# tanmayb123/OpenAI-Whisper-CoreML

Hardware: AMD Instinct MI355X
Metric: audio-sec/s (RTF) + decoder tok/s, Whisper-large-v2 30s chunks, 1->8 GPU (higher is better)
Workload: dtype bf16

## Files before the change

include/whisper_mi355x_debug.h:

```cpp
#ifndef WHISPER_MI355X_DEBUG_H
#define WHISPER_MI355X_DEBUG_H

#include "whisper_mi355x.h"

#ifdef __cplusplus
extern "C" {
#endif

WM_API int wmdbg_mel_filterbank(int n_mels, float *out);
WM_API int wmdbg_mel80(float *out);

WM_API int wmdbg_gemm(wm_ctx *ctx, const float *A, const float *W, const float *bias, float *C, int M, int N,
               int K, int epi);
WM_API int wmdbg_layernorm(wm_ctx *ctx, const float *x, const float *g, const float *b, int rows, int d,
                    float *out_f32, float *out_bf16_as_f32);
WM_API int wmdbg_enc_attention(wm_ctx *ctx, const float *q, const float *k, const float *v, int B, int H, int S,
                        float *out);
WM_API int wmdbg_dec_gemv(wm_ctx *ctx, const float *x, const float *ln_g, const float *ln_b, const float *W,
                   const float *bias, float *out, int B, int N, int K);
WM_API int wmdbg_dec_gemv_resid(wm_ctx *ctx, const float *x, const float *W, const float *bias, float *resid, float *copy_bf16,
                         float *stats, int B, int N, int K);
WM_API int wmdbg_dec_attention(wm_ctx *ctx, const float *q, const float *k, const float *v, int B, int H, int T,
                        int n_keys, int nsplit, float *out);

WM_API int wmdbg_bench_dec_gemv(wm_ctx *ctx, int B, int N, int K, int ln, int resid, int n_mats, int iters,
                         int nw_override, float *avg_us);
WM_API int wmdbg_bench_dec_attention(wm_ctx *ctx, int B, int H, int T, int n_keys, int nsplit, int n_slices,
                              int iters, float *avg_us);

WM_API int wmdbg_bench_launch_floor(wm_ctx *ctx, int iters, int grid, float *eager_us, float *graph_us);

WM_API int wmdbg_bench_graph_branches(wm_ctx *ctx, int iters, int grid, int us_each, float *one_us, float *two_us);

WM_API int wmdbg_bench_gemm(wm_ctx *ctx, int M, int N, int K, int epi, int iters, int n_w, float *us);

WM_API int wmdbg_set_gemm_tile(int tile);

WM_API int wmdbg_lane_parts(int B, int lanes, int explicit_lanes, int n_text_state);
WM_API int wmdbg_cu_mask(int cu_lo, int cu_hi, uint32_t *mask8);

WM_API int wmdbg_set_precision(wm_ctx *ctx, int precision);

WM_API int wmdbg_set_tuning(const char *key, int value);
WM_API int wmdbg_group_count(int B, int lanes, int explicit_lanes);

#ifdef __cplusplus
}
#endif
#endif
```

openai-whisper-coreml_amd/csrc/debug_hooks.cpp:

```cpp
#include <math.h>
#include <stdio.h>
#include <stdlib.h>
#include <string.h>

#include <vector>

#include "../../include/whisper_mi355x_debug.h"
#include "model.h"

int wm_gemm_set_tile_override(int tile);
extern "C" int wmdbg_set_gemm_tile(int tile) { return wm_gemm_set_tile_override(tile); }

extern "C" int wmdbg_set_tuning(const char *key, int value) {
    WM_REQUIRE(key, WM_ERR_INVALID, "wmdbg_set_tuning: null key");
    struct { const char *name; int *field; } table[] = {
        {"gemv_tn", &g_wm_tuning.gemv_tn}, {"gemv_nblk", &g_wm_tuning.gemv_nblk}, {"gemv_no_ppw2", &g_wm_tuning.gemv_no_ppw2}, {"gemv_ppw2_nblk", &g_wm_tuning.gemv_ppw2_nblk},
        {"prefetch_max_b", &g_wm_tuning.prefetch_max_b}, {"xattn_split_below", &g_wm_tuning.xattn_split_below},
        {"xattn_wgs", &g_wm_tuning.xattn_wgs}, {"xattn_no_flat", &g_wm_tuning.xattn_no_flat},
        {"xattn_lds_pad", &g_wm_tuning.xattn_lds_pad}, {"xattn_splits", &g_wm_tuning.xattn_splits},
        {"gemm_tile", &g_wm_tuning.gemm_tile}, {"gemm128_pipe", &g_wm_tuning.gemm128_pipe}, {"gemm_gm", &g_wm_tuning.gemm_gm}, {"no_early_stop", &g_wm_tuning.no_early_stop},
        {"xattn_no_deep", &g_wm_tuning.xattn_no_deep}, {"xattn_never_short", &g_wm_tuning.xattn_never_short},         {"logits_tn", &g_wm_tuning.logits_tn}, {"enc_attn_mfma_sum", &g_wm_tuning.enc_attn_mfma_sum},
        {"group_chunks", &g_wm_tuning.group_chunks}, {"argmax_rows_per_wg", &g_wm_tuning.argmax_rows_per_wg}, {"xattn_fuse_q", &g_wm_tuning.xattn_fuse_q},
        {"lane_parts", &g_wm_tuning.lane_parts}, {"lane_solo_cus", &g_wm_tuning.lane_solo_cus}, {"frontend_per_wave_twiddles", &g_wm_tuning.frontend_per_wave_twiddles},
    };
    if (strcmp(key, "reset") == 0) { g_wm_tuning = WmTuning(); return WM_OK; }
    for (auto &e : table)
        if (strcmp(key, e.name) == 0) { *e.field = value; return WM_OK; }
    wm_set_error("wmdbg_set_tuning: unknown key '%s'", key);
    return WM_ERR_INVALID;
}

extern "C" int wmdbg_group_count(int B, int lanes, int explicit_lanes) { return wm_group_count(B, lanes, explicit_lanes != 0, 0); }
extern "C" int wmdbg_lane_parts(int B, int lanes, int explicit_lanes, int n_text_state) {
    return wm_lane_parts(B, lanes, explicit_lanes != 0, n_text_state, 0);
}
extern "C" int wmdbg_cu_mask(int cu_lo, int cu_hi, uint32_t *mask8) { return wm_cu_mask(cu_lo, cu_hi, mask8); }

extern "C" int wmdbg_mel_filterbank(int n_mels, float *out) {
    WM_REQUIRE(out && n_mels > 0 && n_mels <= 256, WM_ERR_INVALID, "bad args");
    std::vector<float> f;
    wm_mel_filterbank(n_mels, f);
    memcpy(out, f.data(), f.size() * sizeof(float));
    return WM_OK;
}
extern "C" int wmdbg_mel80(float *out) {
    WM_REQUIRE(out, WM_ERR_INVALID, "null");
    memcpy(out, wm_mel80_table(), sizeof(float) * 80 * 201);
    return WM_OK;
}

static int up(void **d, const void *h, size_t bytes, hipStream_t s) {
    WM_HIP(hipMalloc(d, bytes + 512));
    WM_HIP(hipMemsetAsync(*d, 0, bytes + 512, s));
    if (h) WM_HIP(hipMemcpyAsync(*d, h, bytes, hipMemcpyHostToDevice, s));
    return WM_OK;
}
static void to_bf16(const float *in, std::vector<bf16_t> &out, size_t n) {
    out.resize(n);
    for (size_t i = 0; i < n; ++i) {
        uint32_t u;
        memcpy(&u, &in[i], 4);
        u += 0x7fffu + ((u >> 16) & 1u);
        out[i] = (bf16_t)(u >> 16);
    }
}
static void from_bf16(const std::vector<bf16_t> &in, float *out) {
    for (size_t i = 0; i < in.size(); ++i) {
        uint32_t u = (uint32_t)in[i] << 16;
        memcpy(&out[i], &u, 4);
    }
}

extern "C" int wmdbg_gemm(wm_ctx *ctx, const float *A, const float *W, const float *bias, float *C, int M, int N,
                          int K, int epi) {
    WM_TRY(wm_ctx_make_current(ctx));
    WM_REQUIRE(epi == EPI_F32 || epi == EPI_BIAS_BF16 || epi == EPI_GELU_BF16 || epi == EPI_RESID_F32, WM_ERR_INVALID,
               "wmdbg_gemm: epilogue %d not exposed", epi);
    std::vector<bf16_t> a16, w16;
    to_bf16(A, a16, (size_t)M * K);
    to_bf16(W, w16, (size_t)N * K);
    void *dA, *dW, *dB = nullptr, *dC;
    hipStream_t s = ctx->stream;
    WM_TRY(up(&dA, a16.data(), a16.size() * 2, s));
    WM_TRY(up(&dW, w16.data(), w16.size() * 2, s));
    if (bias) WM_TRY(up(&dB, bias, (size_t)N * 4, s));
    const bool f32out = (epi == EPI_F32 || epi == EPI_RESID_F32);
    WM_TRY(up(&dC, epi == EPI_RESID_F32 ? C : nullptr, (size_t)M * N * (f32out ? 4 : 2), s));
    GemmArgs g;
    memset(&g, 0, sizeof(g));
    g.A = (const bf16_t *)dA; g.a_rpb = (long)M + 1; g.a_rstride = K;
    g.W = (const bf16_t *)dW; g.bias = (const float *)dB; g.C = dC;
    g.c_rpb = (long)M + 1; g.c_rstride = N; g.M = M; g.N = N; g.K = K; g.epi = epi;
    int rc = wm_gemm(ctx, g);
    if (rc == WM_OK) {
        if (f32out) {
            WM_HIP(hipMemcpyAsync(C, dC, (size_t)M * N * 4, hipMemcpyDeviceToHost, s));
            WM_HIP(hipStreamSynchronize(s));
        } else {
            std::vector<bf16_t> c16((size_t)M * N);
            WM_HIP(hipMemcpyAsync(c16.data(), dC, c16.size() * 2, hipMemcpyDeviceToHost, s));
            WM_HIP(hipStreamSynchronize(s));
            from_bf16(c16, C);
        }
    }
    (void)hipFree(dA); (void)hipFree(dW); (void)hipFree(dC);
    if (dB) (void)hipFree(dB);
    return rc;
}

extern "C" int wmdbg_layernorm(wm_ctx *ctx, const float *x, const float *g, const float *b, int rows, int d,
                               float *out_f32, float *out_bf16_as_f32) {
    WM_TRY(wm_ctx_make_current(ctx));
    void *dx, *dg, *db, *of, *ob;
    hipStream_t s = ctx->stream;
    WM_TRY(up(&dx, x, (size_t)rows * d * 4, s));
    WM_TRY(up(&dg, g, (size_t)d * 4, s));
    WM_TRY(up(&db, b, (size_t)d * 4, s));
    WM_TRY(up(&of, nullptr, (size_t)rows * d * 4, s));
    WM_TRY(up(&ob, nullptr, (size_t)rows * d * 2, s));
    int rc = wm_layernorm(ctx, (const float *)dx, (const float *)dg, (const float *)db, rows, d, (bf16_t *)ob, (float *)of);
    if (rc == WM_OK) {
        std::vector<bf16_t> t((size_t)rows * d);
        WM_HIP(hipMemcpyAsync(out_f32, of, (size_t)rows * d * 4, hipMemcpyDeviceToHost, s));
        WM_HIP(hipMemcpyAsync(t.data(), ob, t.size() * 2, hipMemcpyDeviceToHost, s));
        WM_HIP(hipStreamSynchronize(s));
        from_bf16(t, out_bf16_as_f32);
    }
    (void)hipFree(dx); (void)hipFree(dg); (void)hipFree(db); (void)hipFree(of); (void)hipFree(ob);
    return rc;
}

extern "C" int wmdbg_enc_attention(wm_ctx *ctx, const float *q, const float *k, const float *v, int B, int H, int S,
                                   float *out) {
    WM_TRY(wm_ctx_make_current(ctx));
    const int d = H * 64, S_pad = ((S + 63) / 64) * 64;
    const size_t M = (size_t)B * S;
    std::vector<bf16_t> qk((M + 64) * 2 * d, 0), vt((size_t)B * H * 64 * S_pad, 0), tmp;
    auto bf = [](float f) { uint32_t u; memcpy(&u, &f, 4); u += 0x7fffu + ((u >> 16) & 1u); return (bf16_t)(u >> 16); };
    for (size_t mrow = 0; mrow < M; ++mrow)
        for (int j = 0; j < d; ++j) {
            qk[mrow * 2 * d + j] = bf(q[mrow * d + j] * WM_ENC_QSCALE);
            qk[mrow * 2 * d + d + j] = bf(k[mrow * d + j]);
        }
    for (int b = 0; b < B; ++b)
        for (int s = 0; s < S; ++s)
            for (int j = 0; j < d; ++j)
                vt[((size_t)(b * H + j / 64) * 64 + j % 64) * S_pad + wm_att_vt_pos((unsigned)s)] = bf(v[((size_t)b * S + s) * d + j]);
    void *dqk, *dvt, *datt;
    hipStream_t st = ctx->stream;
    WM_TRY(up(&dqk, qk.data(), qk.size() * 2, st));
    WM_TRY(up(&dvt, vt.data(), vt.size() * 2, st));
    WM_TRY(up(&datt, nullptr, M * d * 2, st));
    int rc = wm_enc_attention(ctx, (const bf16_t *)dqk, (const bf16_t *)dvt, (bf16_t *)datt, B, H, S, S_pad, d);
    if (rc == WM_OK) {
        tmp.resize(M * d);
        WM_HIP(hipMemcpyAsync(tmp.data(), datt, tmp.size() * 2, hipMemcpyDeviceToHost, st));
        WM_HIP(hipStreamSynchronize(st));
        from_bf16(tmp, out);
    }
    (void)hipFree(dqk); (void)hipFree(dvt); (void)hipFree(datt);
    return rc;
}

extern "C" int wmdbg_dec_gemv(wm_ctx *ctx, const float *x, const float *ln_g, const float *ln_b, const float *W,
                              const float *bias, float *out, int B, int N, int K) {
    WM_TRY(wm_ctx_make_current(ctx));
    WM_REQUIRE(B >= 1 && B <= WM_DEC_MAXB, WM_ERR_INVALID, "wmdbg_dec_gemv: B out of range");
    const int Npad = ((N + 15) / 16) * 16;
    std::vector<bf16_t> w16, x16;
    std::vector<float> wp((size_t)Npad * K, 0.f);
    for (size_t r = 0; r < (size_t)N; ++r)
        for (size_t k = 0; k < (size_t)K; ++k) wp[wm_tiled_offset(r, k, (size_t)K)] = W[r * K + k];
    to_bf16(wp.data(), w16, wp.size());
    {
        const int Bpad = ((B + 15) / 16) * 16;
        std::vector<float> xp((size_t)Bpad * K, 0.f);
        for (size_t b = 0; b < (size_t)B; ++b)
            for (size_t k = 0; k < (size_t)K; ++k) xp[wm_tiled_offset(b, k, (size_t)K)] = x[b * K + k];
        to_bf16(xp.data(), x16, xp.size());
    }
    void *dx16, *dg = nullptr, *db = nullptr, *dW, *dWf = nullptr, *dc1 = nullptr, *dc2 = nullptr, *dbias = nullptr, *dout;
    hipStream_t s = ctx->stream;
    WM_TRY(up(&dx16, x16.data(), x16.size() * 2, s));
    WM_TRY(up(&dW, w16.data(), w16.size() * 2, s));
    WM_TRY(up(&dout, nullptr, (size_t)B * N * 4, s));
    if (bias) WM_TRY(up(&dbias, bias, (size_t)N * 4, s));
    DecGemvArgs a;
    memset(&a, 0, sizeof(a));
    a.B = B; a.N = N; a.K = K; a.W = (const bf16_t *)dW; a.c2 = (const float *)dbias; a.a = (const bf16_t *)dx16;
    a.out_f32 = (float *)dout; a.ldo = N; a.epi = DE_Q; a.pos_ptr = nullptr;
    void *dst = nullptr;
    int rc = WM_OK;
    if (ln_g) {
        WM_TRY(up(&dg, ln_g, (size_t)K * 4, s));
        WM_TRY(up(&db, ln_b, (size_t)K * 4, s));
        WM_TRY(up(&dWf, nullptr, w16.size() * 2, s));
        WM_TRY(up(&dc1, nullptr, (size_t)Npad * 4, s));
        WM_TRY(up(&dc2, nullptr, (size_t)Npad * 4, s));
        rc = wm_ln_fold(ctx, (const bf16_t *)dW, (const float *)dg, (const float *)db, (const float *)dbias, N, K,
                        (bf16_t *)dWf, (float *)dc1, (float *)dc2);
        const int nblk = (B + 15) / 16;
        std::vector<float> st((size_t)nblk * 2 * K, 0.f);
        for (int b = 0; b < B; ++b)
            for (int k = 0; k < K; ++k) {
                const int part = k >> 4;
                const float v = x[(size_t)b * K + k];
                float *blk = st.data() + (size_t)(b >> 4) * 2 * K;
                blk[(part * 16 + (b & 15)) * 2] += v;
                blk[(part * 16 + (b & 15)) * 2 + 1] += v * v;
            }
        WM_TRY(up(&dst, st.data(), st.size() * 4, s));
        a.stats_in = (const float *)dst; a.stats_parts = K / 16;
        a.W = (const bf16_t *)dWf; a.c1 = (const float *)dc1; a.c2 = (const float *)dc2;
    }
    if (rc == WM_OK) rc = wm_dec_gemv(ctx, a);
    if (rc == WM_OK) {
        WM_HIP(hipMemcpyAsync(out, dout, (size_t)B * N * 4, hipMemcpyDeviceToHost, s));
        WM_HIP(hipStreamSynchronize(s));
    }
    void *fr[] = {dx16, dg, db, dW, dWf, dc1, dc2, dbias, dout, dst};
    for (void *p : fr)
        if (p) (void)hipFree(p);
    return rc;
}

extern "C" int wmdbg_dec_gemv_resid(wm_ctx *ctx, const float *x, const float *W, const float *bias, float *resid,
                                    float *copy_bf16, float *stats, int B, int N, int K) {
    WM_TRY(wm_ctx_make_current(ctx));
    WM_REQUIRE(B >= 1 && B <= WM_DEC_MAXB && N % 16 == 0, WM_ERR_INVALID, "wmdbg_dec_gemv_resid: B out of range / N % 16");
    const int Bpad = ((B + 15) / 16) * 16;
    std::vector<bf16_t> w16, x16;
    {
        std::vector<float> wp((size_t)N * K, 0.f), xp((size_t)Bpad * K, 0.f);
        for (size_t r = 0; r < (size_t)N; ++r)
            for (size_t k = 0; k < (size_t)K; ++k) wp[wm_tiled_offset(r, k, (size_t)K)] = W[r * K + k];
        for (size_t b = 0; b < (size_t)B; ++b)
            for (size_t k = 0; k < (size_t)K; ++k) xp[wm_tiled_offset(b, k, (size_t)K)] = x[b * K + k];
        to_bf16(wp.data(), w16, wp.size());
        to_bf16(xp.data(), x16, xp.size());
    }
    void *dx16, *dW, *dbias = nullptr, *dres, *dcopy, *dst;
    hipStream_t s = ctx->stream;
    WM_TRY(up(&dx16, x16.data(), x16.size() * 2, s));
    WM_TRY(up(&dW, w16.data(), w16.size() * 2, s));
    WM_TRY(up(&dres, resid, (size_t)B * N * 4, s));
    WM_TRY(up(&dcopy, nullptr, (size_t)Bpad * N * 2, s));
    WM_TRY(up(&dst, nullptr, (size_t)(Bpad / 16) * 2 * N * 4, s));
    if (bias) WM_TRY(up(&dbias, bias, (size_t)N * 4, s));
    DecGemvArgs a;
    memset(&a, 0, sizeof(a));
    a.epi = DE_RESID; a.B = B; a.N = N; a.K = K; a.W = (const bf16_t *)dW; a.c2 = (const float *)dbias;
    a.a = (const bf16_t *)dx16; a.out_f32 = (float *)dres; a.out_bf16 = (bf16_t *)dcopy; a.ldo = N;
    a.stats_out = (float *)dst;
    int rc = wm_dec_gemv(ctx, a);
    if (rc == WM_OK) {
        std::vector<bf16_t> c16((size_t)Bpad * N), lin((size_t)B * N);
        std::vector<float> st((size_t)(Bpad / 16) * 2 * N);
        WM_HIP(hipMemcpyAsync(resid, dres, (size_t)B * N * 4, hipMemcpyDeviceToHost, s));
        WM_HIP(hipMemcpyAsync(c16.data(), dcopy, c16.size() * 2, hipMemcpyDeviceToHost, s));
        WM_HIP(hipMemcpyAsync(st.data(), dst, st.size() * 4, hipMemcpyDeviceToHost, s));
        WM_HIP(hipStreamSynchronize(s));
        for (size_t b = 0; b < (size_t)B; ++b)
            for (size_t n = 0; n < (size_t)N; ++n) lin[b * N + n] = c16[wm_tiled_offset(b, n, (size_t)N)];
        from_bf16(lin, copy_bf16);
        for (int b = 0; b < B; ++b) {
            const float *blk = st.data() + (size_t)(b >> 4) * 2 * N;
            float s1 = 0.f, s2 = 0.f;
            for (int part = 0; part < N / 16; ++part) {
                s1 += blk[(part * 16 + (b & 15)) * 2];
                s2 += blk[(part * 16 + (b & 15)) * 2 + 1];
            }
            stats[b * 2] = s1;
            stats[b * 2 + 1] = s2;
        }
    }
    void *fr[] = {dx16, dW, dbias, dres, dcopy, dst};
    for (void *p : fr)
        if (p) (void)hipFree(p);
    return rc;
}

extern "C" int wmdbg_dec_attention(wm_ctx *ctx, const float *q, const float *k, const float *v, int B, int H, int T,
                                   int n_keys, int nsplit, float *out) {
    WM_TRY(wm_ctx_make_current(ctx));
    std::vector<bf16_t> k16, v16;
    to_bf16(k, k16, (size_t)B * H * T * 64);
    to_bf16(v, v16, (size_t)B * H * T * 64);
    void *dq, *dk, *dv, *dp;
    hipStream_t s = ctx->stream;
    WM_TRY(up(&dq, q, (size_t)B * H * 64 * 4, s));
    WM_TRY(up(&dk, k16.data(), k16.size() * 2, s));
    WM_TRY(up(&dv, v16.data(), v16.size() * 2, s));
    WM_TRY(up(&dp, nullptr, (size_t)B * H * WM_MAXSPLIT * 66 * 4, s));
    void *datt;
    WM_TRY(up(&datt, nullptr, ((size_t)B + 15) / 16 * 16 * H * 64 * 2, s));
    int rc = nsplit == 0 ? wm_dec_self_attention(ctx, (const float *)dq, (const bf16_t *)dk, (const bf16_t *)dv, B, H, T,
                                                 n_keys, nullptr, (bf16_t *)datt)
                         : wm_dec_attention(ctx, (const float *)dq, (const bf16_t *)dk, (const bf16_t *)dv, B, H, T, n_keys,
                                            nullptr, nsplit < 0 ? 1 : nsplit, (float *)dp, (bf16_t *)datt, nsplit < 0);
    if (rc == WM_OK) {
        const size_t Bpad = ((size_t)B + 15) / 16 * 16, dd = (size_t)H * 64;
        std::vector<bf16_t> o16(Bpad * dd), lin((size_t)B * dd);
        WM_HIP(hipMemcpyAsync(o16.data(), datt, o16.size() * 2, hipMemcpyDeviceToHost, s));
        WM_HIP(hipStreamSynchronize(s));
        for (size_t b = 0; b < (size_t)B; ++b)
            for (size_t k = 0; k < dd; ++k) lin[b * dd + k] = o16[wm_tiled_offset(b, k, dd)];
        from_bf16(lin, out);
    }
    (void)hipFree(datt);
    (void)hipFree(dq); (void)hipFree(dk); (void)hipFree(dv); (void)hipFree(dp);
    return rc;
}


extern "C" int wmdbg_bench_dec_gemv(wm_ctx *ctx, int B, int N, int K, int ln, int resid, int n_mats, int iters,
                                    int nw_override, float *avg_us) {
    (void)nw_override;
    WM_TRY(wm_ctx_make_current(ctx));
    WM_REQUIRE(B >= 1 && B <= WM_DEC_MAXB, WM_ERR_INVALID, "wmdbg_bench_dec_gemv: B out of range");
    hipStream_t s = ctx->stream;
    const int Npad = ((N + 15) / 16) * 16;
    void *dW, *dx16, *dc, *dout, *dout16;
    WM_TRY(up(&dW, nullptr, (size_t)n_mats * Npad * K * 2, s));
    WM_TRY(up(&dx16, nullptr, (size_t)WM_DEC_MAXB * K * 2, s));
    WM_TRY(up(&dc, nullptr, (size_t)Npad * 4, s));
    WM_TRY(up(&dout, nullptr, (size_t)WM_DEC_MAXB * Npad * 4, s));
    WM_TRY(up(&dout16, nullptr, (size_t)WM_DEC_MAXB * Npad * 2, s));
    WM_HIP(hipMemsetAsync(dW, 0x3c, (size_t)n_mats * Npad * K * 2, s));
    DecGemvArgs a;
    memset(&a, 0, sizeof(a));
    a.B = B; a.N = N; a.K = K; a.out_f32 = (float *)dout; a.ldo = Npad; a.epi = resid ? DE_RESID : DE_Q;
    a.a = (const bf16_t *)dx16; a.c2 = (const float *)dc;
    void *dstat;
    WM_TRY(up(&dstat, nullptr, (size_t)(WM_DEC_MAXB / 16) * 2 * (K > N ? K : N) * 4 + 4096, s));
    if (resid) { a.stats_out = (float *)dstat; a.out_bf16 = (bf16_t *)dout16; }
    if (ln) { a.c1 = (const float *)dc; a.stats_in = (const float *)dstat; a.stats_parts = K / 16; }
    hipEvent_t e0, e1;
    WM_HIP(hipEventCreate(&e0));
    WM_HIP(hipEventCreate(&e1));
    int rc = WM_OK;
    hipGraph_t g = nullptr;
    hipGraphExec_t ge = nullptr;
    WM_HIP(hipStreamBeginCapture(s, hipStreamCaptureModeThreadLocal));
    for (int i = 0; i < iters && rc == WM_OK; ++i) {
        a.W = (const bf16_t *)dW + (size_t)(i % n_mats) * Npad * K;
        rc = wm_dec_gemv(ctx, a);
    }
    WM_HIP(hipStreamEndCapture(s, &g));
    if (rc == WM_OK) {
        WM_HIP(hipGraphInstantiate(&ge, g, nullptr, nullptr, 0));
        WM_HIP(hipGraphLaunch(ge, s));
        WM_HIP(hipStreamSynchronize(s));
        WM_HIP(hipEventRecord(e0, s));
        WM_HIP(hipGraphLaunch(ge, s));
    }
    WM_HIP(hipEventRecord(e1, s));
    WM_HIP(hipStreamSynchronize(s));
    float ms = 0.f;
    WM_HIP(hipEventElapsedTime(&ms, e0, e1));
    *avg_us = ms * 1e3f / iters;
    (void)hipEventDestroy(e0); (void)hipEventDestroy(e1);
    if (ge) (void)hipGraphExecDestroy(ge);
    if (g) (void)hipGraphDestroy(g);
    void *fr[] = {dW, dx16, dc, dout, dout16, dstat};
    for (void *p : fr) (void)hipFree(p);
    return rc;
}

extern "C" int wmdbg_bench_dec_attention(wm_ctx *ctx, int B, int H, int T, int n_keys, int nsplit, int n_slices,
                                         int iters, float *avg_us) {
    WM_TRY(wm_ctx_make_current(ctx));
    hipStream_t s = ctx->stream;
    const size_t slice = (size_t)B * H * T * 64;
    void *dk, *dv, *dq, *dp, *datt;
    WM_TRY(up(&dk, nullptr, slice * n_slices * 2, s));
    WM_TRY(up(&dv, nullptr, slice * n_slices * 2, s));
    WM_TRY(up(&dq, nullptr, (size_t)B * H * 64 * 4, s));
    WM_TRY(up(&dp, nullptr, (size_t)B * H * WM_MAXSPLIT * 66 * 4, s));
    WM_TRY(up(&datt, nullptr, ((size_t)B + 15) / 16 * 16 * H * 64 * 2, s));
    hipEvent_t e0, e1;
    WM_HIP(hipEventCreate(&e0));
    WM_HIP(hipEventCreate(&e1));
    int rc = WM_OK;
    for (int pass = 0; pass < 2 && rc == WM_OK; ++pass) {
        if (pass == 1) WM_HIP(hipEventRecord(e0, s));
        for (int i = 0; i < iters && rc == WM_OK; ++i)
            rc = wm_dec_attention(ctx, (const float *)dq, (const bf16_t *)dk + (size_t)(i % n_slices) * slice,
                                  (const bf16_t *)dv + (size_t)(i % n_slices) * slice, B, H, T, n_keys, nullptr, nsplit,
                                  (float *)dp, (bf16_t *)datt, true);
    }
    WM_HIP(hipEventRecord(e1, s));
    WM_HIP(hipStreamSynchronize(s));
    float ms = 0.f;
    WM_HIP(hipEventElapsedTime(&ms, e0, e1));
    *avg_us = ms * 1e3f / iters;
    (void)hipEventDestroy(e0); (void)hipEventDestroy(e1);
    void *fr[] = {dk, dv, dq, dp, datt};
    for (void *p : fr) (void)hipFree(p);
    return rc;
}

int wm_launch_trivial(wm_ctx *ctx, int *p, int grid);
extern "C" int wmdbg_bench_launch_floor(wm_ctx *ctx, int iters, int grid, float *eager_us, float *graph_us) {
    WM_TRY(wm_ctx_make_current(ctx));
    hipStream_t s = ctx->stream;
    void *d;
    WM_TRY(up(&d, nullptr, 64, s));
    hipEvent_t e0, e1;
    WM_HIP(hipEventCreate(&e0));
    WM_HIP(hipEventCreate(&e1));
    for (int i = 0; i < 20; ++i) WM_TRY(wm_launch_trivial(ctx, (int *)d, grid));
    WM_HIP(hipEventRecord(e0, s));
    for (int i = 0; i < iters; ++i) WM_TRY(wm_launch_trivial(ctx, (int *)d, grid));
    WM_HIP(hipEventRecord(e1, s));
    WM_HIP(hipStreamSynchronize(s));
    float ms = 0.f;
    WM_HIP(hipEventElapsedTime(&ms, e0, e1));
    *eager_us = ms * 1e3f / iters;
    hipGraph_t g;
    hipGraphExec_t ge;
    WM_HIP(hipStreamBeginCapture(s, hipStreamCaptureModeThreadLocal));
    for (int i = 0; i < iters; ++i) (void)wm_launch_trivial(ctx, (int *)d, grid);
    WM_HIP(hipStreamEndCapture(s, &g));
    WM_HIP(hipGraphInstantiate(&ge, g, nullptr, nullptr, 0));
    WM_HIP(hipGraphLaunch(ge, s));
    WM_HIP(hipStreamSynchronize(s));
    WM_HIP(hipEventRecord(e0, s));
    WM_HIP(hipGraphLaunch(ge, s));
    WM_HIP(hipEventRecord(e1, s));
    WM_HIP(hipStreamSynchronize(s));
    WM_HIP(hipEventElapsedTime(&ms, e0, e1));
    *graph_us = ms * 1e3f / iters;
    (void)hipGraphExecDestroy(ge); (void)hipGraphDestroy(g);
    (void)hipEventDestroy(e0); (void)hipEventDestroy(e1); (void)hipFree(d);
    return WM_OK;
}

extern "C" int wmdbg_bench_gemm(wm_ctx *ctx, int M, int N, int K, int epi, int iters, int n_w, float *us) {
    WM_TRY(wm_ctx_make_current(ctx));
    WM_REQUIRE(epi == EPI_F32 || epi == EPI_BIAS_BF16 || epi == EPI_GELU_BF16 || epi == EPI_RESID_F32, WM_ERR_INVALID,
               "wmdbg_bench_gemm: epilogue %d not exposed", epi);
    WM_REQUIRE(n_w >= 1 && n_w <= 64, WM_ERR_INVALID, "wmdbg_bench_gemm: n_w out of range");
    hipStream_t s = ctx->stream;
    std::vector<bf16_t> a16((size_t)M * K), w16((size_t)N * K);
    uint32_t x = 12345u;
    auto gauss = [&]() {
        float acc = 0.f;
        for (int i = 0; i < 4; ++i) { x = x * 1664525u + 1013904223u; acc += (float)(x >> 8) * (1.0f / 16777216.0f); }
        return (acc - 2.0f) * 1.7320508f;
    };
    auto f2bf = [](float f) {
        uint32_t u;
        memcpy(&u, &f, 4);
        u += 0x7fffu + ((u >> 16) & 1u);
        return (bf16_t)(u >> 16);
    };
    for (auto &v : a16) v = f2bf(gauss());
    for (auto &v : w16) v = f2bf(0.02f * gauss());
    std::vector<float> bias(N);
    for (auto &v : bias) v = 0.01f * gauss();
    void *dA, *dB, *dC;
    std::vector<void *> dW(n_w, nullptr);
    WM_TRY(up(&dA, a16.data(), a16.size() * 2, s));
    for (int i = 0; i < n_w; ++i) WM_TRY(up(&dW[i], w16.data(), w16.size() * 2, s));
    WM_TRY(up(&dB, bias.data(), (size_t)N * 4, s));
    WM_TRY(up(&dC, nullptr, (size_t)M * N * 4, s));
    GemmArgs g;
    memset(&g, 0, sizeof(g));
    g.A = (const bf16_t *)dA; g.a_rpb = (long)M + 1; g.a_rstride = K;
    g.bias = (const float *)dB; g.C = dC;
    g.c_rpb = (long)M + 1; g.c_rstride = N; g.M = M; g.N = N; g.K = K; g.epi = epi;
    hipEvent_t e0, e1;
    WM_HIP(hipEventCreate(&e0));
    WM_HIP(hipEventCreate(&e1));
    for (int i = 0; i < 3; ++i) { g.W = (const bf16_t *)dW[i % n_w]; WM_TRY(wm_gemm(ctx, g)); }
    WM_HIP(hipEventRecord(e0, s));
    for (int i = 0; i < iters; ++i) { g.W = (const bf16_t *)dW[i % n_w]; WM_TRY(wm_gemm(ctx, g)); }
    WM_HIP(hipEventRecord(e1, s));
    WM_HIP(hipStreamSynchronize(s));
    float ms = 0.f;
    WM_HIP(hipEventElapsedTime(&ms, e0, e1));
    *us = ms * 1e3f / iters;
    (void)hipEventDestroy(e0); (void)hipEventDestroy(e1);
    (void)hipFree(dA); (void)hipFree(dB); (void)hipFree(dC);
    for (void *w : dW) (void)hipFree(w);
    return WM_OK;
}

int wm_launch_spin(hipStream_t s, int *p, int grid, int cycles);
extern "C" int wmdbg_bench_graph_branches(wm_ctx *ctx, int iters, int grid, int us_each, float *one_us, float *two_us) {
    WM_TRY(wm_ctx_make_current(ctx));
    hipStream_t s = ctx->stream, s2;
    WM_HIP(hipStreamCreateWithFlags(&s2, hipStreamNonBlocking));
    void *d;
    WM_TRY(up(&d, nullptr, 256, s));
    const int cycles = us_each * 100;
    hipEvent_t e0, e1, ef, ej;
    WM_HIP(hipEventCreate(&e0)); WM_HIP(hipEventCreate(&e1));
    WM_HIP(hipEventCreateWithFlags(&ef, hipEventDisableTiming)); WM_HIP(hipEventCreateWithFlags(&ej, hipEventDisableTiming));
    for (int nb = 1; nb <= 2; ++nb) {
        hipGraph_t g; hipGraphExec_t ge;
        WM_HIP(hipStreamBeginCapture(s, hipStreamCaptureModeThreadLocal));
        if (nb == 2) { WM_HIP(hipEventRecord(ef, s)); WM_HIP(hipStreamWaitEvent(s2, ef, 0)); }
        for (int i = 0; i < iters; ++i) {
            WM_TRY(wm_launch_spin(s, (int *)d, grid, cycles));
            if (nb == 2) WM_TRY(wm_launch_spin(s2, (int *)d + 16, grid, cycles));
        }
        if (nb == 2) { WM_HIP(hipEventRecord(ej, s2)); WM_HIP(hipStreamWaitEvent(s, ej, 0)); }
        WM_HIP(hipStreamEndCapture(s, &g));
        WM_HIP(hipGraphInstantiate(&ge, g, nullptr, nullptr, 0));
        WM_HIP(hipGraphLaunch(ge, s));
        WM_HIP(hipStreamSynchronize(s));
        WM_HIP(hipEventRecord(e0, s));
        WM_HIP(hipGraphLaunch(ge, s));
        WM_HIP(hipEventRecord(e1, s));
        WM_HIP(hipStreamSynchronize(s));
        float ms = 0.f;
        WM_HIP(hipEventElapsedTime(&ms, e0, e1));
        *(nb == 1 ? one_us : two_us) = ms * 1e3f;
        (void)hipGraphExecDestroy(ge); (void)hipGraphDestroy(g);
    }
    (void)hipEventDestroy(e0); (void)hipEventDestroy(e1); (void)hipEventDestroy(ef); (void)hipEventDestroy(ej);
    (void)hipStreamDestroy(s2); (void)hipFree(d);
    return WM_OK;
}
```

openai-whisper-coreml_amd/csrc/dec_kernels.hip:

```cpp
#include <stdlib.h>

#include <atomic>
#include <string.h>

#include "model.h"

namespace {

typedef __attribute__((ext_vector_type(8))) __bf16 bf16x8;
typedef __attribute__((ext_vector_type(4))) float f32x4;
typedef __attribute__((ext_vector_type(4))) unsigned u32x4;

typedef __attribute__((ext_vector_type(2))) float f32x2;
typedef __attribute__((ext_vector_type(2))) __bf16 bf16x2;

__device__ __forceinline__ bf16_t f2bf(float f) {
    const __bf16 h = (__bf16)f;
    return __builtin_bit_cast(bf16_t, h);
}
__device__ __forceinline__ float bf2f(bf16_t h) { return __uint_as_float((unsigned)h << 16); }
__device__ __forceinline__ unsigned pack2(float a, float b) {
    const f32x2 v = {a, b};
    return __builtin_bit_cast(unsigned, __builtin_convertvector(v, bf16x2));
}
// ... 208 lines not shown
            if (bvalid && nrow == 0) p.tilemax[(long)b * p.n_tiles + tile] = key;
            if (bvalid && nvalid && p.out_f32) p.out_f32[(long)b * p.ldo + n] = v;
            continue;
        }
        if (EPI == DE_RESID) {
            float xn = 0.f;
            if (bvalid && nvalid) {
                xn = o.xold[r] + v;
                p.out_f32[(long)b * p.ldo + n] = xn;
                if (p.out_bf16) p.out_bf16[wm_tiled_offset((size_t)b, (size_t)n, (size_t)p.ldo)] = f2bf(xn - o.off4[r]);
            }
            float s1 = xn, s2 = xn * xn;
#pragma unroll
            for (int q = 1; q < 16; q <<= 1) {
                s1 += __shfl_xor(s1, q);
                s2 += __shfl_xor(s2, q);
            }
            if (p.stats_out && nrow == 0)
                *(float2 *)(p.stats_out + (long)(b0 >> 4) * p.stats_stride + ((long)tile * 16 + bl) * 2) = make_float2(s1, s2);
            continue;
        }
        if (!bvalid || !nvalid) continue;
        if (EPI == DE_QKV) {
            const int d = p.N / 3;
            if (n < d) {
                p.out_f32[(long)b * d + n] = v;
            } else {
                const int hn = (n < 2 * d) ? n - d : n - 2 * d;
                bf16_t *c = (n < 2 * d) ? p.kcache : p.vcache;
                c[((long)(b * p.n_head + (hn >> 6)) * p.n_ctx + pos) * 64 + (hn & 63)] = f2bf(v);
            }
        } else if (EPI == DE_Q) {
            p.out_f32[(long)b * p.ldo + n] = v;
        } else if (EPI == DE_GELU) {
            p.out_bf16[wm_tiled_offset((size_t)b, (size_t)n, (size_t)p.ldo)] = f2bf(gelu_erf(v));
        }
    }
}

#define GEMV_PIN(x) asm volatile("" ::"s"(x))
template <int SPW, int TN, int NBLK, int EPI, bool LN, int PPW = 1, int RSP = 1>
__global__ __launch_bounds__((LN || SPW == 12 || TN * NBLK > 1 || PPW > 1) ? 512 : 1024) void dec_gemv_kernel(
    const bf16_t *__restrict__ hotW, const bf16_t *__restrict__ hotA, const int *__restrict__ hot_pos_ptr,
    const float *__restrict__ hot_c2, int hotK, int hot_n_tiles, int hotB, int hot_bgroups, int hot_n_tg, int hot_n_tg_pad,
    float *hot_out_f32, DecGemvDev pc) {
    extern __shared__ __attribute__((aligned(16))) char smem[];
    DecGemvDev p = pc;
    p.W = hotW; p.a = hotA; p.pos_ptr = hot_pos_ptr; p.c2 = hot_c2; p.K = hotK; p.n_tiles = hot_n_tiles; p.B = hotB;
    p.bgroups = hot_bgroups; p.n_tg = hot_n_tg; p.n_tg_pad = hot_n_tg_pad; p.out_f32 = hot_out_f32;
    constexpr int NU = TN * NBLK;
    const int NP = (p.K >> 5) / SPW;
    const int NW = NP / PPW;
    const int G = p.bgroups;
    const int wg = blockIdx.x;
    const int q = wg >> 3;
    const int tg = G == 1 ? wg : (q / G) * 8 + (wg & 7);
    const int grp = G == 1 ? 0 : q % G;
    if (wg >= p.n_tg_pad * G || tg >= p.n_tg) {
        int t = wg - p.n_tg_pad * G;
        if (p.pf_head_major && t >= 0) {
            const int per = p.pf_head_major, x = t & 7, m = t >> 3;
            const int hh = (x * per) / p.B + (m >> 2);
            const int end = (x + 1) * per < (p.pf_tiles >> 2) * p.B ? (x + 1) * per : (p.pf_tiles >> 2) * p.B;
            t = hh * p.B < end ? hh * 4 + (m & 3) : -1;
        }
        if (t >= 0 && t < p.pf_tiles) l2_warm_tile(p.pf_ptr, p.pf_tile_bytes, t, NW * 64);
        return;
    }
    float *red = (float *)smem;
    float *st = red + NP * NU * 256 + (threadIdx.x >> 6) * 32;
    const int tid = threadIdx.x, lane = tid & 63, wave = tid >> 6;
    const int nrow = lane & 15;
    const int tile0 = tg * TN;
    const int bb = grp * NBLK * 16;

    u32x4 wf[TN][SPW];
    auto load_wf = [&](int part) {
#pragma unroll
        for (int t = 0; t < TN; ++t) {
            const int tc = tile0 + t < p.n_tiles ? tile0 + t : p.n_tiles - 1;
            const bf16_t *wp = p.W + (((long)tc * (p.K >> 5) + (long)part * SPW) * 64 + lane) * 8;
#pragma unroll
#ifdef WM_GEMV_W_NONTEMPORAL
            for (int u = 0; u < SPW; ++u) wf[t][u] = __builtin_nontemporal_load((const u32x4 *)(wp + u * 512));
#else
            for (int u = 0; u < SPW; ++u) wf[t][u] = *(const u32x4 *)(wp + u * 512);
#endif
        }
    };
    load_wf(wave);
    u32x4 af[NBLK][SPW];
    auto load_af = [&](int part) {
#pragma unroll
        for (int j = 0; j < NBLK; ++j) {
            const int blk = (bb >> 4) + j;
            const int blkc = blk * 16 < p.B ? blk : (bb >> 4);
            const bf16_t *ap = p.a + (((long)blkc * (p.K >> 5) + (long)part * SPW) * 64 + lane) * 8;
#pragma unroll
            for (int u = 0; u < SPW; ++u) af[j][u] = *(const u32x4 *)(ap + u * 512);
        }
    };
    load_af(wave);
    GEMV_PIN(p.N); GEMV_PIN(p.ldo);
    if (LN) { GEMV_PIN(p.c1); GEMV_PIN(p.stats_in); GEMV_PIN(p.stats_stride); GEMV_PIN(p.mean_in); GEMV_PIN(p.mean_out); }
    if (EPI == DE_RESID) { GEMV_PIN(p.out_bf16); GEMV_PIN(p.stats_out); GEMV_PIN(p.stats_stride); GEMV_PIN(p.mean_in); }
    if (EPI == DE_QKV) { GEMV_PIN(p.kcache); GEMV_PIN(p.vcache); GEMV_PIN(p.n_ctx); GEMV_PIN(p.n_head); }
    if (EPI == DE_GELU) GEMV_PIN(p.out_bf16);
    if (EPI == DE_LOGITS) {
        GEMV_PIN(p.tilemax); GEMV_PIN(p.arg_first); GEMV_PIN(p.arg_last); GEMV_PIN(p.mask); GEMV_PIN(p.mask_words);
        GEMV_PIN(p.mask_first_pos); GEMV_PIN(p.ts.rng); GEMV_PIN(p.ts.key_ts); GEMV_PIN(p.ts.lse); GEMV_PIN(p.ts.ts_begin);
    }
    int pos = 0;
    unsigned mword0 = 0u, mword1 = 0u;
    GemvUnitOps<EPI, LN> ops;
    constexpr int RS = RSP;
    static_assert(RSP == 1 || RSP == 4, "row split: 1 or 4 waves per unit");
    constexpr int rs_shift = RS == 4 ? 2 : 0;
    const int ntask = NU << rs_shift;
    const bool has_unit = wave < ntask;
    const int my_u = wave >> rs_shift;
    const int my_r0 = RS == 4 ? (wave & 3) : 0, my_r1 = RS == 4 ? my_r0 + 1 : 4;
    const bool my_stats = my_r0 == 0;
    int utile = tile0, ub0 = bb;
    if (has_unit) {
        utile = tile0 + my_u % TN;
        ub0 = bb + (my_u / TN) * 16;
        if (utile >= p.n_tiles) utile = p.n_tiles - 1;
        if (ub0 >= p.B) ub0 = bb;
        gemv_unit_load<EPI, LN>(p, ops, utile, ub0, lane, my_r0, my_r1, my_stats);
    }
    if (p.pos_ptr) pos = *p.pos_ptr;
    if (EPI == DE_LOGITS && p.mask && has_unit) {
        const int n = utile * 16 + nrow;
        const int nc = n < p.N ? n : p.N - 1;
        mword0 = p.mask[nc >> 5];
        mword1 = p.mask[p.mask_words + (nc >> 5)];
    }

    f32x4 acc[NBLK][TN];
#pragma unroll
    for (int pp = 0; pp < PPW; ++pp) {
        const int part = wave + pp * NW;
        if (pp > 0) {
            load_wf(part);
            load_af(part);
        }
#pragma unroll
        for (int j = 0; j < NBLK; ++j)
#pragma unroll
            for (int t = 0; t < TN; ++t) {
                f32x4 a4 = {0.f, 0.f, 0.f, 0.f};
#pragma unroll
                for (int u = 0; u < SPW; ++u)
                    a4 = __builtin_amdgcn_mfma_f32_16x16x32_bf16(__builtin_bit_cast(bf16x8, af[j][u]),
                                                                 __builtin_bit_cast(bf16x8, wf[t][u]), a4, 0, 0, 0);
                acc[j][t] = a4;
            }
        if (PPW > 1 || NU > 1 || wave != 0 || RS == 4) {
#pragma unroll
            for (int j = 0; j < NBLK; ++j)
#pragma unroll
                for (int t = 0; t < TN; ++t) *(f32x4 *)(red + ((part * NU + j * TN + t) * 64 + lane) * 4) = acc[j][t];
        }
    }
    float *stbase = red + NP * NU * 256;
    if (has_unit && my_stats) gemv_unit_stats<EPI, LN>(p, ops, stbase + (RS == 4 ? my_u : wave) * 32, lane, utile, ub0);
    __syncthreads();
    for (int tk = wave; tk < ntask; tk += NW) {
        const int u = tk >> rs_shift;
        const int t = u % TN, j = u / TN;
        const int tile = tile0 + t, b0 = bb + j * 16;
        if (tile >= p.n_tiles || b0 >= p.B) continue;
        st = stbase + (RS == 4 ? u : wave) * 32;
        if (tk != wave) {
            gemv_unit_load<EPI, LN>(p, ops, tile, b0, lane);
            gemv_unit_stats<EPI, LN>(p, ops, st, lane, tile, b0);
            if (EPI == DE_LOGITS && p.mask) {
                const int n = tile * 16 + nrow;
                const int nc = n < p.N ? n : p.N - 1;
                mword0 = p.mask[nc >> 5];
                mword1 = p.mask[p.mask_words + (nc >> 5)];
            }
        }
        f32x4 sum;
        if (RS == 4) {
            const float *rp = red + (u * 64 + lane) * 4 + my_r0;
            float s1 = rp[0];
            for (int w = 1; w < NP; ++w) s1 += rp[w * NU * 256];
            sum = f32x4{s1, s1, s1, s1};
        } else {
            sum = (NU == 1 && PPW == 1) ? acc[0][0] : *(const f32x4 *)(red + ((0 * NU + u) * 64 + lane) * 4);
            for (int w = 1; w < NP; ++w) sum += *(const f32x4 *)(red + ((w * NU + u) * 64 + lane) * 4);
        }
        gemv_unit_epilogue<EPI, LN>(p, ops, sum, st, tile, b0, lane, pos, mword0, mword1, my_r0, my_r1);
    }
}

__global__ __launch_bounds__(256) void ln_fold_kernel(const bf16_t *__restrict__ W, const float *__restrict__ g,
                                                      const float *__restrict__ beta, const float *__restrict__ bias,
                                                      int N, int K, bf16_t *__restrict__ Wf, float *__restrict__ c1,
                                                      float *__restrict__ c2) {
    __shared__ float r1[4], r2[4];
    const int n = blockIdx.x;
    float s1 = 0.f, s2 = 0.f;
    for (int k = threadIdx.x; k < K; k += 256) {
        const size_t o = wm_tiled_offset((size_t)n, (size_t)k, (size_t)K);
        const float w = bf2f(W[o]);
        const bf16_t wf = f2bf(w * g[k]);
        Wf[o] = wf;
        s1 += bf2f(wf);
        s2 += beta[k] * w;
    }
#pragma unroll
    for (int o = 32; o > 0; o >>= 1) {
        s1 += __shfl_xor(s1, o);
        s2 += __shfl_xor(s2, o);
    }
    if ((threadIdx.x & 63) == 0) {
        r1[threadIdx.x >> 6] = s1;
        r2[threadIdx.x >> 6] = s2;
    }
    __syncthreads();
    if (threadIdx.x == 0) {
        c1[n] = (r1[0] + r1[1]) + (r1[2] + r1[3]);
        c2[n] = (n < N && bias ? bias[n] : 0.f) + ((r2[0] + r2[1]) + (r2[2] + r2[3]));
    }
}

__global__ __launch_bounds__(256) void dec_embed_kernel(const int *__restrict__ seq, const int *__restrict__ pos_ptr,
                                                        int B, const bf16_t *__restrict__ emb,
                                                        const float *__restrict__ pemb, int d,
                                                        float *__restrict__ x, bf16_t *__restrict__ xb,
                                                        float *__restrict__ stats_out, float *__restrict__ mean_buf) {
    __shared__ float r1[4], r2[4];
    const int b = blockIdx.x;
    const int pos = *pos_ptr;
    const long tok = seq[pos * B + b];
    float s1 = 0.f, s2 = 0.f;
    for (int j = threadIdx.x; j < d; j += 256) {
        const float v = bf2f(emb[wm_tiled_offset((size_t)tok, (size_t)j, (size_t)d)]) + pemb[(long)pos * d + j];
        x[(long)b * d + j] = v;
        s1 += v;
        s2 += v * v;
    }
#pragma unroll
    for (int o = 32; o > 0; o >>= 1) {
        s1 += __shfl_xor(s1, o);
        s2 += __shfl_xor(s2, o);
    }
    if ((threadIdx.x & 63) == 0) {
        r1[threadIdx.x >> 6] = s1;
        r2[threadIdx.x >> 6] = s2;
    }
    __syncthreads();
    {
        const float mean = ((r1[0] + r1[1]) + (r1[2] + r1[3])) / (float)d;
        for (int j = threadIdx.x; j < d; j += 256)
            xb[wm_tiled_offset((size_t)b, (size_t)j, (size_t)d)] = f2bf(x[(long)b * d + j] - mean);
        if (threadIdx.x == 0 && mean_buf) mean_buf[b] = mean;
    }
    if (stats_out) {
        float *blk = stats_out + (long)(b >> 4) * (2 * d) + (b & 15) * 2;
        for (int pt = 1 + threadIdx.x; pt < d / 16; pt += 256) *(float2 *)(blk + pt * 32) = make_float2(0.f, 0.f);
        if (threadIdx.x == 0)
            *(float2 *)blk = make_float2((r1[0] + r1[1]) + (r1[2] + r1[3]), (r2[0] + r2[1]) + (r2[2] + r2[3]));
    }
}

constexpr int ATT_MAXK = 1536;
#ifndef WM_XATTN_NT
#define WM_XATTN_NT true
#endif

template <int NS>
__device__ __forceinline__ float attn_merge(const float *m, const float *l, const float *o, int ostride, int e) {
    float mm[NS], ll[NS], oo[NS];
#pragma unroll
    for (int w = 0; w < NS; ++w) {
        mm[w] = m[w];
        ll[w] = l[w];
        oo[w] = o[w * ostride + e];
    }
    return attn_merge_core<NS>(mm, ll, oo);
}


template <int NS, int U, bool NT>
__device__ __forceinline__ void attn_load_block(const bf16_t *kb, const bf16_t *vb, int r0, const int &stream, const int &rg,
                                                int lim, int clamp, u32x4 (&kv)[U], u32x4 (&vv)[U]) {
#pragma unroll
    for (int u = 0; u < U; ++u) {
        int i = r0 + u * (NS * 8) + stream * 8 + rg;
        i = i < lim ? i : clamp;
        if (NT) {
            kv[u] = __builtin_nontemporal_load((const u32x4 *)(kb + (long)i * 64));
            vv[u] = __builtin_nontemporal_load((const u32x4 *)(vb + (long)i * 64));
        } else {
            kv[u] = *(const u32x4 *)(kb + (long)i * 64);
            vv[u] = *(const u32x4 *)(vb + (long)i * 64);
        }
    }
}

template <int U>
__device__ __forceinline__ void attn_block_fence(u32x4 (&kv)[U], u32x4 (&vv)[U]) {
    static_assert(U == 4, "attn_block_fence is written for 4 loads per block");
    asm volatile("" : "+v"(kv[0]), "+v"(kv[1]), "+v"(kv[2]), "+v"(kv[3]), "+v"(vv[0]), "+v"(vv[1]), "+v"(vv[2]), "+v"(vv[3]));
}

template <int NS, int U, bool MASK_V>
__device__ __forceinline__ void attn_block(const float (&qe)[8], int r0, int stream, int rg, int n_keys, const u32x4 (&kv)[U],
                                           const u32x4 (&vv)[U], float &m_run, float &l_run, float (&oa)[8]) {
    float sc[U];
    float mb = -1e30f;
#pragma unroll
    for (int u = 0; u < U; ++u) {
        const int i = r0 + u * (NS * 8) + stream * 8 + rg;
        float a = 0.f;
#pragma unroll
        for (int j = 0; j < 4; ++j) {
            a = __fmaf_rn(qe[2 * j], __uint_as_float(kv[u][j] << 16), a);
            a = __fmaf_rn(qe[2 * j + 1], __uint_as_float(kv[u][j] & 0xffff0000u), a);
        }
        a += __shfl_xor(a, 1);
        a += __shfl_xor(a, 2);
        a += __shfl_xor(a, 4);
        sc[u] = i < n_keys ? a : -1e30f;
        mb = fmaxf(mb, sc[u]);
    }
    mb = fmaxf(mb, __shfl_xor(mb, 8));
    mb = fmaxf(mb, __shfl_xor(mb, 16));
    mb = fmaxf(mb, __shfl_xor(mb, 32));
    const float m_new = fmaxf(m_run, mb);
    const float resc = __expf(m_run - m_new);
    l_run *= resc;
#pragma unroll
    for (int j = 0; j < 8; ++j) oa[j] *= resc;
#pragma unroll
    for (int u = 0; u < U; ++u) {
        const bool live_row = sc[u] > -1e29f;
        const float pv = live_row ? __expf(sc[u] - m_new) : 0.f;
        l_run += pv;
#pragma unroll
        for (int j = 0; j < 4; ++j) {
            const unsigned vw = (MASK_V && !live_row) ? 0u : vv[u][j];
            oa[2 * j] = __fmaf_rn(pv, __uint_as_float(vw << 16), oa[2 * j]);
            oa[2 * j + 1] = __fmaf_rn(pv, __uint_as_float(vw & 0xffff0000u), oa[2 * j + 1]);
        }
    }
    m_run = m_new;
}

__device__ __forceinline__ void attn_stream_reduce(float &l_run, float (&oa)[8]) {
#pragma unroll
    for (int i = 0; i < 8; ++i) {
        oa[i] += __shfl_xor(oa[i], 8);
        oa[i] += __shfl_xor(oa[i], 16);
        oa[i] += __shfl_xor(oa[i], 32);
    }
    l_run += __shfl_xor(l_run, 8);
    l_run += __shfl_xor(l_run, 16);
    l_run += __shfl_xor(l_run, 32);
}

struct AttnCold {
    bf16_t *att;
    float *part;
    const char *pf_ptr;
    long pf_tile_bytes;
};
template <int NS, int U, bool NT, bool DEEP = false>
__global__ __launch_bounds__(DEEP ? 256 : NS * 64) void dec_rows_attn_kernel(
    const float *__restrict__ q, const bf16_t *__restrict__ kc, const bf16_t *__restrict__ vc,
    const int *__restrict__ pos_ptr, const int *__restrict__ live_rows ,
    unsigned packA , unsigned packB ,
    unsigned packC , AttnCold cold) {
    const int H = (int)(packA & 0xffu), nsplit = (int)((packA >> 8) & 0xffu), flat_wpw = (int)(packA >> 16);
    const int T_stride = (int)(packB & 0xffffu), n_keys_const = (int)(packB >> 16);
    const int n_bh_full = (int)(packC & 0xffffu), n_wg = (int)(packC >> 16);
    const int d = H * 64;
    const int *n_live_ptr = live_rows ? live_rows + WM_DEC_MAXB : nullptr;
    constexpr bool SELF = NS == 4;
    if ((int)blockIdx.x >= n_wg) {
        l2_warm_tile(cold.pf_ptr, cold.pf_tile_bytes, (int)blockIdx.x - n_wg, blockDim.x);
        return;
    }
    __shared__ float wm_[NS], wl_[NS];
    __shared__ float wo_[NS][64];
    const int tid = threadIdx.x, lane = tid & 63, wave = tid >> 6;
    const int rg = lane >> 3, e8 = lane & 7;
    int stream = (int)blockIdx.y * (NS / nsplit) + wave;
    int bh0 = blockIdx.x, bh_step = n_wg;
    if (flat_wpw > 0) {
        const int unit = (int)blockIdx.x * flat_wpw + wave;
        if (unit >= n_bh_full * NS) return;
        bh0 = unit / NS;
        stream = unit % NS;
        bh_step = n_bh_full;
    }
    const int *dummy = (const int *)q;
    const int pos_raw = *(pos_ptr ? pos_ptr : dummy);
    const int nl_raw = *(n_live_ptr ? n_live_ptr : dummy);
    const int n_clamp = SELF ? T_stride - 1 : n_keys_const - 1;
    auto load_block = [&](const bf16_t *kb, const bf16_t *vb, int r0, int clamp, u32x4 (&kv)[U], u32x4 (&vv)[U]) {
        attn_load_block<NS, U, NT>(kb, vb, r0, stream, rg, clamp, clamp, kv, vv);
    };
    bool first = true;
    int n_bh = n_bh_full, n_keys = n_keys_const;
    for (int pi = bh0; pi < n_bh; pi += bh_step) {
        if (flat_wpw == 0 && !first) __syncthreads();
        const int h = pi % H;
        int b = pi / H;
        if (live_rows) b = live_rows[pi / H];
        const int bh = b * H + h;
        const bf16_t *kb = kc + (long)bh * T_stride * 64 + e8 * 8;
        const bf16_t *vb = vc + (long)bh * T_stride * 64 + e8 * 8;
        const f32x4 *qp = (const f32x4 *)(q + (long)b * d + h * 64 + e8 * 8);
        const f32x4 q0 = qp[0], q1 = qp[1];
        constexpr bool SPEC = SELF || DEEP;
        constexpr int NB = DEEP ? ATT_MAXK / (NS * 8 * U) : 1;
        u32x4 kall[NB][U], vall[NB][U];
        if (SPEC) {
#pragma unroll
            for (int blk = 0; blk < NB; ++blk)
                load_block(kb, vb, blk * (NS * 8 * U), first ? n_clamp : n_keys - 1, kall[blk], vall[blk]);
        }
        if (first) {
            int pos_v = pos_raw, nl_v = nl_raw;
            if (SPEC) asm volatile("" : "+s"(pos_v), "+s"(nl_v) : "v"(q0[0]));
            if (n_live_ptr) n_bh = nl_v * H;
            if (pos_ptr) n_keys = pos_v + 1;
            first = false;
            if (pi >= n_bh) break;
        }
        float qe[8];
#pragma unroll
        for (int i = 0; i < 4; ++i) {
            qe[i] = q0[i] * 0.125f;
            qe[4 + i] = q1[i] * 0.125f;
        }
        float m_run = -1e30f, l_run = 0.f;
        float oa[8] = {0, 0, 0, 0, 0, 0, 0, 0};
        auto process_block = [&](int r0, const u32x4 (&kv)[U], const u32x4 (&vv)[U]) {
            attn_block<NS, U, SELF>(qe, r0, stream, rg, n_keys, kv, vv, m_run, l_run, oa);
        };
        if (DEEP) {
#pragma unroll
            for (int blk = 0; blk < NB; ++blk)
                if (blk * (NS * 8 * U) < n_keys) process_block(blk * (NS * 8 * U), kall[blk], vall[blk]);
        } else {
            if (SPEC) {
                attn_block_fence<U>(kall[0], vall[0]);
                process_block(0, kall[0], vall[0]);
            }
            for (int r0 = SPEC ? NS * 8 * U : 0; r0 < n_keys; r0 += NS * 8 * U) {
                u32x4 kv[U], vv[U];
                load_block(kb, vb, r0, n_keys - 1, kv, vv);
                attn_block_fence<U>(kv, vv);
                process_block(r0, kv, vv);
            }
        }
        attn_stream_reduce(l_run, oa);
        if (nsplit > 1) {
            if (rg == 0) {
                float *po = cold.part + ((long)bh * NS + stream) * 66;
#pragma unroll
                for (int i = 0; i < 8; ++i) po[2 + e8 * 8 + i] = oa[i];
                if (e8 == 0) {
                    po[0] = m_run;
                    po[1] = l_run;
                }
            }
            continue;
        }
        if (rg == 0) {
#pragma unroll
            for (int i = 0; i < 8; ++i) wo_[wave][e8 * 8 + i] = oa[i];
            if (e8 == 0) {
                wm_[wave] = m_run;
                wl_[wave] = l_run;
            }
        }
        __syncthreads();
        if (tid < 64)
            cold.att[wm_tiled_offset((size_t)b, (size_t)(h * 64 + tid), (size_t)d)] = f2bf(attn_merge<NS>(wm_, wl_, &wo_[0][0], 64, tid));
    }
}

template <int NS, int U, bool NT, bool DEEP = false>
__global__ __launch_bounds__(DEEP ? 256 : NS * 64) void dec_xrows_attn_kernel(
    const float *__restrict__ q, const bf16_t *__restrict__ kc, const bf16_t *__restrict__ vc,
    const int *__restrict__ pos_ptr, const int *__restrict__ live_rows ,
    unsigned packA , unsigned packB ,
    unsigned packC , AttnCold cold) {
    const int H = (int)(packA & 0xffu), nsplit = (int)((packA >> 8) & 0xffu), flat_wpw = (int)(packA >> 16);
    const int T_stride = (int)(packB & 0xffffu), n_keys_const = (int)(packB >> 16);
    int n_bh = (int)(packC & 0xffffu);
    const int n_wg = (int)(packC >> 16);
    const int d = H * 64;
    const int *n_live_ptr = live_rows ? live_rows + WM_DEC_MAXB : nullptr;
    bf16_t *att = cold.att;
    float *part = cold.part;
    const char *pf_ptr = cold.pf_ptr;
    const long pf_tile_bytes = cold.pf_tile_bytes;
    if ((int)blockIdx.x >= n_wg) {
        l2_warm_tile(pf_ptr, pf_tile_bytes, (int)blockIdx.x - n_wg, blockDim.x);
        return;
    }
    if (n_live_ptr) n_bh = *n_live_ptr * H;
    __shared__ float wm_[NS], wl_[NS];
    __shared__ float wo_[NS][64];
    const int tid = threadIdx.x, lane = tid & 63, wave = tid >> 6;
    const int rg = lane >> 3, e8 = lane & 7;
    const int n_keys = pos_ptr ? (*pos_ptr + 1) : n_keys_const;
    const int last = n_keys - 1;
    int stream = (int)blockIdx.y * (NS / nsplit) + wave;
    int bh0 = blockIdx.x, bh_step = n_wg;
    if (flat_wpw > 0) {
        const int unit = (int)blockIdx.x * flat_wpw + wave;
        if (unit >= n_bh * NS) return;
        bh0 = unit / NS;
        stream = unit % NS;
        bh_step = n_bh;
    }
    for (int pi = bh0; pi < n_bh; pi += bh_step) {
        if (flat_wpw == 0 && pi != (int)blockIdx.x) __syncthreads();
        const int h = pi % H;
        const int b = live_rows ? live_rows[pi / H] : pi / H;
        const int bh = b * H + h;
        const bf16_t *kb = kc + (long)bh * T_stride * 64 + e8 * 8;
        const bf16_t *vb = vc + (long)bh * T_stride * 64 + e8 * 8;
        float qe[8];
        {
            const float *qp = q + (long)b * d + h * 64 + e8 * 8;
#pragma unroll
            for (int i = 0; i < 8; ++i) qe[i] = qp[i] * 0.125f;
        }
        float m_run = -1e30f, l_run = 0.f;
        float oa[8] = {0, 0, 0, 0, 0, 0, 0, 0};
        auto load_block = [&](int r0, u32x4 (&kv)[U], u32x4 (&vv)[U]) {
            attn_load_block<NS, U, NT>(kb, vb, r0, stream, rg, n_keys, last, kv, vv);
        };
        auto process_block = [&](int r0, const u32x4 (&kv)[U], const u32x4 (&vv)[U]) {
            attn_block<NS, U, false>(qe, r0, stream, rg, n_keys, kv, vv, m_run, l_run, oa);
        };
        if (DEEP) {
            constexpr int NB = ATT_MAXK / (NS * 8 * U);
            u32x4 kall[NB][U], vall[NB][U];
#pragma unroll
            for (int blk = 0; blk < NB; ++blk) load_block(blk * (NS * 8 * U), kall[blk], vall[blk]);
#pragma unroll
            for (int blk = 0; blk < NB; ++blk)
                if (blk * (NS * 8 * U) < n_keys) process_block(blk * (NS * 8 * U), kall[blk], vall[blk]);
        } else {
            for (int r0 = 0; r0 < n_keys; r0 += NS * 8 * U) {
                u32x4 kv[U], vv[U];
                load_block(r0, kv, vv);
                process_block(r0, kv, vv);
            }
        }
        attn_stream_reduce(l_run, oa);
        if (nsplit > 1) {
            if (rg == 0) {
                float *po = part + ((long)bh * NS + stream) * 66;
#pragma unroll
                for (int i = 0; i < 8; ++i) po[2 + e8 * 8 + i] = oa[i];
                if (e8 == 0) {
                    po[0] = m_run;
                    po[1] = l_run;
                }
            }
            continue;
        }
        if (rg == 0) {
#pragma unroll
            for (int i = 0; i < 8; ++i) wo_[wave][e8 * 8 + i] = oa[i];
            if (e8 == 0) {
                wm_[wave] = m_run;
                wl_[wave] = l_run;
            }
        }
        __syncthreads();
        if (tid < 64)
            att[wm_tiled_offset((size_t)b, (size_t)(h * 64 + tid), (size_t)d)] = f2bf(attn_merge<NS>(wm_, wl_, &wo_[0][0], 64, tid));
    }
}


struct FqCold {
    const float *c1, *c2, *stats_in, *mean_in;
    float *mean_out;
    bf16_t *att;
    long stats_stride;
    int K, N;
    const char *pf_ptr;
    long pf_tile_bytes;
    int n_wg;
};
template <int SPW, bool NT>
__global__ __launch_bounds__(512) void dec_xattn_fq_kernel(const bf16_t *__restrict__ Wq, const bf16_t *__restrict__ xb,
                                                           const bf16_t *__restrict__ kc, const bf16_t *__restrict__ vc,
                                                           const int *__restrict__ live_rows, unsigned packA ,
                                                           unsigned packB , int K, FqCold cold) {
    constexpr int NS = 8, U = 4;
    extern __shared__ __attribute__((aligned(16))) char smem[];
    const int H = (int)(packA & 0xffu), B = (int)(packA >> 8);
    const int T_stride = (int)(packB & 0xffffu), n_keys = (int)(packB >> 16);
    const int tid = threadIdx.x, lane = tid & 63, wave = tid >> 6;
    const int rg = lane >> 3, e8 = lane & 7;
    if ((int)blockIdx.x >= cold.n_wg) {
        l2_warm_tile(cold.pf_ptr, cold.pf_tile_bytes, (int)blockIdx.x - cold.n_wg, 512);
        return;
    }
    const int per = (H * B + 7) >> 3;
    const int pidx = ((int)blockIdx.x >> 3) + per * ((int)blockIdx.x & 7);
    if (((int)blockIdx.x >> 3) >= per || pidx >= H * B) return;
    const int h = pidx / B, bi = pidx % B;
    int n_live = B;
    if (live_rows) n_live = live_rows[WM_DEC_MAXB];
    int b = bi;
    if (live_rows) b = live_rows[bi];
    const int NP = (K >> 5) / SPW;
    const int blk = b >> 4, bl = b & 15;
    float *red = (float *)smem;
    float *stbase = red + NP * 4 * 256;
    float *q_lds = stbase + 4 * 32;
    u32x4 wf[4][SPW], af[SPW];
    if (wave < NP) {
#pragma unroll
        for (int t = 0; t < 4; ++t) {
            const bf16_t *wp = Wq + (((long)(h * 4 + t) * (K >> 5) + (long)wave * SPW) * 64 + lane) * 8;
#pragma unroll
            for (int u = 0; u < SPW; ++u) wf[t][u] = *(const u32x4 *)(wp + u * 512);
        }
        const bf16_t *ap = xb + (((long)blk * (K >> 5) + (long)wave * SPW) * 64 + lane) * 8;
#pragma unroll
        for (int u = 0; u < SPW; ++u) af[u] = *(const u32x4 *)(ap + u * 512);
    }
    DecGemvDev p = {};
    p.B = B; p.N = cold.N; p.K = K; p.c1 = cold.c1; p.c2 = cold.c2; p.stats_in = cold.stats_in;
    p.stats_stride = cold.stats_stride; p.mean_in = cold.mean_in; p.mean_out = cold.mean_out;
    p.out_f32 = nullptr; p.ts.rng = nullptr;
    GemvUnitOps<DE_Q, true> ops;
    const int my_tile = h * 4 + (wave & 3);
    if (wave < 4) gemv_unit_load<DE_Q, true>(p, ops, my_tile, blk * 16, lane, 0, 4, true);
    const int stream = wave;
    const int bh = b * H + h;
    const bf16_t *kb = kc + (long)bh * T_stride * 64 + e8 * 8;
    const bf16_t *vb = vc + (long)bh * T_stride * 64 + e8 * 8;
    auto load_block = [&](int r0, u32x4 (&kv)[U], u32x4 (&vv)[U]) {
        attn_load_block<NS, U, NT>(kb, vb, r0, stream, rg, n_keys - 1, n_keys - 1, kv, vv);
    };
    u32x4 kv0[U], vv0[U];
    load_block(0, kv0, vv0);
    if (bi >= n_live) return;
    if (wave < NP) {
#pragma unroll
        for (int t = 0; t < 4; ++t) {
            f32x4 a4 = {0.f, 0.f, 0.f, 0.f};
#pragma unroll
            for (int u = 0; u < SPW; ++u)
                a4 = __builtin_amdgcn_mfma_f32_16x16x32_bf16(__builtin_bit_cast(bf16x8, af[u]), __builtin_bit_cast(bf16x8, wf[t][u]), a4, 0, 0, 0);
            *(f32x4 *)(red + ((wave * 4 + t) * 64 + lane) * 4) = a4;
        }
    }
    if (wave < 4) gemv_unit_stats<DE_Q, true>(p, ops, stbase + wave * 32, lane, my_tile, blk * 16);
    __syncthreads();
    if (wave < 4) {
        f32x4 sum = *(const f32x4 *)(red + ((0 * 4 + wave) * 64 + lane) * 4);
        for (int w = 1; w < NP; ++w) sum += *(const f32x4 *)(red + ((w * 4 + wave) * 64 + lane) * 4);
        const float2 ms = *(const float2 *)(stbase + wave * 32 + bl * 2);
        const int kq = lane >> 4, nrow = lane & 15;
        float v = 0.f;
#pragma unroll
        for (int r = 0; r < 4; ++r)
            if (kq * 4 + r == bl) v = __fmaf_rn(ms.x, sum[r], __fmaf_rn(ms.y, ops.c1v, ops.c2v));
        if (kq == (bl >> 2)) q_lds[wave * 16 + nrow] = v;
    }
    __syncthreads();
    float qe[8];
#pragma unroll
    for (int i = 0; i < 8; ++i) qe[i] = q_lds[e8 * 8 + i] * 0.125f;
    float m_run = -1e30f, l_run = 0.f;
    float oa[8] = {0, 0, 0, 0, 0, 0, 0, 0};
    auto process_block = [&](int r0, const u32x4 (&kv)[U], const u32x4 (&vv)[U]) {
        attn_block<NS, U, false>(qe, r0, stream, rg, n_keys, kv, vv, m_run, l_run, oa);
    };
    process_block(0, kv0, vv0);
    for (int r0 = NS * 8 * U; r0 < n_keys; r0 += NS * 8 * U) {
        u32x4 kv[U], vv[U];
        load_block(r0, kv, vv);
        attn_block_fence<U>(kv, vv);
        process_block(r0, kv, vv);
    }
    attn_stream_reduce(l_run, oa);
    float *wm_ = red, *wl_ = red + NS, *wo_ = red + 2 * NS;
    __syncthreads();
    if (rg == 0) {
#pragma unroll
        for (int i = 0; i < 8; ++i) wo_[wave * 64 + e8 * 8 + i] = oa[i];
        if (e8 == 0) {
            wm_[wave] = m_run;
            wl_[wave] = l_run;
        }
    }
    __syncthreads();
    if (tid < 64)
        cold.att[wm_tiled_offset((size_t)b, (size_t)(h * 64 + tid), (size_t)(H * 64))] = f2bf(attn_merge<NS>(wm_, wl_, wo_, 64, tid));
}

template <int NS>
__global__ __launch_bounds__(64) void dec_attn_combine_kernel(const float *__restrict__ part, int H, int d,
                                                              bf16_t *__restrict__ att) {
    __shared__ float wm_[NS], wl_[NS];
    const int bh = blockIdx.x, b = bh / H, h = bh % H, e = threadIdx.x;
    const float *pp = part + (long)bh * NS * 66;
    float oo[NS], mm[NS], ll[NS];
#pragma unroll
    for (int w = 0; w < NS; ++w) oo[w] = pp[2 + w * 66 + e];
    if (e < NS) {
        wm_[e] = pp[e * 66];
        wl_[e] = pp[e * 66 + 1];
    }
    __syncthreads();
#pragma unroll
    for (int w = 0; w < NS; ++w) {
        mm[w] = wm_[w];
        ll[w] = wl_[w];
    }
    att[wm_tiled_offset((size_t)b, (size_t)(h * 64 + e), (size_t)d)] = f2bf(attn_merge_core<NS>(mm, ll, oo));
}

__global__ __launch_bounds__(1024) void argmax_embed_kernel(const unsigned long long *__restrict__ tilemax,
                                                             int n_tiles, int B, int *__restrict__ seq,
                                                             int *__restrict__ pos_ptr, int n_prompt,
                                                             int *__restrict__ result, int arg_first,
                                                             const bf16_t *__restrict__ emb,
                                                             const float *__restrict__ pemb, int d, int n_ctx,
                                                             float *__restrict__ x, bf16_t *__restrict__ xb,
                                                             float *__restrict__ stats_out, WmTsDev ts,
                                                             int *__restrict__ arrive, int fallback_tok,
                                                             float *__restrict__ mean_buf, WmStopDev stop, int rpw) {
    __shared__ int tok_s[16];
    __shared__ int is_last_s;
    const int lane = threadIdx.x & 63, wave = threadIdx.x >> 6;
    const int pos_raw = *(pos_ptr ? pos_ptr : (const int *)tilemax);
    int pos = 0;
    const int bw = blockIdx.x * rpw;
    __shared__ unsigned long long part_s[16][16];
    const int nrows = B - bw < rpw ? B - bw : rpw;
    const int hpr = (16 - nrows) / nrows;
    const int P = 1 + hpr;
    int my_row = -1, my_pi = 0;
    if (wave < nrows) { my_row = wave; }
    else if (wave - nrows < hpr * nrows) { my_row = (wave - nrows) % nrows; my_pi = 1 + (wave - nrows) / nrows; }
    if (my_row >= 0) {
        const unsigned long long *row = tilemax + (long)(bw + my_row) * n_tiles;
        const int chunk = (n_tiles + P - 1) / P, t_lo = my_pi * chunk, t_hi = t_lo + chunk < n_tiles ? t_lo + chunk : n_tiles;
        unsigned long long key = 0ull;
        for (int t0 = t_lo + lane; t0 < t_hi; t0 += 64 * 8) {
            unsigned long long k[8];
#pragma unroll
            for (int u = 0; u < 8; ++u) {
                const int t = t0 + 64 * u;
                k[u] = row[t < t_hi ? t : t0];
            }
#pragma unroll
            for (int u = 0; u < 8; ++u) key = k[u] > key ? k[u] : key;
        }
#pragma unroll
        for (int o = 32; o > 0; o >>= 1) {
            const unsigned long long ok = __shfl_xor(key, o);
            key = ok > key ? ok : key;
        }
        if (lane == 0) part_s[my_row][my_pi] = key;
    }
    __syncthreads();
    for (int b = bw + wave; b < B && b < bw + nrows; b += 16) {
        unsigned long long key = lane < P ? part_s[wave][lane] : 0ull;
        {
            int pv = pos_raw;
            asm volatile("" : "+s"(pv) : "v"((unsigned)key));
            pos = pos_ptr ? pv : 0;
        }
#pragma unroll
        for (int o = 8; o > 0; o >>= 1) {
            const unsigned long long ok = __shfl_xor(key, o);
            key = ok > key ? ok : key;
        }
        key = __shfl(key, 0);
        if (ts.rng) {
            const int t_first = ts.ts_begin >> 4;
            unsigned long long kts = 0ull;
            float M = -1e30f;
            for (int t = t_first + lane; t < n_tiles; t += 64) {
                const unsigned long long k2 = ts.key_ts[(long)b * n_tiles + t];
                kts = k2 > kts ? k2 : kts;
                M = fmaxf(M, ts.lse[((long)b * n_tiles + t) * 2]);
            }
#pragma unroll
            for (int o = 32; o > 0; o >>= 1) {
                const unsigned long long ok = __shfl_xor(kts, o);
                kts = ok > kts ? ok : kts;
                M = fmaxf(M, __shfl_xor(M, o));
            }
            float S = 0.f;
            for (int t = t_first + lane; t < n_tiles; t += 64) {
                const float2 ms = *(const float2 *)(ts.lse + ((long)b * n_tiles + t) * 2);
                S += ms.y * __expf(ms.x - M);
            }
#pragma unroll
            for (int o = 32; o > 0; o >>= 1) S += __shfl_xor(S, o);
            unsigned u = (unsigned)(key >> 32);
            u = (u & 0x80000000u) ? (u & 0x7fffffffu) : ~u;
            const float text_best = key ? __uint_as_float(u) : -1e30f;
            const float lse = S > 0.f ? M + __logf(S) : -1e30f;
            if (kts != 0ull && (key == 0ull || lse > text_best)) key = kts;
            else key = kts > key ? kts : key;
        }
        if (lane == 0) {
            int tok = key ? (int)(0xFFFFFFFFu - (unsigned)(key & 0xFFFFFFFFull)) : fallback_tok;
            if (stop.done && pos + 1 >= n_prompt) {
                const int gi = pos + 1 - n_prompt;
                if (stop.done[b]) {
                    tok = stop.pad_tok;
                } else if ((stop.eot >= 0 && tok == stop.eot) || (stop.budget && gi + 1 >= stop.budget[b])) {
                    stop.done[b] = 1;
                }
            }
            if (ts.rng && pos + 1 >= n_prompt) {
                int *hs = ts.hist + b * 4;
                const int n_s = hs[0] + 1;
                const bool prev_ts = hs[0] < 1 || hs[1] != 0;
                const bool last_ts = tok >= ts.ts_begin;
                const int last_val = last_ts ? tok : hs[3];
                hs[0] = n_s; hs[2] = hs[1]; hs[1] = last_ts ? 1 : 0; hs[3] = last_val;
                int text_lo = 0, text_hi = ts.ts_begin, ts_lo = ts.ts_begin, ts_hi = ts.n_vocab;
                if (last_ts) {
                    if (prev_ts) ts_hi = ts_lo;
                    else text_lo = ts.eot;
                }
                if (last_val >= 0) {
                    const int floor_ts = (last_ts && !prev_ts) ? last_val : last_val + 1;
                    ts_lo = floor_ts > ts_lo ? floor_ts : ts_lo;
                }
                *(int4 *)(ts.rng + b * 4) = make_int4(text_lo, text_hi, ts_lo, ts_hi);
            }
            int nxt = tok;
            if (seq) {
                if (pos + 1 >= n_prompt) seq[(pos + 1) * B + b] = tok;
                else nxt = seq[(pos + 1) * B + b];
            }
            tok_s[b - bw] = nxt;
            if (result) result[b] = tok - arg_first;
        }
    }
    __syncthreads();
    {
        int pv = pos_raw;
        asm volatile("" : "+s"(pv));
        pos = pos_ptr ? pv : 0;
    }
    if (x && pos + 1 < n_ctx) {
        for (int b = bw + wave; b < B && b < bw + nrows; b += 16) {
            const long tok = tok_s[b - bw];
            float s1 = 0.f, s2 = 0.f;
            constexpr int EV = 8;
            float ev[EV];
#pragma unroll
            for (int i = 0; i < EV; ++i) {
                const int j = lane + 64 * i;
                ev[i] = 0.f;
                if (j < d) {
                    const float v = bf2f(emb[wm_tiled_offset((size_t)tok, (size_t)j, (size_t)d)]) + pemb[(long)(pos + 1) * d + j];
                    x[(long)b * d + j] = v;
                    ev[i] = v;
                    s1 += v;
                    s2 += v * v;
                }
            }
            for (int j = lane + 64 * EV; j < d; j += 64) {
                const float v = bf2f(emb[wm_tiled_offset((size_t)tok, (size_t)j, (size_t)d)]) + pemb[(long)(pos + 1) * d + j];
                x[(long)b * d + j] = v;
                s1 += v;
                s2 += v * v;
            }
#pragma unroll
            for (int o = 32; o > 0; o >>= 1) {
                s1 += __shfl_xor(s1, o);
                s2 += __shfl_xor(s2, o);
            }
            {
                const float mean = s1 / (float)d;
#pragma unroll
                for (int i = 0; i < EV; ++i) {
                    const int j = lane + 64 * i;
                    if (j < d) xb[wm_tiled_offset((size_t)b, (size_t)j, (size_t)d)] = f2bf(ev[i] - mean);
                }
                for (int j = lane + 64 * EV; j < d; j += 64)
                    xb[wm_tiled_offset((size_t)b, (size_t)j, (size_t)d)] = f2bf(x[(long)b * d + j] - mean);
                if (lane == 0 && mean_buf) mean_buf[b] = mean;
            }
            if (stats_out) {
                float *blk = stats_out + (long)(b >> 4) * (2 * d) + (b & 15) * 2;
                for (int pt = 1 + lane; pt < d / 16; pt += 64) *(float2 *)(blk + pt * 32) = make_float2(0.f, 0.f);
                if (lane == 0) *(float2 *)blk = make_float2(s1, s2);
            }
        }
    }
    __syncthreads();
    if (!stop.done) {
        if (threadIdx.x == 0 && pos_ptr) {
            if (gridDim.x == 1) {
                *pos_ptr = pos + 1;
            } else if (atomicAdd(arrive, 1) == (int)gridDim.x - 1) {
                *arrive = 0;
                *pos_ptr = pos + 1;
            }
        }
        return;
    }
    if (threadIdx.x == 0) {
        int last = 1;
        if (gridDim.x > 1) {
            __threadfence();
            last = atomicAdd(arrive, 1) == (int)gridDim.x - 1;
            if (last) {
                *arrive = 0;
                __threadfence();
            }
        }
        is_last_s = last;
    }
    __syncthreads();
    if (is_last_s && wave == 0) {
        int n = 0;
        for (int b0 = 0; b0 < B; b0 += 64) {
            const int b = b0 + lane;
            const bool live = b < B && __hip_atomic_load(stop.done + (b < B ? b : 0), __ATOMIC_RELAXED, __HIP_MEMORY_SCOPE_AGENT) == 0;
            const unsigned long long m = __ballot(live);
            if (live) stop.live_rows[n + __popcll(m & ((1ull << lane) - 1ull))] = b;
            n += __popcll(m);
        }
        if (lane == 0) {
            *stop.n_live = n;
            if (pos_ptr) *pos_ptr = pos + 1;
        }
    }
}

__global__ void dec_live_init_kernel(WmStopDev stop, int B) {
    const int b = threadIdx.x;
    if (b < B) {
        stop.done[b] = 0;
        stop.live_rows[b] = b;
    }
    if (b == 0) *stop.n_live = B;
}

__device__ __forceinline__ unsigned hash32(unsigned x) {
    x ^= x >> 16;
    x *= 0x7feb352du;
    x ^= x >> 15;
    x *= 0x846ca68bu;
    x ^= x >> 16;
    return x;
}
__global__ __launch_bounds__(256) void synth_fill_kernel(void *dst, int is_bf16, size_t n, unsigned key,
                                                         float scale, int layout, int conv_c, int kpad,
                                                         int kind, float gain) {
    for (size_t i = (size_t)blockIdx.x * 256 + threadIdx.x; i < n; i += (size_t)gridDim.x * 256) {
        float v;
        if (kind == 2) {
            v = 1.0f;
        } else if (kind == 3) {
            v = 0.0f;
        } else {
            const unsigned h1 = hash32((unsigned)i ^ key);
            const unsigned h2 = hash32(h1 + 0x85ebca6bu);
            const int s = (int)(h1 & 0xffffu) + (int)(h1 >> 16) + (int)(h2 & 0xffffu) + (int)(h2 >> 16);
            v = __fmul_rn(__fmul_rn((float)(s - 131070), scale), gain);
        }
        size_t o = i;
        if (layout == WL_CONV) {
            const size_t per = (size_t)conv_c * 3;
            const size_t oc = i / per, rem = i % per, c = rem / 3, tap = rem % 3;
            o = oc * kpad + tap * conv_c + c;
        } else if (layout == WL_TILED) {
            o = wm_tiled_offset(i / (size_t)kpad, i % (size_t)kpad, (size_t)kpad);
        }
        if (is_bf16)
            ((bf16_t *)dst)[o] = f2bf(v);
        else
            ((float *)dst)[o] = (kind == 0) ? bf2f(f2bf(v)) : v;
    }
}

#define GEMV_ARGS(p) (p).W, (p).a, (p).pos_ptr, (p).c2, (p).K, (p).n_tiles, (p).B, (p).bgroups, (p).n_tg, (p).n_tg_pad, (p).out_f32, (p)
template <int SPW, int EPI, bool LN>
int launch_gemv_shape(wm_ctx *ctx, const DecGemvDev &p, int tn, int nblk, int nw, int grid, int ppw) {
    hipStream_t s = ctx->stream;
    if (ppw == 2) {
        constexpr bool TWO = !LN && EPI == DE_RESID && SPW >= 6 && SPW <= 10;
        if (!TWO || tn != 1 || nblk < 1 || nblk > 2 || nw % 2) { wm_set_error("dec_gemv: no two-part kernel for this shape"); return WM_ERR_INVALID; }
        const int w2 = nw / 2;
        const size_t lds2 = (size_t)nw * nblk * 1024 + (size_t)w2 * 32 * 4;
        if (nblk == 2) {
            if (w2 != 8) { wm_set_error("dec_gemv: the two-block two-part kernel needs 8 waves"); return WM_ERR_INVALID; }
            dec_gemv_kernel<TWO ? SPW : 6, 1, 2, TWO ? EPI : DE_RESID, TWO ? LN : false, 2, 4><<<grid, w2 * 64, lds2, s>>>(GEMV_ARGS(p));
            WM_HIP(hipGetLastError());
            return WM_OK;
        }
        if (w2 >= 4 && p.B > 1)
            dec_gemv_kernel<TWO ? SPW : 6, 1, 1, TWO ? EPI : DE_RESID, TWO ? LN : false, 2, 4><<<grid, w2 * 64, lds2, s>>>(GEMV_ARGS(p));
        else
            dec_gemv_kernel<TWO ? SPW : 6, 1, 1, TWO ? EPI : DE_RESID, TWO ? LN : false, 2><<<grid, w2 * 64, lds2, s>>>(GEMV_ARGS(p));
        WM_HIP(hipGetLastError());
        return WM_OK;
    }
    constexpr bool RESID = !LN && EPI == DE_RESID;
    const bool split = RESID && p.B > 1 && tn == 1 && nblk * 4 <= nw;
    if (split && RESID) {
        const size_t ldsr = (size_t)nw * nblk * 1024 + (size_t)nw * 32 * 4;
        if (nblk == 1) dec_gemv_kernel<SPW, 1, 1, RESID ? EPI : DE_RESID, RESID ? LN : false, 1, 4><<<grid, nw * 64, ldsr, s>>>(GEMV_ARGS(p));
        else if (nblk == 2 && SPW <= 8) dec_gemv_kernel<SPW <= 8 ? SPW : 2, 1, 2, RESID ? EPI : DE_RESID, RESID ? LN : false, 1, 4><<<grid, nw * 64, ldsr, s>>>(GEMV_ARGS(p));
        else { wm_set_error("dec_gemv: unsupported row-split shape (nblk %d, spw %d)", nblk, SPW); return WM_ERR_INVALID; }
        WM_HIP(hipGetLastError());
        return WM_OK;
    }
    const size_t lds = (size_t)nw * tn * nblk * 1024 + (size_t)nw * 32 * 4;
    const int th = nw * 64;
    constexpr bool WIDE = LN && (EPI == DE_QKV || EPI == DE_GELU || EPI == DE_LOGITS) && SPW <= 6;
    if (tn == 1 && nblk == 1) dec_gemv_kernel<SPW, 1, 1, EPI, LN><<<grid, th, lds, s>>>(GEMV_ARGS(p));
    else if (tn == 1 && nblk == 2 && SPW <= 8) dec_gemv_kernel<SPW <= 8 ? SPW : 2, 1, 2, EPI, LN><<<grid, th, lds, s>>>(GEMV_ARGS(p));
    else if (tn == 2 && nblk == 1 && WIDE && EPI == DE_LOGITS) dec_gemv_kernel<WIDE ? SPW : 2, 2, 1, WIDE ? EPI : DE_LOGITS, LN><<<grid, th, lds, s>>>(GEMV_ARGS(p));
    else if (tn == 4 && nblk == 1 && WIDE && EPI == DE_LOGITS) dec_gemv_kernel<WIDE ? SPW : 2, 4, 1, WIDE ? EPI : DE_LOGITS, LN><<<grid, th, lds, s>>>(GEMV_ARGS(p));
    else if (tn == 2 && nblk == 2 && WIDE) dec_gemv_kernel<WIDE ? SPW : 2, 2, 2, EPI, LN><<<grid, th, lds, s>>>(GEMV_ARGS(p));
    else if (tn == 4 && nblk == 2 && WIDE) dec_gemv_kernel<WIDE ? SPW : 2, 4, 2, EPI, LN><<<grid, th, lds, s>>>(GEMV_ARGS(p));
    else { wm_set_error("dec_gemv: unsupported launch shape (tn %d, nblk %d, spw %d)", tn, nblk, SPW); return WM_ERR_INVALID; }
    WM_HIP(hipGetLastError());
    return WM_OK;
}

template <int EPI, bool LN>
int launch_gemv(wm_ctx *ctx, const DecGemvDev &p, int spw, int tn, int nblk, int nw, int grid, int ppw) {
    switch (spw) {
        case 2: return launch_gemv_shape<2, EPI, LN>(ctx, p, tn, nblk, nw, grid, ppw);
        case 4: return launch_gemv_shape<4, EPI, LN>(ctx, p, tn, nblk, nw, grid, ppw);
        case 5: return launch_gemv_shape<5, EPI, LN>(ctx, p, tn, nblk, nw, grid, ppw);
        case 6: return launch_gemv_shape<6, EPI, LN>(ctx, p, tn, nblk, nw, grid, ppw);
        case 8: return launch_gemv_shape<8, EPI, LN>(ctx, p, tn, nblk, nw, grid, ppw);
        case 10: return launch_gemv_shape<10, EPI, LN>(ctx, p, tn, nblk, nw, grid, ppw);
        case 12: return launch_gemv_shape<12, EPI, LN>(ctx, p, tn, nblk, nw, grid, ppw);
        default: wm_set_error("dec_gemv: unsupported k-steps per wave %d", spw); return WM_ERR_INVALID;
    }
}

}

int wm_dec_gemv_split(int K, int *spw) {
    const int steps = K / 32;
    for (int nw = steps >= 96 ? 16 : 8; nw >= 1; --nw) {
        if (steps % nw) continue;
        const int s = steps / nw;
        if (s == 2 || s == 4 || s == 5 || s == 6 || s == 8 || s == 10 || s == 12) {
            if (spw) *spw = s;
            return nw;
        }
    }
    return 0;
}

static bool pf_enabled(int B) { return B <= g_wm_tuning.prefetch_max_b; }

static void pick_shape(int epi, bool ln, int spw, int nw, int B, int n_tiles, int n_cus, int *tn, int *nblk) {
    const int env_tn = g_wm_tuning.gemv_tn, env_nb = g_wm_tuning.gemv_nblk;
    const int blocks = (B + 15) / 16;
    *tn = 1;
    *nblk = 1;
    if (blocks < 2 && epi == DE_LOGITS && ln && spw <= 6) {
        *tn = (g_wm_tuning.logits_tn == 1 || g_wm_tuning.logits_tn == 2) ? g_wm_tuning.logits_tn : 4;
        return;
    }
    if (blocks < 2 || nw > 8 || spw > 8) return;
    *nblk = env_nb == 1 ? 1 : 2;
    const bool wide = ln && (epi == DE_QKV || epi == DE_GELU || epi == DE_LOGITS) && *nblk == 2 && spw <= 6;
    if (!wide) return;
    const int g = (blocks + 1) / 2;
    int best = 1, best_rounds = 1 << 30, best_wgs = 0;
    for (int t = 1; t <= 4; t *= 2) {
        const int wgs = ((n_tiles + t - 1) / t) * g;
        const int cap = n_cus * (t == 1 ? 2 : 1);
        const int rounds = (wgs + cap - 1) / cap;
        const int fill = n_cus * 3 / 4;
        const bool better = rounds < best_rounds || (rounds == best_rounds && best_wgs >= fill && wgs >= fill);
        if (better) { best = t; best_rounds = rounds; best_wgs = wgs; }
    }
    if (env_tn == 1 || env_tn == 2 || env_tn == 4) best = env_tn;
    *tn = best;
}

int wm_dec_gemv(wm_ctx *ctx, const DecGemvArgs &a) {
    WM_REQUIRE(a.B >= 1 && a.B <= WM_DEC_MAXB, WM_ERR_INVALID, "dec_gemv: B=%d out of range", a.B);
    WM_REQUIRE(a.K % 32 == 0, WM_ERR_INVALID, "dec_gemv: K=%d must be a multiple of 32", a.K);
    int spw = 0;
    const int nw = wm_dec_gemv_split(a.K, &spw);
    WM_REQUIRE(nw >= 1, WM_ERR_INVALID, "dec_gemv: K=%d cannot be split over the waves of a workgroup", a.K);
    const bool ln = a.c1 != nullptr;
    WM_REQUIRE(!ln || (a.stats_in && a.K % 64 == 0 && a.K / 16 <= 80), WM_ERR_INVALID,
               "dec_gemv: LayerNorm mode needs the producer's K/16 partial statistics (K a multiple of 64, <= 1280)");
    WM_REQUIRE(a.a != nullptr && a.W != nullptr, WM_ERR_INVALID, "dec_gemv: null operand");
    DecGemvDev p;
    memset(&p, 0, sizeof(p));
    p.B = a.B; p.N = a.N; p.K = a.K;
    p.W = a.W; p.c1 = a.c1; p.c2 = a.c2; p.a = a.a;
    p.stats_in = a.stats_in; p.stats_parts = a.K / 16; p.stats_out = a.stats_out;
    p.mean_in = a.mean_in; p.mean_out = a.mean_out;
    p.stats_stride = 2L * (a.epi == DE_RESID ? a.N : a.K);
    p.out_f32 = a.out_f32; p.out_bf16 = a.out_bf16;
    p.kcache = a.kcache; p.vcache = a.vcache; p.pos_ptr = a.pos_ptr; p.n_ctx = a.n_ctx; p.n_head = a.n_head;
    p.ldo = a.ldo; p.tilemax = a.argmax; p.arg_first = a.arg_first; p.arg_last = a.arg_last;
    p.mask = a.mask; p.mask_words = a.mask_words; p.mask_first_pos = a.mask_first_pos;
    p.ts = a.ts;
    p.n_tiles = (a.N + 15) / 16;
    int tn = 1, nblk = 1;
    pick_shape(a.epi, ln, spw, nw, a.B, p.n_tiles, ctx->n_cus, &tn, &nblk);
    p.bgroups = ((a.B + 15) / 16 + nblk - 1) / nblk;
    const bool no_ppw = g_wm_tuning.gemv_no_ppw2 != 0;
    const int ppw = (!no_ppw && !ln && a.epi == DE_RESID && nw == 16 && a.B > 16 && spw >= 6 && spw <= 10 && tn == 1 &&
                     nblk == 1) ? 2 : 1;
    if (ppw == 2) {
        const int blocks = (a.B + 15) / 16;
        const int knob = g_wm_tuning.gemv_ppw2_nblk;
        const bool two = knob ? knob == 2 : (p.n_tiles * blocks > ctx->n_cus && p.n_tiles * ((blocks + 1) / 2) <= ctx->n_cus);
        if (two) {
            nblk = 2;
            p.bgroups = (blocks + 1) / 2;
        }
    }
    p.n_tg = (p.n_tiles + tn - 1) / tn;
    p.n_tg_pad = p.bgroups > 1 ? (p.n_tg + 7) / 8 * 8 : p.n_tg;
    int grid = p.n_tg_pad * p.bgroups;
    if (pf_enabled(a.B) && a.pf_ptr && a.pf_rows >= 16 && grid % 8 == 0) {
        p.pf_ptr = (const char *)a.pf_ptr;
        p.pf_tile_bytes = 16L * a.pf_k * 2;
        p.pf_tiles = a.pf_rows / 16;
        p.pf_head_major = a.pf_head_major;
        grid += a.pf_head_major ? 32 * (a.pf_head_major / a.B + 2) : p.pf_tiles;
    }
    switch (a.epi * 2 + (ln ? 1 : 0)) {
        case DE_QKV * 2 + 1: {
            WmProfScope ps(&ctx->prof, "dec_gemv_ln_qkv", ctx->stream);
            return launch_gemv<DE_QKV, true>(ctx, p, spw, tn, nblk, nw, grid, ppw);
        }
        case DE_Q * 2 + 1: {
            WmProfScope ps(&ctx->prof, "dec_gemv_ln_q", ctx->stream);
            return launch_gemv<DE_Q, true>(ctx, p, spw, tn, nblk, nw, grid, ppw);
        }
        case DE_GELU * 2 + 1: {
            WmProfScope ps(&ctx->prof, "dec_gemv_ln_fc1", ctx->stream);
            return launch_gemv<DE_GELU, true>(ctx, p, spw, tn, nblk, nw, grid, ppw);
        }
        case DE_LOGITS * 2 + 1: {
            WmProfScope ps(&ctx->prof, "dec_gemv_ln_logits", ctx->stream);
            return launch_gemv<DE_LOGITS, true>(ctx, p, spw, tn, nblk, nw, grid, ppw);
        }
        case DE_RESID * 2: {
            WmProfScope ps(&ctx->prof, a.K > a.N ? "dec_gemv_fc2" : "dec_gemv_attn_out", ctx->stream);
            return launch_gemv<DE_RESID, false>(ctx, p, spw, tn, nblk, nw, grid, ppw);
        }
        case DE_Q * 2: {
            WmProfScope ps(&ctx->prof, "dec_gemv_plain", ctx->stream);
            return launch_gemv<DE_Q, false>(ctx, p, spw, tn, nblk, nw, grid, ppw);
        }
        default:
            wm_set_error("dec_gemv: unsupported (epilogue %d, LayerNorm %d) pair", a.epi, (int)ln);
            return WM_ERR_INVALID;
    }
}

int wm_ln_fold(wm_ctx *ctx, const bf16_t *W, const float *g, const float *beta, const float *bias, int N, int K,
               bf16_t *Wf, float *c1, float *c2) {
    const int npad = (N + 15) / 16 * 16;
    ln_fold_kernel<<<npad, 256, 0, ctx->stream>>>(W, g, beta, bias, N, K, Wf, c1, c2);
    WM_HIP(hipGetLastError());
    return WM_OK;
}

int wm_dec_embed(wm_ctx *ctx, const int *seq, const int *pos_ptr, int B, const bf16_t *emb, const float *pemb,
                 int d, float *x, bf16_t *xb, float *stats_out, float *mean_buf) {
    WmProfScope ps(&ctx->prof, "dec_embed", ctx->stream);
    dec_embed_kernel<<<B, 256, 0, ctx->stream>>>(seq, pos_ptr, B, emb, pemb, d, x, xb, stats_out, mean_buf);
    WM_HIP(hipGetLastError());
    return WM_OK;
}

int wm_dec_attn_splits(int B, int H) {
    const int bh = B * H;
    const int thr = g_wm_tuning.xattn_split_below;
    if (bh >= thr) return 1;
    int ns = 2;
    while (ns < 8 && bh * ns < 192) ns *= 2;
    return ns;
}

int wm_dec_attention(wm_ctx *ctx, const float *q, const bf16_t *kc, const bf16_t *vc, int B, int H,
                     int T_stride, int n_keys, const int *pos_ptr, int nsplit, float *part, bf16_t *att,
                     bool cross, const bf16_t *pf_ptr, int pf_rows, int pf_k, const int *live_rows, const int *n_live,
                     bool short_lived) {
    WM_REQUIRE(nsplit == 1 || nsplit == 2 || nsplit == 4 || nsplit == 8, WM_ERR_INVALID,
               "dec_attention: nsplit %d is not 1, 2, 4 or 8", nsplit);
    WM_REQUIRE(T_stride <= ATT_MAXK && n_keys <= ATT_MAXK, WM_ERR_INVALID,
               "dec_attention: more than %d keys", ATT_MAXK);
    WM_REQUIRE(nsplit == 1 || part != nullptr, WM_ERR_INVALID, "dec_attention: split launch without a partials buffer");
    WM_REQUIRE(H >= 1 && H <= 255 && B * H < 65536, WM_ERR_INVALID, "dec_attention: %d heads x %d rows do not fit the packed arguments", H, B);
    WM_REQUIRE((!live_rows && !n_live) || n_live == live_rows + WM_DEC_MAXB, WM_ERR_INVALID, "dec_attention: the live count must follow the live rows");
    {
        WmProfScope ps(&ctx->prof, cross ? "dec_attn_cross" : "dec_attn_self", ctx->stream);
        const int cap_cus = g_wm_tuning.xattn_wgs > 0 && g_wm_tuning.xattn_wgs < ctx->n_cus ? g_wm_tuning.xattn_wgs : ctx->n_cus;
        const int cap = short_lived ? (1 << 30) : cap_cus;
        int n_wg = B * H;
        if (n_wg > cap) {
            const int rounds = (n_wg + cap - 1) / cap;
            n_wg = (n_wg + rounds - 1) / rounds;
        }
        int gx = n_wg;
        long tile_bytes = 0;
        if (pf_enabled(B) && pf_ptr && nsplit == 1 && gx % 8 == 0 && pf_rows >= 16) {
            tile_bytes = 16L * pf_k * 2;
            gx += pf_rows / 16;
        }
        const bool no_flat = g_wm_tuning.xattn_no_flat != 0;
        if (nsplit > 1 && !no_flat) {
            const int units = B * H * 8;
            int wpw = (units + 255) / 256;
            wpw = wpw < 1 ? 1 : (wpw > 4 ? 4 : wpw);
            const int g = (units + wpw - 1) / wpw;
            const AttnCold cold = {att, part, nullptr, 0};
            const unsigned pA = (unsigned)H | (8u << 8) | ((unsigned)wpw << 16), pB = (unsigned)T_stride | ((unsigned)n_keys << 16);
            const unsigned pC = (unsigned)(B * H) | ((unsigned)g << 16);
            WM_REQUIRE(g < 65536, WM_ERR_INVALID, "dec_attention: flat grid too large");
            if (g_wm_tuning.xattn_no_deep)
                dec_xrows_attn_kernel<8, 4, WM_XATTN_NT><<<g, wpw * 64, 0, ctx->stream>>>(
                    q, kc, vc, pos_ptr, live_rows, pA, pB, pC, cold);
            else if ((size_t)B * H * T_stride * 64 * 2 * 2 <= (size_t)3200 * 1024)
                dec_rows_attn_kernel<8, 4, false, true><<<g, wpw * 64, 0, ctx->stream>>>(
                    q, kc, vc, pos_ptr, live_rows, pA, pB, pC, cold);
            else
                dec_rows_attn_kernel<8, 4, WM_XATTN_NT, true><<<g, wpw * 64, 0, ctx->stream>>>(
                    q, kc, vc, pos_ptr, live_rows, pA, pB, pC, cold);
        } else {
            dim3 grid(gx, nsplit);
            const int lds_pad = g_wm_tuning.xattn_lds_pad;
            static std::atomic<int> pad_set[64];
            if (lds_pad > pad_set[ctx->device & 63].load(std::memory_order_acquire)) {
                WM_HIP(hipFuncSetAttribute((const void *)dec_xrows_attn_kernel<8, 4, WM_XATTN_NT>,
                                           hipFuncAttributeMaxDynamicSharedMemorySize, lds_pad));
                pad_set[ctx->device & 63].store(lds_pad, std::memory_order_release);
            }
            const AttnCold cold = {att, part, (const char *)pf_ptr, tile_bytes};
            const unsigned pA = (unsigned)H | ((unsigned)nsplit << 8), pB = (unsigned)T_stride | ((unsigned)n_keys << 16);
            const unsigned pC = (unsigned)(B * H) | ((unsigned)n_wg << 16);
            dec_xrows_attn_kernel<8, 4, WM_XATTN_NT><<<grid, (8 / nsplit) * 64, nsplit == 1 ? lds_pad : 0, ctx->stream>>>(
                q, kc, vc, pos_ptr, live_rows, pA, pB, pC, cold);
        }
        WM_HIP(hipGetLastError());
    }
    if (nsplit > 1) {
        WmProfScope ps(&ctx->prof, "dec_attn_combine", ctx->stream);
        dec_attn_combine_kernel<8><<<B * H, 64, 0, ctx->stream>>>(part, H, H * 64, att);
        WM_HIP(hipGetLastError());
    }
    return WM_OK;
}

bool wm_dec_xattn_fq_applies(int B, int H, int K, bool short_lived) {
    if (!g_wm_tuning.xattn_fuse_q || short_lived) return false;
    const int pairs = B * H;
    if (pairs < g_wm_tuning.xattn_split_below || pairs > 256 || K != H * 64) return false;
    int spw = 0;
    const int nw = wm_dec_gemv_split(K, &spw);
    return nw >= 1 && nw <= 8 && (spw == 2 || spw == 4 || spw == 5 || spw == 6);
}

int wm_dec_xattn_fq(wm_ctx *ctx, const DecGemvArgs &qa, const bf16_t *kc, const bf16_t *vc, int B, int H, int T_stride,
                    int n_keys, bf16_t *att, const int *live_rows, const int *n_live, const bf16_t *pf_ptr, int pf_rows, int pf_k) {
    WM_REQUIRE(qa.c1 && qa.stats_in && qa.N == qa.K && qa.K == H * 64, WM_ERR_INVALID, "xattn_fq: not a LayerNorm-folded d x d query projection");
    WM_REQUIRE(H >= 1 && H <= 255 && B >= 1 && B <= WM_DEC_MAXB && T_stride <= ATT_MAXK && n_keys >= 1 && n_keys <= ATT_MAXK,
               WM_ERR_INVALID, "xattn_fq: bad geometry");
    WM_REQUIRE((!live_rows && !n_live) || n_live == live_rows + WM_DEC_MAXB, WM_ERR_INVALID, "xattn_fq: the live count must follow the live rows");
    int spw = 0;
    const int nw = wm_dec_gemv_split(qa.K, &spw);
    WM_REQUIRE(nw >= 1 && nw <= 8, WM_ERR_INVALID, "xattn_fq: K split over more than 8 waves");
    WmProfScope ps(&ctx->prof, "dec_attn_cross_fq", ctx->stream);
    FqCold cold;
    cold.c1 = qa.c1; cold.c2 = qa.c2; cold.stats_in = qa.stats_in; cold.mean_in = qa.mean_in; cold.mean_out = qa.mean_out;
    cold.att = att; cold.stats_stride = 2L * qa.K; cold.K = qa.K; cold.N = qa.N;
    const unsigned pA = (unsigned)H | ((unsigned)B << 8), pB = (unsigned)T_stride | ((unsigned)n_keys << 16);
    int grid = 8 * ((H * B + 7) / 8);
    cold.n_wg = grid; cold.pf_ptr = nullptr; cold.pf_tile_bytes = 0;
    if (pf_enabled(B) && pf_ptr && pf_rows >= 16) {
        cold.pf_ptr = (const char *)pf_ptr;
        cold.pf_tile_bytes = 16L * pf_k * 2;
        grid += pf_rows / 16;
    }
    const size_t lds = ((size_t)nw * 1024 + 128 + 64) * sizeof(float);
    hipStream_t s = ctx->stream;
    switch (spw) {
        case 2: dec_xattn_fq_kernel<2, WM_XATTN_NT><<<grid, 512, lds, s>>>(qa.W, qa.a, kc, vc, live_rows, pA, pB, qa.K, cold); break;
        case 4: dec_xattn_fq_kernel<4, WM_XATTN_NT><<<grid, 512, lds, s>>>(qa.W, qa.a, kc, vc, live_rows, pA, pB, qa.K, cold); break;
        case 5: dec_xattn_fq_kernel<5, WM_XATTN_NT><<<grid, 512, lds, s>>>(qa.W, qa.a, kc, vc, live_rows, pA, pB, qa.K, cold); break;
        case 6: dec_xattn_fq_kernel<6, WM_XATTN_NT><<<grid, 512, lds, s>>>(qa.W, qa.a, kc, vc, live_rows, pA, pB, qa.K, cold); break;
        default: wm_set_error("xattn_fq: unsupported k-steps per wave %d", spw); return WM_ERR_INVALID;
    }
    WM_HIP(hipGetLastError());
    return WM_OK;
}

int wm_dec_self_attention(wm_ctx *ctx, const float *q, const bf16_t *kc, const bf16_t *vc, int B, int H, int T_stride,
                          int n_keys, const int *pos_ptr, bf16_t *att, const bf16_t *pf_ptr, int pf_rows, int pf_k,
                          const int *live_rows, const int *n_live) {
    WM_REQUIRE(T_stride <= ATT_MAXK && n_keys <= ATT_MAXK && (pos_ptr || n_keys >= 1), WM_ERR_INVALID,
               "dec_self_attention: 1..%d keys", ATT_MAXK);
    WM_REQUIRE(H >= 1 && H <= 255 && B * H < 65536, WM_ERR_INVALID, "dec_self_attention: %d heads x %d rows do not fit the packed arguments", H, B);
    WM_REQUIRE((!live_rows && !n_live) || n_live == live_rows + WM_DEC_MAXB, WM_ERR_INVALID, "dec_self_attention: the live count must follow the live rows");
    WmProfScope ps(&ctx->prof, "dec_attn_self", ctx->stream);
    int gx = B * H;
    long tile_bytes = 0;
    if (pf_enabled(B) && pf_ptr && gx % 8 == 0 && pf_rows >= 16) {
        tile_bytes = 16L * pf_k * 2;
        gx += pf_rows / 16;
    }
    const AttnCold cold = {att, nullptr, (const char *)pf_ptr, tile_bytes};
    const unsigned pA = (unsigned)H | (1u << 8), pB = (unsigned)T_stride | ((unsigned)n_keys << 16);
    const unsigned pC = (unsigned)(B * H) | ((unsigned)(B * H) << 16);
    dec_rows_attn_kernel<4, 4, false><<<gx, 256, 0, ctx->stream>>>(q, kc, vc, pos_ptr, live_rows, pA, pB, pC, cold);
    WM_HIP(hipGetLastError());
    return WM_OK;
}

int wm_argmax_embed(wm_ctx *ctx, const unsigned long long *tilemax, int n_tiles, int B, int *seq, int *pos_ptr,
                    int n_prompt, int *result, int arg_first, const bf16_t *emb, const float *pemb, int d, int n_ctx,
                    float *x, bf16_t *xb, float *stats_out, const WmTsDev *ts, int *arrive, int fallback_tok,
                    float *mean_buf, const WmStopDev *stop) {
    WmProfScope ps(&ctx->prof, "argmax_embed", ctx->stream);
    WmTsDev t;
    memset(&t, 0, sizeof(t));
    if (ts) t = *ts;
    WmStopDev sp;
    memset(&sp, 0, sizeof(sp));
    if (stop) sp = *stop;
    int rpw = (arrive && (B > 16 || !sp.done)) ? 1 : 16;
    if (arrive && g_wm_tuning.argmax_rows_per_wg >= 1 && g_wm_tuning.argmax_rows_per_wg <= 16) rpw = g_wm_tuning.argmax_rows_per_wg;
    const int grid = arrive ? (B + rpw - 1) / rpw : 1;
    WM_REQUIRE(grid == 1 || B <= rpw * grid, WM_ERR_INVALID, "argmax_embed: bad grid");
    WM_REQUIRE(arrive || B <= 16, WM_ERR_INVALID, "argmax_embed: more than 16 rows need the arrival counter");
    argmax_embed_kernel<<<grid, 1024, 0, ctx->stream>>>(tilemax, n_tiles, B, seq, pos_ptr, n_prompt, result, arg_first,
                                                        emb, pemb, d, n_ctx, x, xb, stats_out, t, arrive, fallback_tok,
                                                        mean_buf, sp, rpw);
    WM_HIP(hipGetLastError());
    return WM_OK;
}

int wm_stop_init(wm_ctx *ctx, const WmStopDev &stop, int B) {
    dec_live_init_kernel<<<1, WM_DEC_MAXB, 0, ctx->stream>>>(stop, B);
    WM_HIP(hipGetLastError());
    return WM_OK;
}

namespace {
__global__ void ts_init_kernel(WmTsDev ts, int B) {
    const int b = threadIdx.x;
    if (b >= B) return;
    const int hi = ts.max_initial >= 0 && ts.ts_begin + ts.max_initial + 1 < ts.n_vocab ? ts.ts_begin + ts.max_initial + 1
                                                                                         : ts.n_vocab;
    *(int4 *)(ts.rng + b * 4) = make_int4(0, 0, ts.ts_begin, hi);
    *(int4 *)(ts.hist + b * 4) = make_int4(0, 0, 1, -1);
}
}

int wm_ts_init(wm_ctx *ctx, const WmTsDev &ts, int B) {
    ts_init_kernel<<<1, WM_DEC_MAXB, 0, ctx->stream>>>(ts, B);
    WM_HIP(hipGetLastError());
    return WM_OK;
}

namespace {
__global__ __launch_bounds__(128) void range_softmax_kernel(const float *__restrict__ logits, long ldo, int first, int n,
                                                            float *__restrict__ probs) {
    __shared__ float red[2];
    const int b = blockIdx.x, tid = threadIdx.x;
    const float *row = logits + (long)b * ldo + first;
    float m = -1e30f;
    for (int i = tid; i < n; i += 128) m = fmaxf(m, row[i]);
#pragma unroll
    for (int o = 32; o > 0; o >>= 1) m = fmaxf(m, __shfl_xor(m, o));
    if ((tid & 63) == 0) red[tid >> 6] = m;
    __syncthreads();
    m = fmaxf(red[0], red[1]);
    __syncthreads();
    float s = 0.f;
    for (int i = tid; i < n; i += 128) s += __expf(row[i] - m);
#pragma unroll
    for (int o = 32; o > 0; o >>= 1) s += __shfl_xor(s, o);
    if ((tid & 63) == 0) red[tid >> 6] = s;
    __syncthreads();
    const float inv = 1.0f / (red[0] + red[1]);
    for (int i = tid; i < n; i += 128) probs[(long)b * n + i] = __expf(row[i] - m) * inv;
}
}

int wm_range_softmax(wm_ctx *ctx, const float *logits, long ldo, int B, int first, int n, float *probs) {
    range_softmax_kernel<<<B, 128, 0, ctx->stream>>>(logits, ldo, first, n, probs);
    WM_HIP(hipGetLastError());
    return WM_OK;
}

int wm_fill_synthetic(wm_ctx *ctx, const WmTensor &t, uint32_t seed, int tensor_id, float gain) {
    if (t.kind == 4) return WM_OK;
    const unsigned key = [&] {
        unsigned x = seed + (unsigned)tensor_id * 0x9E3779B9u;
        x ^= x >> 16; x *= 0x7feb352du; x ^= x >> 15; x *= 0x846ca68bu; x ^= x >> 16;
        return x;
    }();
    const double std = (t.kind == 0) ? 0.02 : 0.01;
    const float scale = (float)(std / 37837.22659);
    const int grid = (int)((t.n_elems + 255) / 256 < 16384 ? (t.n_elems + 255) / 256 : 16384);
    synth_fill_kernel<<<grid, 256, 0, ctx->stream>>>(t.ptr, t.is_bf16 ? 1 : 0, t.n_elems, key, scale, t.layout,
                                                     t.conv_c, t.conv_kpad, t.kind, gain);
    WM_HIP(hipGetLastError());
    return WM_OK;
}

namespace {
__global__ void trivial_kernel(int *p) {
    if (p && threadIdx.x == 0 && blockIdx.x == 0) *p = *p + 1;
}
}
int wm_launch_trivial(wm_ctx *ctx, int *p, int grid) {
    trivial_kernel<<<grid, 64, 0, ctx->stream>>>(p);
    WM_HIP(hipGetLastError());
    return WM_OK;
}

namespace {
__global__ void spin_kernel(int *p, int cycles) {
    const long long t0 = wall_clock64();
    while (wall_clock64() - t0 < cycles) __builtin_amdgcn_s_sleep(2);
    if (p && threadIdx.x == 0 && blockIdx.x == 0) *p = *p + 1;
}
}
int wm_launch_spin(hipStream_t s, int *p, int grid, int cycles) {
    spin_kernel<<<grid, 256, 0, s>>>(p, cycles);
    return hipGetLastError() == hipSuccess ? WM_OK : WM_ERR_HIP;
}
```

openai-whisper-coreml_amd/csrc/model.cpp:

```cpp
#include "model.h"

#include <math.h>
#include <string.h>

static inline bf16_t host_f2bf(float f) {
    uint32_t u;
    memcpy(&u, &f, 4);
    u += 0x7fffu + ((u >> 16) & 1u);
    return (bf16_t)(u >> 16);
}
static inline float host_bf2f(bf16_t h) {
    uint32_t u = (uint32_t)h << 16;
    float f;
    memcpy(&f, &u, 4);
    return f;
}

static int dalloc(WmModel *m, void **p, size_t bytes, hipStream_t s) {
    bytes = (bytes + 255) & ~(size_t)255;
    WM_HIP(hipMalloc(p, bytes + 256));
    WM_HIP(hipMemsetAsync(*p, 0, bytes + 256, s));
    m->allocs.push_back(*p);
    return WM_OK;
}
template <typename T>
static int dalloc_t(WmModel *m, T **p, size_t n, hipStream_t s) {
    return dalloc(m, (void **)p, n * sizeof(T), s);
}

static void reg(WmModel *m, const std::string &name, void *ptr, bool is_bf16, size_t n, int kind,
                int layout = WL_PLAIN, int conv_c = 0, int kpad = 0) {
    WmTensor t;
    t.name = name; t.ptr = ptr; t.is_bf16 = is_bf16; t.n_elems = n; t.kind = kind;
    t.layout = layout; t.conv_c = conv_c; t.conv_kpad = kpad;
    m->index[name] = (int)m->tensors.size();
    m->tensors.push_back(t);
}

static int alloc_decode_buffers(WmModel *m, hipStream_t s) {
    const wm_dims &D = m->dims;
    const int d = D.n_text_state;
    WM_TRY(dalloc_t(m, &m->dx, (size_t)WM_DEC_MAXB * d, s));
    WM_TRY(dalloc_t(m, &m->dxb, (size_t)WM_DEC_MAXB * d, s));
    WM_TRY(dalloc_t(m, &m->dmean, (size_t)2 * WM_DEC_MAXB, s));
    WM_TRY(dalloc_t(m, &m->dq, (size_t)WM_DEC_MAXB * d, s));
    WM_TRY(dalloc_t(m, &m->dpart, (size_t)WM_DEC_MAXB * D.n_text_head * WM_MAXSPLIT * 66, s));
    WM_TRY(dalloc_t(m, &m->datt, (size_t)WM_DEC_MAXB * d, s));
    WM_TRY(dalloc_t(m, &m->dstats, (size_t)(WM_DEC_MAXB / 16) * (d / 16) * 16 * 2, s));
    WM_TRY(dalloc_t(m, &m->dhid, (size_t)WM_DEC_MAXB * 4 * d, s));
    WM_TRY(dalloc_t(m, &m->dlogits, (size_t)WM_DEC_MAXB * m->vpad, s));
    WM_TRY(dalloc_t(m, &m->dargmax, (size_t)WM_DEC_MAXB * (m->vpad / 16), s));
    WM_TRY(dalloc_t(m, &m->dresult, WM_DEC_MAXB, s));
    WM_TRY(dalloc_t(m, &m->dseq, (size_t)WM_DEC_MAXB * (D.n_text_ctx + 1), s));
    WM_TRY(dalloc_t(m, &m->dpos, 4, s));
    WM_TRY(dalloc_t(m, &m->darrive, 4, s));
    WM_TRY(dalloc_t(m, &m->ddone, WM_DEC_MAXB, s));
    WM_TRY(dalloc_t(m, &m->dbudget, WM_DEC_MAXB, s));
    WM_TRY(dalloc_t(m, &m->dlive, WM_DEC_MAXB + 4, s));
    m->dnlive = m->dlive + WM_DEC_MAXB;
    if (!m->h_nlive) WM_HIP(hipHostMalloc((void **)&m->h_nlive, WM_NLIVE_RING * sizeof(int), hipHostMallocDefault));
    WM_TRY(dalloc_t(m, &m->dts_rng, (size_t)WM_DEC_MAXB * 4, s));
    WM_TRY(dalloc_t(m, &m->dts_hist, (size_t)WM_DEC_MAXB * 4, s));
    WM_TRY(dalloc_t(m, &m->dts_key, (size_t)WM_DEC_MAXB * (m->vpad / 16), s));
    WM_TRY(dalloc_t(m, &m->dts_lse, (size_t)WM_DEC_MAXB * (m->vpad / 16) * 2, s));
    WM_TRY(dalloc_t(m, &m->dmask, (size_t)2 * (m->vpad / 32), s));
    WM_HIP(hipMemsetAsync(m->dmask, 0, (size_t)2 * (m->vpad / 32) * 4, s));
    return WM_OK;
}

WmStopDev wm_model_stop_dev(const WmModel *m) {
    WmStopDev t;
    memset(&t, 0, sizeof(t));
    if (!m->stop_on) return t;
    t.done = m->ddone; t.budget = m->budget_on ? m->dbudget : nullptr; t.live_rows = m->dlive; t.n_live = m->dnlive;
    t.eot = m->stop_eot;
    t.pad_tok = m->stop_eot >= 0 ? m->stop_eot : 0;
    return t;
}

void wm_model_drop_graphs(WmModel *m) {
    for (WmModel::GraphSet &g : m->graph_sets) g.destroy();
    m->graph_sets.clear();
    m->graph_cur = -1;
    m->lid_graph.destroy();
}

WmTsDev wm_model_ts_dev(const WmModel *m) {
    WmTsDev t;
    memset(&t, 0, sizeof(t));
    if (!m->ts_on) return t;
    t.rng = m->dts_rng; t.hist = m->dts_hist; t.key_ts = m->dts_key; t.lse = m->dts_lse;
    t.ts_begin = m->ts_begin; t.eot = m->ts_eot; t.n_vocab = m->dims.n_vocab; t.max_initial = m->ts_max_initial;
    return t;
}

int wm_model_set_timestamp_rules(wm_ctx *ctx, int enable, int32_t ts_begin, int32_t eot, int32_t max_initial) {
    WmModel *m = ctx->model;
    WM_REQUIRE(m, WM_ERR_STATE, "context has no model");
    if (enable) {
        const int V = m->dims.n_vocab;
        WM_REQUIRE(ts_begin > 0 && ts_begin < V && eot >= 0 && eot < ts_begin, WM_ERR_INVALID,
                   "timestamp rules: need 0 <= eot < timestamp_begin < n_vocab (%d)", V);
        if (!m->mask_host.empty())
            WM_REQUIRE(!((m->mask_host[eot >> 5] >> (eot & 31)) & 1u), WM_ERR_INVALID,
                       "timestamp rules: <|endoftext|> (%d) is in the suppress list", eot);
        if (m->ts_begin != ts_begin || m->ts_eot != eot || m->ts_max_initial != max_initial) {
            wm_model_drop_graphs(m);
        }
        m->ts_begin = ts_begin; m->ts_eot = eot; m->ts_max_initial = max_initial;
    }
    m->ts_on = enable != 0;
    return WM_OK;
}

int wm_model_set_suppress(wm_ctx *ctx, const int32_t *ids, int n, const int32_t *first_ids, int n_first) {
    WmModel *m = ctx->model;
    WM_REQUIRE(m, WM_ERR_STATE, "context has no model");
    WM_REQUIRE(n >= 0 && n_first >= 0 && (n == 0 || ids) && (n_first == 0 || first_ids), WM_ERR_INVALID,
               "set_suppress: bad list");
    const int words = m->vpad / 32, V = m->dims.n_vocab;
    std::vector<unsigned> bits((size_t)2 * words, 0u);
    for (int i = 0; i < n; ++i) {
        WM_REQUIRE(ids[i] >= 0 && ids[i] < V, WM_ERR_INVALID, "set_suppress: token %d outside [0, %d)", ids[i], V);
        bits[ids[i] >> 5] |= 1u << (ids[i] & 31);
    }
    for (int i = 0; i < words; ++i) bits[words + i] = bits[i];
    for (int i = 0; i < n_first; ++i) {
        WM_REQUIRE(first_ids[i] >= 0 && first_ids[i] < V, WM_ERR_INVALID, "set_suppress: token %d outside [0, %d)",
                   first_ids[i], V);
        bits[words + (first_ids[i] >> 5)] |= 1u << (first_ids[i] & 31);
    }
    size_t live0 = 0, live1 = 0;
    for (int t = 0; t < V; ++t) {
        live0 += !((bits[t >> 5] >> (t & 31)) & 1u);
        live1 += !((bits[words + (t >> 5)] >> (t & 31)) & 1u);
    }
    WM_REQUIRE(live0 > 0 && live1 > 0, WM_ERR_INVALID, "set_suppress: every token would be suppressed");
    if (m->ts_on)
        WM_REQUIRE(!((bits[m->ts_eot >> 5] >> (m->ts_eot & 31)) & 1u), WM_ERR_INVALID,
                   "set_suppress: <|endoftext|> (%d) must stay admissible while the timestamp rules are on", m->ts_eot);
    m->mask_host.assign(bits.begin(), bits.begin() + words);
    WM_HIP(hipMemcpyAsync(m->dmask, bits.data(), bits.size() * 4, hipMemcpyHostToDevice, ctx->stream));
    WM_HIP(hipStreamSynchronize(ctx->stream));
    m->mask_on = (n + n_first) > 0;
    return WM_OK;
}

int wm_model_create(wm_ctx *ctx, const wm_dims *dims) {
    const wm_dims &D = *dims;
    WM_REQUIRE(D.n_mels == 80 || D.n_mels == 128, WM_ERR_INVALID, "n_mels must be 80 or 128");
    WM_REQUIRE(D.n_audio_ctx == 1500, WM_ERR_INVALID, "n_audio_ctx must be 1500 (30 s chunks)");
    WM_REQUIRE(D.n_audio_state == D.n_text_state, WM_ERR_INVALID, "audio/text widths must match");
    WM_REQUIRE(D.n_audio_state % 64 == 0 && D.n_audio_state <= 1280 && D.n_audio_state >= 64,
               WM_ERR_INVALID, "model width must be a multiple of 64 in [64, 1280]");
    WM_REQUIRE(D.n_audio_head * 64 == D.n_audio_state && D.n_text_head * 64 == D.n_text_state,
               WM_ERR_INVALID, "head_dim must be 64 (Whisper uses 64 at every size)");
    WM_REQUIRE(D.n_text_ctx >= 8 && D.n_text_ctx <= 448 && D.n_vocab >= 16, WM_ERR_INVALID, "bad text dims");
    WM_REQUIRE(D.n_audio_layer >= 1 && D.n_text_layer >= 1, WM_ERR_INVALID, "bad layer counts");
    WM_REQUIRE(wm_dec_gemv_split(D.n_text_state, nullptr) > 0 && wm_dec_gemv_split(4 * D.n_text_state, nullptr) > 0,
               WM_ERR_INVALID, "model width %d: the decode GEMV cannot split K = d / 4d over its waves", D.n_text_state);
    WmModel *m = new WmModel();
    ctx->model = m;
    m->dims = D;
    const int d = D.n_audio_state;
    hipStream_t s = ctx->stream;
    m->k1pad = ((3 * D.n_mels + 63) / 64) * 64;
    m->vpad = ((D.n_vocab + 15) / 16) * 16;

    WM_TRY(dalloc_t(m, &m->conv1_w, (size_t)d * m->k1pad, s));
    WM_TRY(dalloc_t(m, &m->conv1_b, d, s));
    WM_TRY(dalloc_t(m, &m->conv2_w, (size_t)d * 3 * d, s));
    WM_TRY(dalloc_t(m, &m->conv2_b, d, s));
    WM_TRY(dalloc_t(m, &m->enc_pos, (size_t)D.n_audio_ctx * d, s));
    reg(m, "encoder.conv1.weight", m->conv1_w, true, (size_t)d * D.n_mels * 3, 0, WL_CONV, D.n_mels, m->k1pad);
    reg(m, "encoder.conv1.bias", m->conv1_b, false, d, 1);
    reg(m, "encoder.conv2.weight", m->conv2_w, true, (size_t)d * d * 3, 0, WL_CONV, d, 3 * d);
    reg(m, "encoder.conv2.bias", m->conv2_b, false, d, 1);
    reg(m, "encoder.positional_embedding", m->enc_pos, false, (size_t)D.n_audio_ctx * d, 4);

    auto attn_regs = [&](const std::string &p, bf16_t *wq, float *bq, bf16_t *wk, bf16_t *wv, float *bv,
                         bf16_t *wo, float *bo, float *lg, float *lb, const char *a, int lq, int lkv, int lo) {
        const size_t dd = (size_t)d * d;
        reg(m, p + "." + a + ".query.weight", wq, true, dd, 0, lq, 0, d);
        reg(m, p + "." + a + ".query.bias", bq, false, d, 1);
        reg(m, p + "." + a + ".key.weight", wk, true, dd, 0, lkv, 0, d);
        reg(m, p + "." + a + ".value.weight", wv, true, dd, 0, lkv, 0, d);
        reg(m, p + "." + a + ".value.bias", bv, false, d, 1);
        reg(m, p + "." + a + ".out.weight", wo, true, dd, 0, lo, 0, d);
        reg(m, p + "." + a + ".out.bias", bo, false, d, 1);
        reg(m, p + "." + a + "_ln.weight", lg, false, d, 2);
        reg(m, p + "." + a + "_ln.bias", lb, false, d, 3);
    };
    auto mlp_regs = [&](const std::string &p, bf16_t *w1, float *b1, bf16_t *w2, float *b2, float *lg, float *lb,
                        int lay) {
        reg(m, p + ".mlp.0.weight", w1, true, (size_t)4 * d * d, 0, lay, 0, d);
        reg(m, p + ".mlp.0.bias", b1, false, 4 * d, 1);
        reg(m, p + ".mlp.2.weight", w2, true, (size_t)4 * d * d, 0, lay, 0, 4 * d);
        reg(m, p + ".mlp.2.bias", b2, false, d, 1);
        reg(m, p + ".mlp_ln.weight", lg, false, d, 2);
        reg(m, p + ".mlp_ln.bias", lb, false, d, 3);
    };

    m->enc.resize(D.n_audio_layer);
    for (int i = 0; i < D.n_audio_layer; ++i) {
        EncLayerW &L = m->enc[i];
        WM_TRY(dalloc_t(m, &L.ln1_g, d, s)); WM_TRY(dalloc_t(m, &L.ln1_b, d, s));
        WM_TRY(dalloc_t(m, &L.wqkv, (size_t)3 * d * d, s)); WM_TRY(dalloc_t(m, &L.bqkv, 3 * d, s));
        WM_TRY(dalloc_t(m, &L.wo, (size_t)d * d, s)); WM_TRY(dalloc_t(m, &L.bo, d, s));
        WM_TRY(dalloc_t(m, &L.ln2_g, d, s)); WM_TRY(dalloc_t(m, &L.ln2_b, d, s));
        WM_TRY(dalloc_t(m, &L.w1, (size_t)4 * d * d, s)); WM_TRY(dalloc_t(m, &L.b1, 4 * d, s));
        WM_TRY(dalloc_t(m, &L.w2, (size_t)4 * d * d, s)); WM_TRY(dalloc_t(m, &L.b2, d, s));
        const std::string p = "encoder.blocks." + std::to_string(i);
        attn_regs(p, L.wqkv, L.bqkv, L.wqkv + (size_t)d * d, L.wqkv + (size_t)2 * d * d, L.bqkv + 2 * d, L.wo,
                  L.bo, L.ln1_g, L.ln1_b, "attn", WL_PLAIN, WL_PLAIN, WL_PLAIN);
        mlp_regs(p, L.w1, L.b1, L.w2, L.b2, L.ln2_g, L.ln2_b, WL_PLAIN);
    }
    WM_TRY(dalloc_t(m, &m->ln_post_g, d, s)); WM_TRY(dalloc_t(m, &m->ln_post_b, d, s));
    reg(m, "encoder.ln_post.weight", m->ln_post_g, false, d, 2);
    reg(m, "encoder.ln_post.bias", m->ln_post_b, false, d, 3);

    WM_TRY(dalloc_t(m, &m->tok_emb, (size_t)m->vpad * d, s));
    WM_TRY(dalloc_t(m, &m->dec_pos, (size_t)D.n_text_ctx * d, s));
    reg(m, "decoder.token_embedding.weight", m->tok_emb, true, (size_t)D.n_vocab * d, 0, WL_TILED, 0, d);
    reg(m, "decoder.positional_embedding", m->dec_pos, false, (size_t)D.n_text_ctx * d, 0);
    m->dec.resize(D.n_text_layer);
    for (int i = 0; i < D.n_text_layer; ++i) {
        DecLayerW &L = m->dec[i];
        WM_TRY(dalloc_t(m, &L.ln1_g, d, s)); WM_TRY(dalloc_t(m, &L.ln1_b, d, s));
        WM_TRY(dalloc_t(m, &L.wqkv, (size_t)3 * d * d, s)); WM_TRY(dalloc_t(m, &L.bqkv, 3 * d, s));
        WM_TRY(dalloc_t(m, &L.wo, (size_t)d * d, s)); WM_TRY(dalloc_t(m, &L.bo, d, s));
        WM_TRY(dalloc_t(m, &L.lnx_g, d, s)); WM_TRY(dalloc_t(m, &L.lnx_b, d, s));
        WM_TRY(dalloc_t(m, &L.wxq, (size_t)d * d, s)); WM_TRY(dalloc_t(m, &L.bxq, d, s));
        WM_TRY(dalloc_t(m, &L.wxkv, (size_t)2 * d * d, s)); WM_TRY(dalloc_t(m, &L.bxkv, 2 * d, s));
        WM_TRY(dalloc_t(m, &L.wxo, (size_t)d * d, s)); WM_TRY(dalloc_t(m, &L.bxo, d, s));
        WM_TRY(dalloc_t(m, &L.ln2_g, d, s)); WM_TRY(dalloc_t(m, &L.ln2_b, d, s));
        WM_TRY(dalloc_t(m, &L.w1, (size_t)4 * d * d, s)); WM_TRY(dalloc_t(m, &L.b1, 4 * d, s));
        WM_TRY(dalloc_t(m, &L.w2, (size_t)4 * d * d, s)); WM_TRY(dalloc_t(m, &L.b2, d, s));
        WM_TRY(dalloc_t(m, &L.wqkv_f, (size_t)3 * d * d, s)); WM_TRY(dalloc_t(m, &L.wxq_f, (size_t)d * d, s));
        WM_TRY(dalloc_t(m, &L.w1_f, (size_t)4 * d * d, s));
        WM_TRY(dalloc_t(m, &L.qkv_c1, 3 * d, s)); WM_TRY(dalloc_t(m, &L.qkv_c2, 3 * d, s));
        WM_TRY(dalloc_t(m, &L.xq_c1, d, s)); WM_TRY(dalloc_t(m, &L.xq_c2, d, s));
        WM_TRY(dalloc_t(m, &L.fc1_c1, 4 * d, s)); WM_TRY(dalloc_t(m, &L.fc1_c2, 4 * d, s));
        const std::string p = "decoder.blocks." + std::to_string(i);
        attn_regs(p, L.wqkv, L.bqkv, L.wqkv + (size_t)d * d, L.wqkv + (size_t)2 * d * d, L.bqkv + 2 * d, L.wo,
                  L.bo, L.ln1_g, L.ln1_b, "attn", WL_TILED, WL_TILED, WL_TILED);
        attn_regs(p, L.wxq, L.bxq, L.wxkv, L.wxkv + (size_t)d * d, L.bxkv + d, L.wxo, L.bxo, L.lnx_g, L.lnx_b,
                  "cross_attn", WL_TILED, WL_PLAIN, WL_TILED);
        mlp_regs(p, L.w1, L.b1, L.w2, L.b2, L.ln2_g, L.ln2_b, WL_TILED);
    }
    WM_TRY(dalloc_t(m, &m->ln_g, d, s)); WM_TRY(dalloc_t(m, &m->ln_b, d, s));
    reg(m, "decoder.ln.weight", m->ln_g, false, d, 2);
    reg(m, "decoder.ln.bias", m->ln_b, false, d, 3);
    WM_TRY(dalloc_t(m, &m->emb_f, (size_t)m->vpad * d, s));
    WM_TRY(dalloc_t(m, &m->logit_c1, m->vpad, s)); WM_TRY(dalloc_t(m, &m->logit_c2, m->vpad, s));

    WM_TRY(alloc_decode_buffers(m, s));
    WM_HIP(hipStreamSynchronize(s));
    return WM_OK;
}

int wm_model_clone(wm_ctx *child, const wm_ctx *parent) {
    const WmModel *pm = parent->model;
    WM_REQUIRE(pm && pm->finalized, WM_ERR_STATE, "clone: the parent's weights must be finalised");
    WmModel *m = new WmModel();
    child->model = m;
    m->dims = pm->dims; m->finalized = true; m->k1pad = pm->k1pad; m->vpad = pm->vpad;
    m->conv1_w = pm->conv1_w; m->conv2_w = pm->conv2_w; m->conv1_b = pm->conv1_b; m->conv2_b = pm->conv2_b;
    m->enc_pos = pm->enc_pos; m->enc = pm->enc; m->ln_post_g = pm->ln_post_g; m->ln_post_b = pm->ln_post_b;
    m->tok_emb = pm->tok_emb; m->dec_pos = pm->dec_pos; m->dec = pm->dec; m->ln_g = pm->ln_g; m->ln_b = pm->ln_b;
    m->emb_f = pm->emb_f; m->logit_c1 = pm->logit_c1; m->logit_c2 = pm->logit_c2;
    m->tensors = pm->tensors; m->index = pm->index;
    m->shares_weights = true;
    WM_TRY(alloc_decode_buffers(m, child->stream));
    WM_HIP(hipMemcpyAsync(m->dmask, pm->dmask, (size_t)2 * (m->vpad / 32) * 4, hipMemcpyDeviceToDevice, child->stream));
    m->mask_on = pm->mask_on; m->mask_host = pm->mask_host;
    m->ts_on = pm->ts_on; m->ts_begin = pm->ts_begin; m->ts_eot = pm->ts_eot; m->ts_max_initial = pm->ts_max_initial;
    WM_HIP(hipStreamSynchronize(child->stream));
    return WM_OK;
}

void wm_model_destroy(wm_ctx *ctx) {
    WmModel *m = ctx->model;
    if (!m) return;
    wm_model_drop_graphs(m);
    if (m->h_nlive) (void)hipHostFree(m->h_nlive);
    for (void *p : m->allocs) (void)hipFree(p);
    if (m->pcm_stage) (void)hipFree(m->pcm_stage);
    if (m->io_stage) (void)hipFree(m->io_stage);
    delete m;
    ctx->model = nullptr;
}

int wm_model_set_tensor(wm_ctx *ctx, const char *name, const float *data, size_t n) {
    WmModel *m = ctx->model;
    WM_REQUIRE(m, WM_ERR_STATE, "context has no model");
    WM_REQUIRE(!m->shares_weights, WM_ERR_STATE, "a cloned context shares its parent's weights: set them on the parent");
    WM_REQUIRE(name && data, WM_ERR_INVALID, "null name / data");
    auto it = m->index.find(name);
    WM_REQUIRE(it != m->index.end(), WM_ERR_INVALID, "unknown tensor '%s'", name);
    WmTensor &t = m->tensors[it->second];
    WM_REQUIRE(n == t.n_elems, WM_ERR_INVALID, "tensor '%s': %zu elements given, %zu expected", name, n, t.n_elems);
    if (!t.is_bf16) {
        WM_HIP(hipMemcpy(t.ptr, data, n * sizeof(float), hipMemcpyHostToDevice));
    } else if (t.layout == WL_PLAIN) {
        std::vector<bf16_t> tmp(n);
        for (size_t i = 0; i < n; ++i) tmp[i] = host_f2bf(data[i]);
        WM_HIP(hipMemcpy(t.ptr, tmp.data(), n * sizeof(bf16_t), hipMemcpyHostToDevice));
    } else if (t.layout == WL_TILED) {
        const size_t K = (size_t)t.conv_kpad, N = n / K;
        const size_t Np = (N + 15) / 16 * 16;
        std::vector<bf16_t> tmp(Np * K, 0);
        for (size_t r = 0; r < N; ++r)
            for (size_t k = 0; k < K; ++k) tmp[wm_tiled_offset(r, k, K)] = host_f2bf(data[r * K + k]);
        WM_HIP(hipMemcpy(t.ptr, tmp.data(), tmp.size() * sizeof(bf16_t), hipMemcpyHostToDevice));
    } else {
        const size_t per = (size_t)t.conv_c * 3, O = n / per;
        std::vector<bf16_t> tmp(O * t.conv_kpad, 0);
        for (size_t o = 0; o < O; ++o)
            for (int c = 0; c < t.conv_c; ++c)
                for (int tap = 0; tap < 3; ++tap)
                    tmp[o * t.conv_kpad + (size_t)tap * t.conv_c + c] = host_f2bf(data[o * per + (size_t)c * 3 + tap]);
        WM_HIP(hipMemcpy(t.ptr, tmp.data(), tmp.size() * sizeof(bf16_t), hipMemcpyHostToDevice));
    }
    t.set = true;
    m->finalized = false;
    return WM_OK;
}

int wm_model_get_tensor(wm_ctx *ctx, const char *name, float *data, size_t n) {
    WmModel *m = ctx->model;
    WM_REQUIRE(m, WM_ERR_STATE, "context has no model");
    WM_REQUIRE(name && data, WM_ERR_INVALID, "null name / data");
    auto it = m->index.find(name);
    WM_REQUIRE(it != m->index.end(), WM_ERR_INVALID, "unknown tensor '%s'", name);
    const WmTensor &t = m->tensors[it->second];
    WM_REQUIRE(n == t.n_elems, WM_ERR_INVALID, "tensor '%s': %zu elements asked, %zu stored", name, n, t.n_elems);
    WM_HIP(hipStreamSynchronize(ctx->stream));
    if (!t.is_bf16) {
        WM_HIP(hipMemcpy(data, t.ptr, n * sizeof(float), hipMemcpyDeviceToHost));
    } else if (t.layout == WL_PLAIN) {
        std::vector<bf16_t> tmp(n);
        WM_HIP(hipMemcpy(tmp.data(), t.ptr, n * sizeof(bf16_t), hipMemcpyDeviceToHost));
        for (size_t i = 0; i < n; ++i) data[i] = host_bf2f(tmp[i]);
    } else if (t.layout == WL_TILED) {
        const size_t K = (size_t)t.conv_kpad, N = n / K;
        const size_t Np = (N + 15) / 16 * 16;
        std::vector<bf16_t> tmp(Np * K);
        WM_HIP(hipMemcpy(tmp.data(), t.ptr, tmp.size() * sizeof(bf16_t), hipMemcpyDeviceToHost));
        for (size_t r = 0; r < N; ++r)
            for (size_t k = 0; k < K; ++k) data[r * K + k] = host_bf2f(tmp[wm_tiled_offset(r, k, K)]);
    } else {
        const size_t per = (size_t)t.conv_c * 3, O = n / per;
        std::vector<bf16_t> tmp(O * t.conv_kpad);
        WM_HIP(hipMemcpy(tmp.data(), t.ptr, tmp.size() * sizeof(bf16_t), hipMemcpyDeviceToHost));
        for (size_t o = 0; o < O; ++o)
            for (int c = 0; c < t.conv_c; ++c)
                for (int tap = 0; tap < 3; ++tap)
                    data[o * per + (size_t)c * 3 + tap] = host_bf2f(tmp[o * t.conv_kpad + (size_t)tap * t.conv_c + c]);
    }
    return WM_OK;
}

int wm_model_init_synthetic(wm_ctx *ctx, uint64_t seed, float matrix_gain) {
    WmModel *m = ctx->model;
    WM_REQUIRE(m, WM_ERR_STATE, "context has no model");
    WM_REQUIRE(!m->shares_weights, WM_ERR_STATE, "a cloned context shares its parent's weights");
    const int d = m->dims.n_audio_state;
    for (size_t i = 0; i < m->tensors.size(); ++i) {
        WmTensor &t = m->tensors[i];
        if (t.kind == 4) {
            const int L = m->dims.n_audio_ctx, half = d / 2;
            std::vector<float> pe((size_t)L * d);
            const double inc = log(10000.0) / (half - 1);
            for (int p = 0; p < L; ++p)
                for (int j = 0; j < half; ++j) {
                    const double a = (double)p * exp(-inc * j);
                    pe[(size_t)p * d + j] = (float)sin(a);
                    pe[(size_t)p * d + half + j] = (float)cos(a);
                }
            WM_HIP(hipMemcpy(t.ptr, pe.data(), pe.size() * sizeof(float), hipMemcpyHostToDevice));
        } else {
            const bool scaled = t.kind == 0 && t.name.find("positional") == std::string::npos;
            WM_TRY(wm_fill_synthetic(ctx, t, (uint32_t)(seed & 0xffffffffu), (int)i, scaled ? matrix_gain : 1.0f));
        }
        t.set = true;
    }
    WM_HIP(hipStreamSynchronize(ctx->stream));
    m->finalized = false;
    return WM_OK;
}

int wm_model_finalize(wm_ctx *ctx) {
    WmModel *m = ctx->model;
    WM_REQUIRE(m, WM_ERR_STATE, "context has no model");
    for (const WmTensor &t : m->tensors)
        WM_REQUIRE(t.set, WM_ERR_STATE, "tensor '%s' was never set", t.name.c_str());
    const int d = m->dims.n_text_state;
    for (DecLayerW &L : m->dec) {
        WM_TRY(wm_ln_fold(ctx, L.wqkv, L.ln1_g, L.ln1_b, L.bqkv, 3 * d, d, L.wqkv_f, L.qkv_c1, L.qkv_c2));
        WM_TRY(wm_ln_fold(ctx, L.wxq, L.lnx_g, L.lnx_b, L.bxq, d, d, L.wxq_f, L.xq_c1, L.xq_c2));
        WM_TRY(wm_ln_fold(ctx, L.w1, L.ln2_g, L.ln2_b, L.b1, 4 * d, d, L.w1_f, L.fc1_c1, L.fc1_c2));
    }
    WM_TRY(wm_ln_fold(ctx, m->tok_emb, m->ln_g, m->ln_b, nullptr, m->dims.n_vocab, d, m->emb_f, m->logit_c1, m->logit_c2));
    WM_HIP(hipStreamSynchronize(ctx->stream));
    m->finalized = true;
    return WM_OK;
}

int wm_model_reserve(wm_ctx *ctx, int B) {
    WmModel *m = ctx->model;
    WM_REQUIRE(m, WM_ERR_STATE, "context has no model");
    if (B <= m->cap_b) return WM_OK;
    WM_HIP(hipStreamSynchronize(ctx->stream));
    void *olds[] = {m->mel_t, m->h1p, m->x, m->xn, m->qk, m->vt, m->att, m->hid, m->xa_f32, m->mel_f32, m->xkv, m->skv};
    for (void *p : olds)
        if (p) {
            (void)hipFree(p);
            for (auto &a : m->allocs)
                if (a == p) a = nullptr;
        }
    const wm_dims &D = m->dims;
    const int d = D.n_audio_state, H = D.n_audio_head;
    const size_t M = (size_t)B * 1500;
    hipStream_t s = ctx->stream;
    WM_TRY(dalloc_t(m, &m->mel_t, (size_t)B * 3002 * D.n_mels, s));
    WM_TRY(dalloc_t(m, &m->h1p, (size_t)B * 3001 * d, s));
    WM_TRY(dalloc_t(m, &m->x, M * d, s));
    WM_TRY(dalloc_t(m, &m->xn, M * d, s));
    WM_TRY(dalloc_t(m, &m->qk, (M + 64) * 2 * d, s));
    WM_TRY(dalloc_t(m, &m->vt, (size_t)B * H * 64 * 1536, s));
    WM_TRY(dalloc_t(m, &m->att, M * d, s));
    WM_TRY(dalloc_t(m, &m->hid, M * 4 * d, s));
    WM_TRY(dalloc_t(m, &m->xa_f32, M * d, s));
    WM_TRY(dalloc_t(m, &m->mel_f32, (size_t)B * D.n_mels * WM_N_FRAMES, s));
    WM_TRY(dalloc_t(m, &m->xkv, (size_t)D.n_text_layer * 2 * B * H * 1500 * 64, s));
    const int Bd = B < WM_DEC_MAXB ? B : WM_DEC_MAXB;
    WM_TRY(dalloc_t(m, &m->skv, (size_t)D.n_text_layer * 2 * Bd * H * D.n_text_ctx * 64, s));
    m->cap_b = B;
    WM_HIP(hipStreamSynchronize(s));
    return WM_OK;
}

static GemmArgs plain_gemm(const bf16_t *A, int lda, const bf16_t *W, const float *bias, void *C, int ldc,
                           int M, int N, int K, int epi) {
    GemmArgs g;
    memset(&g, 0, sizeof(g));
    g.A = A; g.a_rpb = (long)M + 1; g.a_bstride = 0; g.a_rstride = lda;
    g.W = W; g.bias = bias; g.C = C;
    g.c_rpb = (long)M + 1; g.c_bstride = 0; g.c_rstride = ldc;
    g.M = M; g.N = N; g.K = K; g.epi = epi;
    return g;
}

int wm_model_encode_dev(wm_ctx *ctx, const float *d_mel, int B, float *d_xa_out) {
    WmModel *m = ctx->model;
    WM_REQUIRE(m && m->finalized, WM_ERR_STATE, "model weights not finalised (wm_finalize)");
    WM_REQUIRE(B >= 1, WM_ERR_INVALID, "B must be >= 1");
    WM_TRY(wm_model_reserve(ctx, B));
    const wm_dims &D = m->dims;
    const int d = D.n_audio_state, H = D.n_audio_head, S = 1500, C = D.n_mels;
    const int M = B * S;
    WM_TRY(wm_mel_to_time_major(ctx, d_mel, B, C, m->mel_t));
    {
        GemmArgs g;
        memset(&g, 0, sizeof(g));
        g.A = m->mel_t; g.a_rpb = 3000; g.a_bstride = 3002L * C; g.a_rstride = C;
        g.W = m->conv1_w; g.bias = m->conv1_b;
        g.C = m->h1p + d; g.c_rpb = 3000; g.c_bstride = 3001L * d; g.c_rstride = d;
        g.M = B * 3000; g.N = d; g.K = m->k1pad; g.epi = EPI_GELU_BF16;
        WM_TRY(wm_gemm(ctx, g));
    }
    {
        GemmArgs g;
        memset(&g, 0, sizeof(g));
        g.A = m->h1p; g.a_rpb = S; g.a_bstride = 3001L * d; g.a_rstride = 2L * d;
        g.W = m->conv2_w; g.bias = m->conv2_b;
        g.C = m->x; g.c_rpb = S; g.c_bstride = (long)S * d; g.c_rstride = d;
        g.M = M; g.N = d; g.K = 3 * d; g.epi = EPI_CONV2_F32; g.pos = m->enc_pos;
        WM_TRY(wm_gemm(ctx, g));
    }
    for (int i = 0; i < D.n_audio_layer; ++i) {
        const EncLayerW &L = m->enc[i];
        WM_TRY(wm_layernorm(ctx, m->x, L.ln1_g, L.ln1_b, M, d, m->xn, nullptr));
        GemmArgs g = plain_gemm(m->xn, d, L.wqkv, L.bqkv, m->qk, 2 * d, M, 3 * d, d, EPI_QKV_ENC);
        g.vt = m->vt; g.d_model = d; g.n_head = H; g.seq = S; g.seq_pad = 1536; g.batch = B;
        WM_TRY(wm_gemm(ctx, g));
        WM_TRY(wm_enc_attention(ctx, m->qk, m->vt, m->att, B, H, S, 1536, d));
        WM_TRY(wm_gemm(ctx, plain_gemm(m->att, d, L.wo, L.bo, m->x, d, M, d, d, EPI_RESID_F32)));
        WM_TRY(wm_layernorm(ctx, m->x, L.ln2_g, L.ln2_b, M, d, m->xn, nullptr));
        WM_TRY(wm_gemm(ctx, plain_gemm(m->xn, d, L.w1, L.b1, m->hid, 4 * d, M, 4 * d, d, EPI_GELU_BF16)));
        WM_TRY(wm_gemm(ctx, plain_gemm(m->hid, 4 * d, L.w2, L.b2, m->x, d, M, d, 4 * d, EPI_RESID_F32)));
    }
    WM_TRY(wm_layernorm(ctx, m->x, m->ln_post_g, m->ln_post_b, M, d, m->xn, d_xa_out ? d_xa_out : m->xa_f32));
    return WM_OK;
}

int wm_model_set_xa(wm_ctx *ctx, const float *d_xa, int B) {
    WmModel *m = ctx->model;
    WM_REQUIRE(m && m->finalized, WM_ERR_STATE, "model weights not finalised (wm_finalize)");
    WM_TRY(wm_model_reserve(ctx, B));
    return wm_f32_to_bf16(ctx, d_xa, m->xn, (size_t)B * 1500 * m->dims.n_audio_state);
}

int wm_model_cross_kv(wm_ctx *ctx, int B) {
    WmModel *m = ctx->model;
    const wm_dims &D = m->dims;
    const int d = D.n_text_state, H = D.n_text_head, S = 1500, M = B * S;
    for (int l = 0; l < D.n_text_layer; ++l) {
        const DecLayerW &L = m->dec[l];
        GemmArgs g = plain_gemm(m->xn, d, L.wxkv, L.bxkv, m->xkv + (size_t)l * 2 * B * H * S * 64, 0, M, 2 * d, d,
                                EPI_XKV);
        g.d_model = d; g.n_head = H; g.seq = S; g.batch = B;
        WM_TRY(wm_gemm(ctx, g));
    }
    return WM_OK;
}

int wm_model_decode_begin(wm_ctx *ctx, int B) {
    WmModel *m = ctx->model;
    WM_REQUIRE(m && m->finalized, WM_ERR_STATE, "model weights not finalised (wm_finalize)");
    WM_REQUIRE(B >= 1 && B <= WM_DEC_MAXB, WM_ERR_INVALID, "decode batch must be 1..%d", WM_DEC_MAXB);
    WM_HIP(hipMemsetAsync(m->darrive, 0, sizeof(int), ctx->stream));
    m->stop_on = false;
    m->xattn_shared = false;
    return WM_OK;
}

int wm_model_set_pos(wm_ctx *ctx, int pos) {
    WmModel *m = ctx->model;
    if (pos == 0) {
        WM_HIP(hipMemsetAsync(m->dpos, 0, sizeof(int), ctx->stream));
        return WM_OK;
    }
    WM_HIP(hipMemcpyAsync(m->dpos, &pos, sizeof(int), hipMemcpyHostToDevice, ctx->stream));
    WM_HIP(hipStreamSynchronize(ctx->stream));
    return WM_OK;
}

int wm_model_decode_step(wm_ctx *ctx, int B, bool want_logits, int arg_first, int arg_last, int mask_first_pos, bool use_ts) {
    WmModel *m = ctx->model;
    const wm_dims &D = m->dims;
    const int d = D.n_text_state, H = D.n_text_head, T = D.n_text_ctx, S = 1500;
    const int ns = wm_dec_attn_splits(B, H);
    const int xns = g_wm_tuning.xattn_splits > 0 ? g_wm_tuning.xattn_splits : ns;
    const int *live = m->stop_on ? m->dlive : nullptr, *nlive = m->stop_on ? m->dnlive : nullptr;
    int cur = 0;
    auto mean_buf = [&](int i) { return m->dmean + (size_t)i * WM_DEC_MAXB; };
    for (int l = 0; l < D.n_text_layer; ++l) {
        const DecLayerW &L = m->dec[l];
        bf16_t *kc = m->skv + (size_t)(l * 2 + 0) * B * H * T * 64;
        bf16_t *vc = m->skv + (size_t)(l * 2 + 1) * B * H * T * 64;
        const bf16_t *xk = m->xkv + (size_t)(l * 2 + 0) * B * H * S * 64;
        const bf16_t *xv = m->xkv + (size_t)(l * 2 + 1) * B * H * S * 64;
        DecGemvArgs a;
        memset(&a, 0, sizeof(a));
        a.epi = DE_QKV; a.B = B; a.N = 3 * d; a.K = d; a.W = L.wqkv_f; a.c1 = L.qkv_c1; a.c2 = L.qkv_c2;
        a.a = m->dxb; a.out_f32 = m->dq; a.kcache = kc; a.vcache = vc;
        a.stats_in = m->dstats;
        a.mean_in = mean_buf(cur); a.mean_out = mean_buf(cur ^ 1); cur ^= 1;
        a.pos_ptr = m->dpos; a.n_ctx = T; a.n_head = H;
        WM_TRY(wm_dec_gemv(ctx, a));
        WM_TRY(wm_dec_self_attention(ctx, m->dq, kc, vc, B, H, T, 0, m->dpos, m->datt, L.wo, d, d, live, nlive));
        memset(&a, 0, sizeof(a));
        a.epi = DE_RESID; a.B = B; a.N = d; a.K = d; a.W = L.wo; a.c2 = L.bo;
        a.a = m->datt; a.out_f32 = m->dx; a.out_bf16 = m->dxb; a.ldo = d; a.stats_out = m->dstats;
        a.mean_in = mean_buf(cur);
        a.pf_ptr = L.wxq_f; a.pf_rows = d; a.pf_k = d;
        const bool xshort = m->xattn_shared && !g_wm_tuning.xattn_never_short;
        const bool fuse_q = xns == 1 && wm_dec_xattn_fq_applies(B, H, d, xshort);
        a.pf_head_major = fuse_q ? (H * B + 7) / 8 : 0;
        WM_TRY(wm_dec_gemv(ctx, a));
        memset(&a, 0, sizeof(a));
        a.epi = DE_Q; a.B = B; a.N = d; a.K = d; a.W = L.wxq_f; a.c1 = L.xq_c1; a.c2 = L.xq_c2;
        a.a = m->dxb; a.out_f32 = m->dq; a.ldo = d;
        a.stats_in = m->dstats;
        a.mean_in = mean_buf(cur); a.mean_out = mean_buf(cur ^ 1); cur ^= 1;
        if (fuse_q) {
            WM_TRY(wm_dec_xattn_fq(ctx, a, xk, xv, B, H, S, S, m->datt, live, nlive, L.wxo, d, d));
        } else {
            WM_TRY(wm_dec_gemv(ctx, a));
            WM_TRY(wm_dec_attention(ctx, m->dq, xk, xv, B, H, S, S, nullptr, xns, m->dpart, m->datt, true, L.wxo, d, d, live, nlive, xshort));
        }
        memset(&a, 0, sizeof(a));
        a.epi = DE_RESID; a.B = B; a.N = d; a.K = d; a.W = L.wxo; a.c2 = L.bxo;
        a.a = m->datt; a.out_f32 = m->dx; a.out_bf16 = m->dxb; a.ldo = d; a.stats_out = m->dstats;
        a.mean_in = mean_buf(cur);
        a.pf_ptr = L.w1_f; a.pf_rows = 4 * d; a.pf_k = d;
        WM_TRY(wm_dec_gemv(ctx, a));
        memset(&a, 0, sizeof(a));
        a.epi = DE_GELU; a.B = B; a.N = 4 * d; a.K = d; a.W = L.w1_f; a.c1 = L.fc1_c1; a.c2 = L.fc1_c2;
        a.a = m->dxb; a.out_bf16 = m->dhid; a.ldo = 4 * d;
        a.stats_in = m->dstats;
        a.mean_in = mean_buf(cur); a.mean_out = mean_buf(cur ^ 1); cur ^= 1;
        a.pf_ptr = L.w2; a.pf_rows = d; a.pf_k = 4 * d;
        WM_TRY(wm_dec_gemv(ctx, a));
        memset(&a, 0, sizeof(a));
        a.epi = DE_RESID; a.B = B; a.N = d; a.K = 4 * d; a.W = L.w2; a.c2 = L.b2;
        a.a = m->dhid; a.out_f32 = m->dx; a.out_bf16 = m->dxb; a.ldo = d; a.stats_out = m->dstats;
        a.mean_in = mean_buf(cur);
        if (l + 1 < D.n_text_layer) { a.pf_ptr = m->dec[l + 1].wqkv_f; a.pf_rows = 3 * d; a.pf_k = d; }
        WM_TRY(wm_dec_gemv(ctx, a));
    }
    {
        DecGemvArgs a;
        memset(&a, 0, sizeof(a));
        a.epi = DE_LOGITS; a.B = B; a.N = D.n_vocab; a.K = d; a.W = m->emb_f; a.c1 = m->logit_c1; a.c2 = m->logit_c2;
        a.a = m->dxb; a.stats_in = m->dstats;
        a.mean_in = mean_buf(cur); a.mean_out = mean_buf(cur ^ 1);
        a.out_f32 = want_logits ? m->dlogits : nullptr; a.ldo = m->vpad;
        a.argmax = m->dargmax; a.arg_first = arg_first; a.arg_last = arg_last;
        if (mask_first_pos >= 0) {
            a.mask = m->dmask; a.mask_words = m->vpad / 32; a.mask_first_pos = mask_first_pos; a.pos_ptr = m->dpos;
        }
        if (use_ts) a.ts = wm_model_ts_dev(m);
        WM_TRY(wm_dec_gemv(ctx, a));
    }
    return WM_OK;
}

int wm_model_embed_first(wm_ctx *ctx, int B) {
    WmModel *m = ctx->model;
    return wm_dec_embed(ctx, m->dseq, m->dpos, B, m->tok_emb, m->dec_pos, m->dims.n_text_state, m->dx, m->dxb, m->dstats, m->dmean);
}

int wm_model_close_step(wm_ctx *ctx, int B, int n_prompt, bool write_seq, int *result, int arg_first, bool use_ts) {
    WmModel *m = ctx->model;
    const WmTsDev t = wm_model_ts_dev(m);
    const WmStopDev sp = wm_model_stop_dev(m);
    return wm_argmax_embed(ctx, m->dargmax, m->vpad / 16, B, write_seq ? m->dseq : nullptr, m->dpos, n_prompt, result,
                           arg_first, m->tok_emb, m->dec_pos, m->dims.n_text_state, m->dims.n_text_ctx, m->dx, m->dxb,
                           m->dstats, use_ts ? &t : nullptr, m->darrive, use_ts ? m->ts_eot : arg_first, m->dmean,
                           m->stop_on ? &sp : nullptr);
}
```

openai-whisper-coreml_amd/csrc/model.h:

```cpp
#pragma once
#include "wm_internal.h"

struct EncLayerW {
    float *ln1_g, *ln1_b;
    bf16_t *wqkv;
    float *bqkv;
    bf16_t *wo;
    float *bo;
    float *ln2_g, *ln2_b;
    bf16_t *w1;
    float *b1;
    bf16_t *w2;
    float *b2;
};
struct DecLayerW {
    float *ln1_g, *ln1_b;
    bf16_t *wqkv;
    float *bqkv;
    bf16_t *wo;
    float *bo;
    float *lnx_g, *lnx_b;
    bf16_t *wxq;
    float *bxq;
    bf16_t *wxkv;
    float *bxkv;
    bf16_t *wxo;
    float *bxo;
    float *ln2_g, *ln2_b;
    bf16_t *w1;
    float *b1;
    bf16_t *w2;
    float *b2;
    bf16_t *wqkv_f, *wxq_f, *w1_f;
    float *qkv_c1, *qkv_c2, *xq_c1, *xq_c2, *fc1_c1, *fc1_c2;
};

enum WmLayout { WL_PLAIN = 0, WL_CONV = 1, WL_TILED = 2 };
__host__ __device__ static inline size_t wm_tiled_offset(size_t n, size_t k, size_t K) {
    return (((n >> 4) * (K >> 5) + (k >> 5)) * 64 + (n & 15) + 16 * ((k & 31) >> 3)) * 8 + (k & 7);
}
struct WmTensor {
    std::string name;
    void *ptr = nullptr;
    bool is_bf16 = false;
    size_t n_elems = 0;
    int layout = WL_PLAIN;
    int conv_c = 0, conv_kpad = 0;
    int kind = 0;
    bool set = false;
};

struct WmTsDev {
    int *rng;
    int *hist;
    unsigned long long *key_ts;
    float *lse;
    int ts_begin, eot, n_vocab, max_initial;
};

struct WmStopDev {
    int *done;
    const int *budget;
    int *live_rows;
    int *n_live;
    int eot, pad_tok;
};

struct WmModel {
    wm_dims dims;
    bool finalized = false;
    bool shares_weights = false;
    int k1pad = 0;
    int vpad = 0;
    bf16_t *conv1_w = nullptr, *conv2_w = nullptr;
    float *conv1_b = nullptr, *conv2_b = nullptr, *enc_pos = nullptr;
    std::vector<EncLayerW> enc;
    float *ln_post_g = nullptr, *ln_post_b = nullptr;
    bf16_t *tok_emb = nullptr;
    float *dec_pos = nullptr;
    std::vector<DecLayerW> dec;
    float *ln_g = nullptr, *ln_b = nullptr;
    bf16_t *emb_f = nullptr;
    float *logit_c1 = nullptr, *logit_c2 = nullptr;
    std::vector<void *> allocs;
    std::vector<WmTensor> tensors;
    std::map<std::string, int> index;
    int cap_b = 0;
    bf16_t *mel_t = nullptr;
    bf16_t *h1p = nullptr;
    float *x = nullptr;
    bf16_t *xn = nullptr;
    bf16_t *qk = nullptr;
    bf16_t *vt = nullptr;
    bf16_t *att = nullptr;
    bf16_t *hid = nullptr;
    float *xa_f32 = nullptr;
    float *mel_f32 = nullptr;
    bf16_t *xkv = nullptr;
    bf16_t *skv = nullptr;
    float *dx = nullptr;
    bf16_t *dxb = nullptr;
    float *dmean = nullptr;
    float *dq = nullptr;
    float *dpart = nullptr;
    float *dstats = nullptr;
    bf16_t *datt = nullptr;
    bf16_t *dhid = nullptr;
    float *dlogits = nullptr;
    unsigned long long *dargmax = nullptr;
    int *dresult = nullptr;
    int *dseq = nullptr;
    int *dpos = nullptr;
    int *darrive = nullptr;
    int *ddone = nullptr, *dbudget = nullptr, *dlive = nullptr, *dnlive = nullptr;
    int *h_nlive = nullptr;
    bool xattn_shared = false;
    bool stop_on = false;
    bool budget_on = false;
    int stop_eot = -1;
    std::vector<int32_t> budget_host;
    struct GraphSet {
        int B = 0, n_prompt = 0, cap_b = 0, mask = 0, stop_key = 0;
        int burst[2] = {0, 0};
        hipGraph_t g1[2] = {nullptr, nullptr}, gk[2] = {nullptr, nullptr};
        hipGraphExec_t e1[2] = {nullptr, nullptr}, ek[2] = {nullptr, nullptr};
        void destroy() {
            for (int i = 0; i < 2; ++i) {
                if (e1[i]) (void)hipGraphExecDestroy(e1[i]);
                if (g1[i]) (void)hipGraphDestroy(g1[i]);
                if (ek[i]) (void)hipGraphExecDestroy(ek[i]);
                if (gk[i]) (void)hipGraphDestroy(gk[i]);
                e1[i] = ek[i] = nullptr;
                g1[i] = gk[i] = nullptr;
            }
        }
        unsigned long stamp = 0;
    };
    struct LidGraph {
        int B = 0, cap_b = 0, first = 0, last = 0, logits = 0;
        hipGraph_t g = nullptr;
        hipGraphExec_t e = nullptr;
        void destroy() {
            if (e) (void)hipGraphExecDestroy(e);
            if (g) (void)hipGraphDestroy(g);
            e = nullptr; g = nullptr; B = 0;
        }
    } lid_graph;
    std::vector<int32_t> lid_host;
    static constexpr int kMaxGraphSets = 4;
    std::vector<GraphSet> graph_sets;
    int graph_cur = -1;
    unsigned long graph_clock = 0;
    unsigned *dmask = nullptr;
    bool mask_on = false;
    std::vector<unsigned> mask_host;
    bool ts_on = false;
    int ts_begin = 0, ts_eot = 0, ts_max_initial = -1;
    int *dts_rng = nullptr, *dts_hist = nullptr;
    unsigned long long *dts_key = nullptr;
    float *dts_lse = nullptr;
    void *pcm_stage = nullptr;
    size_t pcm_stage_bytes = 0;
    float *io_stage = nullptr;
    size_t io_stage_bytes = 0;
};

int wm_model_create(wm_ctx *ctx, const wm_dims *dims);
void wm_model_destroy(wm_ctx *ctx);
int wm_model_clone(wm_ctx *child, const wm_ctx *parent);
int wm_model_reserve(wm_ctx *ctx, int B);
int wm_model_set_tensor(wm_ctx *ctx, const char *name, const float *data, size_t n);
int wm_model_get_tensor(wm_ctx *ctx, const char *name, float *data, size_t n);
int wm_model_init_synthetic(wm_ctx *ctx, uint64_t seed, float matrix_gain);
int wm_model_finalize(wm_ctx *ctx);
int wm_model_encode_dev(wm_ctx *ctx, const float *d_mel, int B, float *d_xa_out );
int wm_model_cross_kv(wm_ctx *ctx, int B);
int wm_model_set_xa(wm_ctx *ctx, const float *d_xa, int B);
int wm_model_decode_begin(wm_ctx *ctx, int B);
int wm_model_decode_step(wm_ctx *ctx, int B, bool want_logits, int arg_first, int arg_last, int mask_first_pos = -1,
                         bool use_ts = false);
WmTsDev wm_model_ts_dev(const WmModel *m);
int wm_model_set_timestamp_rules(wm_ctx *ctx, int enable, int32_t ts_begin, int32_t eot, int32_t max_initial);
int wm_model_set_suppress(wm_ctx *ctx, const int32_t *ids, int n, const int32_t *first_ids, int n_first);
int wm_model_embed_first(wm_ctx *ctx, int B);
int wm_model_close_step(wm_ctx *ctx, int B, int n_prompt, bool write_seq, int *result, int arg_first, bool use_ts = false);
WmStopDev wm_model_stop_dev(const WmModel *m);
void wm_model_drop_graphs(WmModel *m);
int wm_model_set_pos(wm_ctx *ctx, int pos);

enum GemmEpi {
    EPI_BIAS_BF16 = 0,
    EPI_GELU_BF16 = 1,
    EPI_RESID_F32 = 2,
    EPI_CONV2_F32 = 3,
    EPI_QKV_ENC = 4,
    EPI_XKV = 5,
    EPI_F32 = 6
};
#define WM_ENC_QSCALE (0.125f * 1.44269504088896340736f)
__host__ __device__ static inline unsigned wm_att_vt_pos(unsigned s) { return (s & ~12u) | ((s & 4u) << 1) | ((s & 8u) >> 1); }
struct GemmArgs {
    const bf16_t *A;
    long a_rpb, a_bstride, a_rstride;
    const bf16_t *W;
    const float *bias;
    void *C;
    long c_rpb, c_bstride, c_rstride;
    int M, N, K;
    int epi;
    const float *pos;
    bf16_t *vt;
    int d_model, n_head, seq, seq_pad, batch;
};
int wm_gemm(wm_ctx *ctx, const GemmArgs &g);

int wm_layernorm(wm_ctx *ctx, const float *x, const float *g, const float *b, int rows, int d,
                 bf16_t *out_bf16 , float *out_f32 );
int wm_mel_to_time_major(wm_ctx *ctx, const float *mel, int B, int n_mels, bf16_t *mel_t);
int wm_f32_to_bf16(wm_ctx *ctx, const float *in, bf16_t *out, size_t n);
int wm_enc_attention(wm_ctx *ctx, const bf16_t *qk, const bf16_t *vt, bf16_t *att, int B, int H,
                     int S, int S_pad, int d);

constexpr int WM_DEC_MAXB = 128;
constexpr int WM_NLIVE_RING = 16;
constexpr int WM_MAXSPLIT = 8;
enum DecEpi { DE_QKV = 0, DE_Q = 1, DE_RESID = 2, DE_GELU = 3, DE_LOGITS = 4 };
struct DecGemvArgs {
    int epi;
    int B, N, K;
    const bf16_t *W;
    const float *c1;
    const float *c2;
    const bf16_t *a;
    const float *stats_in;
    int stats_parts;
    float *stats_out;
    const float *mean_in;
    float *mean_out;
    float *out_f32;
    bf16_t *out_bf16;
    bf16_t *kcache, *vcache;
    const int *pos_ptr;
    int n_ctx, n_head;
    long ldo;
    unsigned long long *argmax;
    int arg_first, arg_last;
    const unsigned *mask;
    int mask_words, mask_first_pos;
    WmTsDev ts;
    const bf16_t *pf_ptr;
    int pf_rows, pf_k;
    int pf_head_major;
};
int wm_dec_gemv(wm_ctx *ctx, const DecGemvArgs &a);
bool wm_dec_xattn_fq_applies(int B, int H, int K, bool short_lived);
int wm_dec_xattn_fq(wm_ctx *ctx, const DecGemvArgs &qa, const bf16_t *kc, const bf16_t *vc, int B, int H, int T_stride,
                    int n_keys, bf16_t *att, const int *live_rows, const int *n_live, const bf16_t *pf_ptr = nullptr,
                    int pf_rows = 0, int pf_k = 0);
int wm_dec_gemv_split(int K, int *spw);
int wm_ln_fold(wm_ctx *ctx, const bf16_t *W, const float *g, const float *beta, const float *bias , int N,
               int K, bf16_t *Wf, float *c1, float *c2);
int wm_dec_embed(wm_ctx *ctx, const int *seq, const int *pos_ptr, int B, const bf16_t *emb, const float *pemb,
                 int d, float *x, bf16_t *xb, float *stats_out, float *mean_buf );
int wm_dec_attn_splits(int B, int H);
int wm_dec_attention(wm_ctx *ctx, const float *q, const bf16_t *kc, const bf16_t *vc, int B, int H,
                     int T_stride, int n_keys, const int *pos_ptr, int nsplit, float *part, bf16_t *att,
                     bool cross, const bf16_t *pf_ptr = nullptr, int pf_rows = 0, int pf_k = 0,
                     const int *live_rows = nullptr, const int *n_live = nullptr, bool short_lived = false);
int wm_dec_self_attention(wm_ctx *ctx, const float *q, const bf16_t *kc, const bf16_t *vc, int B, int H, int T_stride,
                          int n_keys, const int *pos_ptr, bf16_t *att, const bf16_t *pf_ptr = nullptr, int pf_rows = 0,
                          int pf_k = 0, const int *live_rows = nullptr, const int *n_live = nullptr);
int wm_argmax_embed(wm_ctx *ctx, const unsigned long long *tilemax, int n_tiles, int B, int *seq, int *pos_ptr,
                    int n_prompt, int *result, int arg_first, const bf16_t *emb, const float *pemb, int d, int n_ctx,
                    float *x, bf16_t *xb, float *stats_out, const WmTsDev *ts = nullptr, int *arrive = nullptr,
                    int fallback_tok = 0, float *mean_buf = nullptr, const WmStopDev *stop = nullptr);
int wm_stop_init(wm_ctx *ctx, const WmStopDev &stop, int B);
int wm_ts_init(wm_ctx *ctx, const WmTsDev &ts, int B);
int wm_range_softmax(wm_ctx *ctx, const float *logits, long ldo, int B, int first, int n, float *probs);
int wm_fill_synthetic(wm_ctx *ctx, const WmTensor &t, uint32_t seed, int tensor_id, float gain);
```

openai-whisper-coreml_amd/csrc/wm_internal.h:

```cpp
#pragma once
#include <hip/hip_runtime.h>
#include <stdint.h>
#include <exception>
#include <map>
#include <new>
#include <string>
#include <vector>

#include "../../include/whisper_mi355x.h"

void wm_set_error(const char *fmt, ...);

#define WM_HIP(expr)                                                                      \
    do {                                                                                  \
        hipError_t _e = (expr);                                                           \
        if (_e != hipSuccess) {                                                           \
            wm_set_error("%s:%d: %s failed: %s", __FILE__, __LINE__, #expr,               \
                         hipGetErrorString(_e));                                          \
            return WM_ERR_HIP;                                                            \
        }                                                                                 \
    } while (0)

#define WM_TRY(expr)                                                                      \
    do {                                                                                  \
        int _s = (expr);                                                                  \
        if (_s != WM_OK) return _s;                                                       \
    } while (0)

#define WM_REQUIRE(cond, code, ...)                                                       \
    do {                                                                                  \
        if (!(cond)) {                                                                    \
            wm_set_error(__VA_ARGS__);                                                    \
            return (code);                                                                \
        }                                                                                 \
    } while (0)

#define WM_API_CATCH                                                                      \
    catch (const std::bad_alloc &) {                                                      \
        wm_set_error("out of host memory");                                               \
        return WM_ERR_NOMEM;                                                              \
    }                                                                                     \
    catch (const std::exception &e) {                                                     \
        wm_set_error("internal error: %s", e.what());                                     \
        return WM_ERR_NOMEM;                                                              \
    }                                                                                     \
    catch (...) {                                                                         \
        wm_set_error("internal error (unknown exception)");                               \
        return WM_ERR_NOMEM;                                                              \
    }

constexpr int WM_N_SAMPLES = 480000;
constexpr int WM_N_FFT = 400;
constexpr int WM_HOP = 160;
constexpr int WM_N_BINS = 201;
constexpr int WM_N_FRAMES = 3000;
constexpr int WM_MEL_MAXW = 32;

typedef unsigned short bf16_t;

struct WmProfFamily {
    double ms = 0.0;
    long n = 0;
    std::vector<std::pair<hipEvent_t, hipEvent_t>> pending;
};

struct WmProfiler {
    bool on = false;
    std::map<std::string, WmProfFamily> fam;
    std::vector<hipEvent_t> pool;
    hipEvent_t get();
    void begin(const char *name, hipStream_t s, hipEvent_t *e0);
    void end(const char *name, hipStream_t s, hipEvent_t e0);
    void drain();
    void reset();
    ~WmProfiler();
};

struct WmProfScope {
    WmProfiler *p;
    const char *name;
    hipStream_t s;
    hipEvent_t e0 = nullptr;
    WmProfScope(WmProfiler *p_, const char *n, hipStream_t s_) : p(p_), name(n), s(s_) {
        if (p && p->on) p->begin(name, s, &e0);
    }
    ~WmProfScope() {
        if (p && p->on && e0) p->end(name, s, e0);
    }
};

struct WmFrontend {
    float *cos32 = nullptr, *sin32 = nullptr, *win32 = nullptr;
    double *cos64 = nullptr, *sin64 = nullptr, *win64 = nullptr;
    int *band_start[2] = {nullptr, nullptr};
    int *band_len[2] = {nullptr, nullptr};
    float *band_w[2] = {nullptr, nullptr};
    int band_maxw[2] = {0, 0};
    void *gmax = nullptr;
    int gmax_cap = 0;
    void *scratch = nullptr;
    size_t scratch_bytes = 0;
    bool ready = false;
};

int wm_frontend_init(WmFrontend *fe, hipStream_t stream);
void wm_frontend_destroy(WmFrontend *fe);
int wm_frontend_run(WmFrontend *fe, WmProfiler *prof, hipStream_t stream, const void *d_pcm,
                    wm_dtype pcm_dtype, int n_chunks, int n_mels, void *d_out,
                    wm_dtype out_dtype);
void wm_mel_filterbank(int n_mels, std::vector<float> &out );
const float *wm_mel80_table();

struct WmModel;
struct wm_ctx;

struct WmDebugHooks {
    int (*encode_dev)(wm_ctx *ctx, const float *d_mel, int B, float *d_xa);
    int (*decode_logits_dev)(wm_ctx *ctx, const int32_t *host_tokens , int B, int T, const float *d_xa,
                             float *d_logits );
};

struct wm_ctx {
    int device = 0;
    hipStream_t stream = nullptr;
    WmProfiler prof;
    WmFrontend fe;
    WmModel *model = nullptr;
    float stage_ms[3] = {0, 0, 0};
    std::vector<wm_ctx *> lanes;
    const WmDebugHooks *dbg_hooks = nullptr;
    int max_lanes = 0;
    int n_cus = 256, cu_lo = 0, cu_hi = 32;
    std::vector<wm_ctx *> part_lanes[2];
    bool no_cu_masks = false;
    std::map<int, wm_ctx *> solo_lanes;
};
int wm_clone_cus(wm_ctx *parent, int cu_lo, int cu_hi, wm_ctx **out);
int wm_cu_mask(int cu_lo, int cu_hi, uint32_t mask[8]);

int wm_ctx_make_current(const wm_ctx *ctx);
int wm_group_count(int B, int L, bool explicit_lanes, int gc_probe);
int wm_lane_parts(int B, int L, bool explicit_lanes, int n_text_state, int n_text_layer);

struct WmTuning {
    int gemv_tn = 0;
    int gemv_nblk = 0;
    int gemv_ppw2_nblk = 0;
    int gemv_no_ppw2 = 0;
    int prefetch_max_b = 16;
    int xattn_split_below = 96;
    int xattn_wgs = 256;
    int xattn_no_flat = 0;
    int xattn_lds_pad = 84 * 1024;
    int xattn_splits = 0;
    int gemm_tile = 0;
    int gemm_gm = 4;
    int gemm128_pipe = 0;
    int no_early_stop = 0;
    int logits_tn = 0;
    int enc_attn_mfma_sum = 0;
    int xattn_never_short = 0;
    int xattn_no_deep = 0;
    int xattn_fuse_q = 1;
    int argmax_rows_per_wg = 0;
    int group_chunks = 0;
    int frontend_per_wave_twiddles = 0;
    int lane_parts = 0;
    int lane_solo_cus = 0;
};
extern WmTuning g_wm_tuning;

#include <atomic>
extern std::atomic<int> g_wm_active_decodes[64];
```

Before: 2207.

## Compress cross-attention KV cache to a packed 12-bit format with bf16 fallback

```diff
diff --git a/include/whisper_mi355x_debug.h b/include/whisper_mi355x_debug.h
--- a/include/whisper_mi355x_debug.h
+++ b/include/whisper_mi355x_debug.h
@@ -22,6 +22,9 @@
                          float *stats, int B, int N, int K);
 WM_API int wmdbg_dec_attention(wm_ctx *ctx, const float *q, const float *k, const float *v, int B, int H, int T,
                         int n_keys, int nsplit, float *out);
+WM_API long wmdbg_xkv_plane_bytes(int T);
+WM_API int wmdbg_xkv_pack(wm_ctx *ctx, const uint16_t *src, int n_planes, int T, uint8_t *out, unsigned long long *stats);
+WM_API int wmdbg_xkv_stats(wm_ctx *ctx, unsigned long long *stats);
 
 WM_API int wmdbg_bench_dec_gemv(wm_ctx *ctx, int B, int N, int K, int ln, int resid, int n_mats, int iters,
                          int nw_override, float *avg_us);
diff --git a/openai-whisper-coreml_amd/csrc/debug_hooks.cpp b/openai-whisper-coreml_amd/csrc/debug_hooks.cpp
--- a/openai-whisper-coreml_amd/csrc/debug_hooks.cpp
+++ b/openai-whisper-coreml_amd/csrc/debug_hooks.cpp
@@ -21,7 +21,7 @@
         {"gemm_tile", &g_wm_tuning.gemm_tile}, {"gemm128_pipe", &g_wm_tuning.gemm128_pipe}, {"gemm_gm", &g_wm_tuning.gemm_gm}, {"no_early_stop", &g_wm_tuning.no_early_stop},
         {"xattn_no_deep", &g_wm_tuning.xattn_no_deep}, {"xattn_never_short", &g_wm_tuning.xattn_never_short},         {"logits_tn", &g_wm_tuning.logits_tn}, {"enc_attn_mfma_sum", &g_wm_tuning.enc_attn_mfma_sum},
         {"group_chunks", &g_wm_tuning.group_chunks}, {"argmax_rows_per_wg", &g_wm_tuning.argmax_rows_per_wg}, {"xattn_fuse_q", &g_wm_tuning.xattn_fuse_q},
-        {"lane_parts", &g_wm_tuning.lane_parts}, {"lane_solo_cus", &g_wm_tuning.lane_solo_cus}, {"frontend_per_wave_twiddles", &g_wm_tuning.frontend_per_wave_twiddles},
+        {"xkv_bf16", &g_wm_tuning.xkv_bf16}, {"lane_parts", &g_wm_tuning.lane_parts}, {"lane_solo_cus", &g_wm_tuning.lane_solo_cus}, {"frontend_per_wave_twiddles", &g_wm_tuning.frontend_per_wave_twiddles},
     };
     if (strcmp(key, "reset") == 0) { g_wm_tuning = WmTuning(); return WM_OK; }
     for (auto &e : table)
@@ -294,10 +294,19 @@
     WM_TRY(up(&dp, nullptr, (size_t)B * H * WM_MAXSPLIT * 66 * 4, s));
     void *datt;
     WM_TRY(up(&datt, nullptr, ((size_t)B + 15) / 16 * 16 * H * 64 * 2, s));
+    char *pk = nullptr, *pv = nullptr;
+    if (nsplit != 0 && !g_wm_tuning.xkv_bf16) {
+        const size_t pb = (size_t)B * H * wm_xkv_plane_bytes(T);
+        WM_TRY(up((void **)&pk, nullptr, pb, s));
+        WM_TRY(up((void **)&pv, nullptr, pb, s));
+        WM_TRY(wm_xkv_pack(ctx, (const bf16_t *)dk, pk, (long)B * H, T, nullptr));
+        WM_TRY(wm_xkv_pack(ctx, (const bf16_t *)dv, pv, (long)B * H, T, nullptr));
+    }
     int rc = nsplit == 0 ? wm_dec_self_attention(ctx, (const float *)dq, (const bf16_t *)dk, (const bf16_t *)dv, B, H, T,
                                                  n_keys, nullptr, (bf16_t *)datt)
                          : wm_dec_attention(ctx, (const float *)dq, (const bf16_t *)dk, (const bf16_t *)dv, B, H, T, n_keys,
-                                            nullptr, nsplit < 0 ? 1 : nsplit, (float *)dp, (bf16_t *)datt, nsplit < 0);
+                                            nullptr, nsplit < 0 ? 1 : nsplit, (float *)dp, (bf16_t *)datt, nsplit < 0, nullptr, 0,
+                                            0, nullptr, nullptr, false, pk, pv);
     if (rc == WM_OK) {
         const size_t Bpad = ((size_t)B + 15) / 16 * 16, dd = (size_t)H * 64;
         std::vector<bf16_t> o16(Bpad * dd), lin((size_t)B * dd);
@@ -308,6 +317,8 @@
         from_bf16(lin, out);
     }
     (void)hipFree(datt);
+    if (pk) (void)hipFree(pk);
+    if (pv) (void)hipFree(pv);
     (void)hipFree(dq); (void)hipFree(dk); (void)hipFree(dv); (void)hipFree(dp);
     return rc;
 }
@@ -378,6 +389,14 @@
     WM_TRY(up(&dq, nullptr, (size_t)B * H * 64 * 4, s));
     WM_TRY(up(&dp, nullptr, (size_t)B * H * WM_MAXSPLIT * 66 * 4, s));
     WM_TRY(up(&datt, nullptr, ((size_t)B + 15) / 16 * 16 * H * 64 * 2, s));
+    char *pk = nullptr, *pv = nullptr;
+    const size_t pslice = (size_t)B * H * wm_xkv_plane_bytes(T);
+    if (!g_wm_tuning.xkv_bf16) {
+        WM_TRY(up((void **)&pk, nullptr, pslice * n_slices, s));
+        WM_TRY(up((void **)&pv, nullptr, pslice * n_slices, s));
+        WM_TRY(wm_xkv_pack(ctx, (const bf16_t *)dk, pk, (long)B * H * n_slices, T, nullptr));
+        WM_TRY(wm_xkv_pack(ctx, (const bf16_t *)dv, pv, (long)B * H * n_slices, T, nullptr));
+    }
     hipEvent_t e0, e1;
     WM_HIP(hipEventCreate(&e0));
     WM_HIP(hipEventCreate(&e1));
@@ -387,7 +406,8 @@
         for (int i = 0; i < iters && rc == WM_OK; ++i)
             rc = wm_dec_attention(ctx, (const float *)dq, (const bf16_t *)dk + (size_t)(i % n_slices) * slice,
                                   (const bf16_t *)dv + (size_t)(i % n_slices) * slice, B, H, T, n_keys, nullptr, nsplit,
-                                  (float *)dp, (bf16_t *)datt, true);
+                                  (float *)dp, (bf16_t *)datt, true, nullptr, 0, 0, nullptr, nullptr, false,
+                                  pk ? pk + (i % n_slices) * pslice : nullptr, pv ? pv + (i % n_slices) * pslice : nullptr);
     }
     WM_HIP(hipEventRecord(e1, s));
     WM_HIP(hipStreamSynchronize(s));
@@ -395,9 +415,40 @@
     WM_HIP(hipEventElapsedTime(&ms, e0, e1));
     *avg_us = ms * 1e3f / iters;
     (void)hipEventDestroy(e0); (void)hipEventDestroy(e1);
-    void *fr[] = {dk, dv, dq, dp, datt};
-    for (void *p : fr) (void)hipFree(p);
-    return rc;
+    void *fr[] = {dk, dv, dq, dp, datt, pk, pv};
+    for (void *p : fr)
+        if (p) (void)hipFree(p);
+    return rc;
+}
+
+extern "C" long wmdbg_xkv_plane_bytes(int T) { return wm_xkv_plane_bytes(T); }
+extern "C" int wmdbg_xkv_pack(wm_ctx *ctx, const uint16_t *src, int n_planes, int T, uint8_t *out, unsigned long long *stats) {
+    WM_TRY(wm_ctx_make_current(ctx));
+    WM_REQUIRE(n_planes >= 1 && T >= 1, WM_ERR_INVALID, "wmdbg_xkv_pack: bad geometry");
+    hipStream_t s = ctx->stream;
+    const size_t in_bytes = (size_t)n_planes * T * 64 * 2, out_bytes = (size_t)n_planes * wm_xkv_plane_bytes(T);
+    void *din, *dout, *dst;
+    WM_TRY(up(&din, src, in_bytes, s));
+    WM_TRY(up(&dout, nullptr, out_bytes, s));
+    WM_TRY(up(&dst, nullptr, 3 * sizeof(unsigned long long), s));
+    int rc = wm_xkv_pack(ctx, (const bf16_t *)din, (char *)dout, n_planes, T, (unsigned long long *)dst);
+    unsigned long long st[3] = {0, 0, 0};
+    if (rc == WM_OK) {
+        WM_HIP(hipMemcpyAsync(out, dout, out_bytes, hipMemcpyDeviceToHost, s));
+        WM_HIP(hipMemcpyAsync(st, dst, sizeof(st), hipMemcpyDeviceToHost, s));
+        WM_HIP(hipStreamSynchronize(s));
+        for (int i = 0; i < 3; ++i) stats[i] += st[i];
+    }
+    (void)hipFree(din); (void)hipFree(dout); (void)hipFree(dst);
+    return rc;
+}
+
+extern "C" int wmdbg_xkv_stats(wm_ctx *ctx, unsigned long long *stats) {
+    WM_TRY(wm_ctx_make_current(ctx));
+    WM_REQUIRE(ctx->model, WM_ERR_STATE, "wmdbg_xkv_stats: context has no model");
+    WM_HIP(hipStreamSynchronize(ctx->stream));
+    WM_HIP(hipMemcpy(stats, ctx->model->xkv_stats, 3 * sizeof(unsigned long long), hipMemcpyDeviceToHost));
+    return WM_OK;
 }
 
 int wm_launch_trivial(wm_ctx *ctx, int *p, int grid);
diff --git a/openai-whisper-coreml_amd/csrc/dec_kernels.hip b/openai-whisper-coreml_amd/csrc/dec_kernels.hip
--- a/openai-whisper-coreml_amd/csrc/dec_kernels.hip
+++ b/openai-whisper-coreml_amd/csrc/dec_kernels.hip
@@ -534,6 +534,72 @@
     }
 }
 
+constexpr int XKV_ROW_BYTES = 96;
+__host__ __device__ constexpr long xkv_plane_bytes(int T_stride) { return (long)T_stride * XKV_ROW_BYTES + ATT_MAXK * 4L; }
+__device__ __forceinline__ int xkv_meta_index(int i) { return (i >> 8) * 256 + (i & 63) * 4 + ((i >> 6) & 3); }
+typedef unsigned u32x3a __attribute__((ext_vector_type(3), aligned(4)));
+
+__device__ __forceinline__ u32x4 xkv_decode(u32x3a d, unsigned meta) {
+    const unsigned t03 = __builtin_amdgcn_perm(meta, meta, 0u) + 0x01020304u;
+    const unsigned cw = d[2];
+    const unsigned h0 = __builtin_amdgcn_perm(meta, t03, cw & 0x07070707u) | ((cw << 4) & 0x80808080u);
+    const unsigned h1 = __builtin_amdgcn_perm(meta, t03, (cw >> 4) & 0x07070707u) | (cw & 0x80808080u);
+    u32x4 w;
+    w[0] = __builtin_amdgcn_perm(h0, d[0], 0x05010400u);
+    w[1] = __builtin_amdgcn_perm(h0, d[0], 0x07030602u);
+    w[2] = __builtin_amdgcn_perm(h1, d[1], 0x05010400u);
+    w[3] = __builtin_amdgcn_perm(h1, d[1], 0x07030602u);
+    return w;
+}
+
+template <int NS, int U, bool NT>
+__device__ __forceinline__ void attn_load_block_packed(const char *kp, const char *vp, const unsigned *km, const unsigned *vm,
+                                                       const bf16_t *kx, const bf16_t *vx, unsigned kml, unsigned vml, int r0,
+                                                       const int &stream, const int &rg, int lim, int clamp, u32x4 (&kv)[U],
+                                                       u32x4 (&vv)[U]) {
+    static_assert(NS == 8 && U == 4, "the metadata layout is written for 8 streams of 4 rows per block");
+    const int mo = (r0 >> 8) * 256 + (stream * 8 + rg) * 4;
+    u32x4 km4, vm4;
+    u32x3a kd[U], vd[U];
+    int row[U];
+    if (NT) {
+        km4 = __builtin_nontemporal_load((const u32x4 *)(km + mo));
+        vm4 = __builtin_nontemporal_load((const u32x4 *)(vm + mo));
+    } else {
+        km4 = *(const u32x4 *)(km + mo);
+        vm4 = *(const u32x4 *)(vm + mo);
+    }
+#pragma unroll
+    for (int u = 0; u < U; ++u) {
+        int i = r0 + u * (NS * 8) + stream * 8 + rg;
+        const bool in = i < lim;
+        row[u] = in ? i : clamp;
+        if (NT) {
+            kd[u] = __builtin_nontemporal_load((const u32x3a *)(kp + (long)row[u] * XKV_ROW_BYTES));
+            vd[u] = __builtin_nontemporal_load((const u32x3a *)(vp + (long)row[u] * XKV_ROW_BYTES));
+        } else {
+            kd[u] = *(const u32x3a *)(kp + (long)row[u] * XKV_ROW_BYTES);
+            vd[u] = *(const u32x3a *)(vp + (long)row[u] * XKV_ROW_BYTES);
+        }
+        if (!in) {
+            km4[u] = kml;
+            vm4[u] = vml;
+        }
+    }
+#pragma unroll
+    for (int u = 0; u < U; ++u) {
+        kv[u] = xkv_decode(kd[u], km4[u]);
+        vv[u] = xkv_decode(vd[u], vm4[u]);
+    }
+    if (((km4[0] | km4[1] | km4[2] | km4[3] | vm4[0] | vm4[1] | vm4[2] | vm4[3]) & 0x80u) != 0u) {
+#pragma unroll
+        for (int u = 0; u < U; ++u) {
+            if (km4[u] & 0x80u) kv[u] = *(const u32x4 *)(kx + (long)row[u] * 64);
+            if (vm4[u] & 0x80u) vv[u] = *(const u32x4 *)(vx + (long)row[u] * 64);
+        }
+    }
+}
+
 template <int U>
 __device__ __forceinline__ void attn_block_fence(u32x4 (&kv)[U], u32x4 (&vv)[U]) {
     static_assert(U == 4, "attn_block_fence is written for 4 loads per block");
@@ -600,8 +666,9 @@
     float *part;
     const char *pf_ptr;
     long pf_tile_bytes;
+    const bf16_t *kx, *vx;
 };
-template <int NS, int U, bool NT, bool DEEP = false>
+template <int NS, int U, bool NT, bool DEEP = false, bool PK = false>
 __global__ __launch_bounds__(DEEP ? 256 : NS * 64) void dec_rows_attn_kernel(
     const float *__restrict__ q, const bf16_t *__restrict__ kc, const bf16_t *__restrict__ vc,
     const int *__restrict__ pos_ptr, const int *__restrict__ live_rows ,
@@ -634,8 +701,16 @@
     const int pos_raw = *(pos_ptr ? pos_ptr : dummy);
     const int nl_raw = *(n_live_ptr ? n_live_ptr : dummy);
     const int n_clamp = SELF ? T_stride - 1 : n_keys_const - 1;
+    const char *kp = nullptr, *vp = nullptr;
     auto load_block = [&](const bf16_t *kb, const bf16_t *vb, int r0, int clamp, u32x4 (&kv)[U], u32x4 (&vv)[U]) {
-        attn_load_block<NS, U, NT>(kb, vb, r0, stream, rg, clamp, clamp, kv, vv);
+        if constexpr (PK) {
+            const unsigned *km = (const unsigned *)(kp + (long)T_stride * XKV_ROW_BYTES);
+            const unsigned *vm = (const unsigned *)(vp + (long)T_stride * XKV_ROW_BYTES);
+            attn_load_block_packed<NS, U, NT>(kp + e8 * 12, vp + e8 * 12, km, vm, kb, vb, km[xkv_meta_index(clamp)],
+                                              vm[xkv_meta_index(clamp)], r0, stream, rg, clamp, clamp, kv, vv);
+        } else {
+            attn_load_block<NS, U, NT>(kb, vb, r0, stream, rg, clamp, clamp, kv, vv);
+        }
     };
     bool first = true;
     int n_bh = n_bh_full, n_keys = n_keys_const;
@@ -645,8 +720,10 @@
         int b = pi / H;
         if (live_rows) b = live_rows[pi / H];
         const int bh = b * H + h;
-        const bf16_t *kb = kc + (long)bh * T_stride * 64 + e8 * 8;
-        const bf16_t *vb = vc + (long)bh * T_stride * 64 + e8 * 8;
+        const bf16_t *kb = (PK ? cold.kx : kc) + (long)bh * T_stride * 64 + e8 * 8;
+        const bf16_t *vb = (PK ? cold.vx : vc) + (long)bh * T_stride * 64 + e8 * 8;
+        kp = (const char *)kc + (long)bh * xkv_plane_bytes(T_stride);
+        vp = (const char *)vc + (long)bh * xkv_plane_bytes(T_stride);
         const f32x4 *qp = (const f32x4 *)(q + (long)b * d + h * 64 + e8 * 8);
         const f32x4 q0 = qp[0], q1 = qp[1];
         constexpr bool SPEC = SELF || DEEP;
@@ -719,7 +796,7 @@
     }
 }
 
-template <int NS, int U, bool NT, bool DEEP = false>
+template <int NS, int U, bool NT, bool DEEP = false, bool PK = false>
 __global__ __launch_bounds__(DEEP ? 256 : NS * 64) void dec_xrows_attn_kernel(
     const float *__restrict__ q, const bf16_t *__restrict__ kc, const bf16_t *__restrict__ vc,
     const int *__restrict__ pos_ptr, const int *__restrict__ live_rows ,
@@ -760,8 +837,17 @@
         const int h = pi % H;
         const int b = live_rows ? live_rows[pi / H] : pi / H;
         const int bh = b * H + h;
-        const bf16_t *kb = kc + (long)bh * T_stride * 64 + e8 * 8;
-        const bf16_t *vb = vc + (long)bh * T_stride * 64 + e8 * 8;
+        const bf16_t *kb = (PK ? cold.kx : kc) + (long)bh * T_stride * 64 + e8 * 8;
+        const bf16_t *vb = (PK ? cold.vx : vc) + (long)bh * T_stride * 64 + e8 * 8;
+        const char *kp = (const char *)kc + (long)bh * xkv_plane_bytes(T_stride), *vp = (const char *)vc + (long)bh * xkv_plane_bytes(T_stride);
+        const unsigned *km = (const unsigned *)(kp + (long)T_stride * XKV_ROW_BYTES), *vm = (const unsigned *)(vp + (long)T_stride * XKV_ROW_BYTES);
+        unsigned kml = 0, vml = 0;
+        if (PK) {
+            kml = km[xkv_meta_index(last)];
+            vml = vm[xkv_meta_index(last)];
+            kp += e8 * 12;
+            vp += e8 * 12;
+        }
         float qe[8];
         {
             const float *qp = q + (long)b * d + h * 64 + e8 * 8;
@@ -771,7 +857,10 @@
         float m_run = -1e30f, l_run = 0.f;
         float oa[8] = {0, 0, 0, 0, 0, 0, 0, 0};
         auto load_block = [&](int r0, u32x4 (&kv)[U], u32x4 (&vv)[U]) {
-            attn_load_block<NS, U, NT>(kb, vb, r0, stream, rg, n_keys, last, kv, vv);
+            if constexpr (PK)
+                attn_load_block_packed<NS, U, NT>(kp, vp, km, vm, kb, vb, kml, vml, r0, stream, rg, n_keys, last, kv, vv);
+            else
+                attn_load_block<NS, U, NT>(kb, vb, r0, stream, rg, n_keys, last, kv, vv);
         };
         auto process_block = [&](int r0, const u32x4 (&kv)[U], const u32x4 (&vv)[U]) {
             attn_block<NS, U, false>(qe, r0, stream, rg, n_keys, kv, vv, m_run, l_run, oa);
@@ -828,8 +917,9 @@
     const char *pf_ptr;
     long pf_tile_bytes;
     int n_wg;
+    const bf16_t *kx, *vx;
 };
-template <int SPW, bool NT>
+template <int SPW, bool NT, bool PK = false>
 __global__ __launch_bounds__(512) void dec_xattn_fq_kernel(const bf16_t *__restrict__ Wq, const bf16_t *__restrict__ xb,
                                                            const bf16_t *__restrict__ kc, const bf16_t *__restrict__ vc,
                                                            const int *__restrict__ live_rows, unsigned packA ,
@@ -878,10 +968,21 @@
     if (wave < 4) gemv_unit_load<DE_Q, true>(p, ops, my_tile, blk * 16, lane, 0, 4, true);
     const int stream = wave;
     const int bh = b * H + h;
-    const bf16_t *kb = kc + (long)bh * T_stride * 64 + e8 * 8;
-    const bf16_t *vb = vc + (long)bh * T_stride * 64 + e8 * 8;
+    const bf16_t *kb = (PK ? cold.kx : kc) + (long)bh * T_stride * 64 + e8 * 8;
+    const bf16_t *vb = (PK ? cold.vx : vc) + (long)bh * T_stride * 64 + e8 * 8;
+    const char *kp = (const char *)kc + (long)bh * xkv_plane_bytes(T_stride), *vp = (const char *)vc + (long)bh * xkv_plane_bytes(T_stride);
+    const unsigned *km = (const unsigned *)(kp + (long)T_stride * XKV_ROW_BYTES), *vm = (const unsigned *)(vp + (long)T_stride * XKV_ROW_BYTES);
+    unsigned kml = 0, vml = 0;
+    if (PK) {
+        kml = km[xkv_meta_index(n_keys - 1)];
+        vml = vm[xkv_meta_index(n_keys - 1)];
+    }
     auto load_block = [&](int r0, u32x4 (&kv)[U], u32x4 (&vv)[U]) {
-        attn_load_block<NS, U, NT>(kb, vb, r0, stream, rg, n_keys - 1, n_keys - 1, kv, vv);
+        if constexpr (PK)
+            attn_load_block_packed<NS, U, NT>(kp + e8 * 12, vp + e8 * 12, km, vm, kb, vb, kml, vml, r0, stream, rg, n_keys - 1,
+                                              n_keys - 1, kv, vv);
+        else
+            attn_load_block<NS, U, NT>(kb, vb, r0, stream, rg, n_keys - 1, n_keys - 1, kv, vv);
     };
     u32x4 kv0[U], vv0[U];
     load_block(0, kv0, vv0);
@@ -961,6 +1062,52 @@
         ll[w] = wl_[w];
     }
     att[wm_tiled_offset((size_t)b, (size_t)(h * 64 + e), (size_t)d)] = f2bf(attn_merge_core<NS>(mm, ll, oo));
+}
+
+__global__ __launch_bounds__(256) void xkv_pack_kernel(const bf16_t *__restrict__ src, char *__restrict__ dst, long n_planes,
+                                                       int T_stride, unsigned long long *__restrict__ stats) {
+    const int lane = threadIdx.x & 63;
+    const long gr = (long)blockIdx.x * 4 + (threadIdx.x >> 6);
+    const long plane = gr / ATT_MAXK;
+    const int i = (int)(gr % ATT_MAXK);
+    if (plane >= n_planes) return;
+    char *pd = dst + plane * xkv_plane_bytes(T_stride);
+    unsigned *meta = (unsigned *)(pd + (long)T_stride * XKV_ROW_BYTES);
+    if (i >= T_stride) {
+        if (lane == 0) meta[xkv_meta_index(i)] = 0u;
+        return;
+    }
+    const unsigned x = ((const unsigned short *)src)[(plane * T_stride + i) * 64 + lane];
+    const int h7 = (int)((x >> 8) & 0x7fu);
+    int mx = h7;
+#pragma unroll
+    for (int o = 1; o < 64; o <<= 1) mx = max(mx, __shfl_xor(mx, o));
+    const int base = max(mx, 6);
+    const bool esc = base - h7 > 6;
+    int emax = esc ? h7 : -1, emin = esc ? h7 : 128;
+#pragma unroll
+    for (int o = 1; o < 64; o <<= 1) {
+        emax = max(emax, __shfl_xor(emax, o));
+        emin = min(emin, __shfl_xor(emin, o));
+    }
+    const unsigned code = (esc ? 7u : (unsigned)(base - h7)) | ((x >> 12) & 8u);
+    const unsigned hi_code = __shfl_down(code, 4);
+    const int e8 = lane >> 3, k = lane & 7;
+    char *row = pd + (long)i * XKV_ROW_BYTES + e8 * 12;
+    row[k] = (char)(x & 0xffu);
+    if (k < 4) row[8 + k] = (char)(code | hi_code << 4);
+    const unsigned long long n_esc = __popcll(__ballot(esc));
+    if (lane == 0) {
+        const bool ovf = emax >= 0 && emax != emin;
+        meta[xkv_meta_index(i)] = ovf ? 0xffffffffu
+                                      : (unsigned)(base - 4) | (unsigned)(base - 5) << 8 | (unsigned)(base - 6) << 16 |
+                                            (unsigned)(emax < 0 ? 0 : emax) << 24;
+        if (stats && n_esc) {
+            atomicAdd(&stats[0], n_esc);
+            atomicAdd(&stats[1], 1ull);
+            if (ovf) atomicAdd(&stats[2], 1ull);
+        }
+    }
 }
 
 __global__ __launch_bounds__(1024) void argmax_embed_kernel(const unsigned long long *__restrict__ tilemax,
@@ -1439,7 +1586,7 @@
 int wm_dec_attention(wm_ctx *ctx, const float *q, const bf16_t *kc, const bf16_t *vc, int B, int H,
                      int T_stride, int n_keys, const int *pos_ptr, int nsplit, float *part, bf16_t *att,
                      bool cross, const bf16_t *pf_ptr, int pf_rows, int pf_k, const int *live_rows, const int *n_live,
-                     bool short_lived) {
+                     bool short_lived, const char *pk, const char *pv) {
     WM_REQUIRE(nsplit == 1 || nsplit == 2 || nsplit == 4 || nsplit == 8, WM_ERR_INVALID,
                "dec_attention: nsplit %d is not 1, 2, 4 or 8", nsplit);
     WM_REQUIRE(T_stride <= ATT_MAXK && n_keys <= ATT_MAXK, WM_ERR_INVALID,
@@ -1447,6 +1594,8 @@
     WM_REQUIRE(nsplit == 1 || part != nullptr, WM_ERR_INVALID, "dec_attention: split launch without a partials buffer");
     WM_REQUIRE(H >= 1 && H <= 255 && B * H < 65536, WM_ERR_INVALID, "dec_attention: %d heads x %d rows do not fit the packed arguments", H, B);
     WM_REQUIRE((!live_rows && !n_live) || n_live == live_rows + WM_DEC_MAXB, WM_ERR_INVALID, "dec_attention: the live count must follow the live rows");
+    WM_REQUIRE(!pk == !pv && (!pk || !pos_ptr), WM_ERR_INVALID, "dec_attention: a packed cache needs both planes and a fixed key count");
+    const bf16_t *kin = pk ? (const bf16_t *)pk : kc, *vin = pk ? (const bf16_t *)pv : vc;
     {
         WmProfScope ps(&ctx->prof, cross ? "dec_attn_cross" : "dec_attn_self", ctx->stream);
         const int cap_cus = g_wm_tuning.xattn_wgs > 0 && g_wm_tuning.xattn_wgs < ctx->n_cus ? g_wm_tuning.xattn_wgs : ctx->n_cus;
@@ -1468,19 +1617,22 @@
             int wpw = (units + 255) / 256;
             wpw = wpw < 1 ? 1 : (wpw > 4 ? 4 : wpw);
             const int g = (units + wpw - 1) / wpw;
-            const AttnCold cold = {att, part, nullptr, 0};
+            const AttnCold cold = {att, part, nullptr, 0, kc, vc};
             const unsigned pA = (unsigned)H | (8u << 8) | ((unsigned)wpw << 16), pB = (unsigned)T_stride | ((unsigned)n_keys << 16);
             const unsigned pC = (unsigned)(B * H) | ((unsigned)g << 16);
             WM_REQUIRE(g < 65536, WM_ERR_INVALID, "dec_attention: flat grid too large");
+#define WM_XATTN_LAUNCH(KERNEL, ...)                                                                               \
+    do {                                                                                                           \
+        if (pk) KERNEL<__VA_ARGS__, true><<<g, wpw * 64, 0, ctx->stream>>>(q, kin, vin, pos_ptr, live_rows, pA, pB, pC, cold); \
+        else KERNEL<__VA_ARGS__, false><<<g, wpw * 64, 0, ctx->stream>>>(q, kc, vc, pos_ptr, live_rows, pA, pB, pC, cold);   \
+    } while (0)
             if (g_wm_tuning.xattn_no_deep)
-                dec_xrows_attn_kernel<8, 4, WM_XATTN_NT><<<g, wpw * 64, 0, ctx->stream>>>(
-                    q, kc, vc, pos_ptr, live_rows, pA, pB, pC, cold);
+                WM_XATTN_LAUNCH(dec_xrows_attn_kernel, 8, 4, WM_XATTN_NT, false);
             else if ((size_t)B * H * T_stride * 64 * 2 * 2 <= (size_t)3200 * 1024)
-                dec_rows_attn_kernel<8, 4, false, true><<<g, wpw * 64, 0, ctx->stream>>>(
-                    q, kc, vc, pos_ptr, live_rows, pA, pB, pC, cold);
+                WM_XATTN_LAUNCH(dec_rows_attn_kernel, 8, 4, false, true);
             else
-                dec_rows_attn_kernel<8, 4, WM_XATTN_NT, true><<<g, wpw * 64, 0, ctx->stream>>>(
-                    q, kc, vc, pos_ptr, live_rows, pA, pB, pC, cold);
+                WM_XATTN_LAUNCH(dec_rows_attn_kernel, 8, 4, WM_XATTN_NT, true);
+#undef WM_XATTN_LAUNCH
         } else {
             dim3 grid(gx, nsplit);
             const int lds_pad = g_wm_tuning.xattn_lds_pad;
@@ -1488,13 +1640,19 @@
             if (lds_pad > pad_set[ctx->device & 63].load(std::memory_order_acquire)) {
                 WM_HIP(hipFuncSetAttribute((const void *)dec_xrows_attn_kernel<8, 4, WM_XATTN_NT>,
                                            hipFuncAttributeMaxDynamicSharedMemorySize, lds_pad));
+                WM_HIP(hipFuncSetAttribute((const void *)dec_xrows_attn_kernel<8, 4, WM_XATTN_NT, false, true>,
+                                           hipFuncAttributeMaxDynamicSharedMemorySize, lds_pad));
                 pad_set[ctx->device & 63].store(lds_pad, std::memory_order_release);
             }
-            const AttnCold cold = {att, part, (const char *)pf_ptr, tile_bytes};
+            const AttnCold cold = {att, part, (const char *)pf_ptr, tile_bytes, kc, vc};
             const unsigned pA = (unsigned)H | ((unsigned)nsplit << 8), pB = (unsigned)T_stride | ((unsigned)n_keys << 16);
             const unsigned pC = (unsigned)(B * H) | ((unsigned)n_wg << 16);
-            dec_xrows_attn_kernel<8, 4, WM_XATTN_NT><<<grid, (8 / nsplit) * 64, nsplit == 1 ? lds_pad : 0, ctx->stream>>>(
-                q, kc, vc, pos_ptr, live_rows, pA, pB, pC, cold);
+            if (pk)
+                dec_xrows_attn_kernel<8, 4, WM_XATTN_NT, false, true><<<grid, (8 / nsplit) * 64, nsplit == 1 ? lds_pad : 0, ctx->stream>>>(
+                    q, kin, vin, pos_ptr, live_rows, pA, pB, pC, cold);
+            else
+                dec_xrows_attn_kernel<8, 4, WM_XATTN_NT><<<grid, (8 / nsplit) * 64, nsplit == 1 ? lds_pad : 0, ctx->stream>>>(
+                    q, kc, vc, pos_ptr, live_rows, pA, pB, pC, cold);
         }
         WM_HIP(hipGetLastError());
     }
@@ -1516,7 +1674,8 @@
 }
 
 int wm_dec_xattn_fq(wm_ctx *ctx, const DecGemvArgs &qa, const bf16_t *kc, const bf16_t *vc, int B, int H, int T_stride,
-                    int n_keys, bf16_t *att, const int *live_rows, const int *n_live, const bf16_t *pf_ptr, int pf_rows, int pf_k) {
+                    int n_keys, bf16_t *att, const int *live_rows, const int *n_live, const bf16_t *pf_ptr, int pf_rows, int pf_k,
+                    const char *pk, const char *pv) {
     WM_REQUIRE(qa.c1 && qa.stats_in && qa.N == qa.K && qa.K == H * 64, WM_ERR_INVALID, "xattn_fq: not a LayerNorm-folded d x d query projection");
     WM_REQUIRE(H >= 1 && H <= 255 && B >= 1 && B <= WM_DEC_MAXB && T_stride <= ATT_MAXK && n_keys >= 1 && n_keys <= ATT_MAXK,
                WM_ERR_INVALID, "xattn_fq: bad geometry");
@@ -1524,6 +1683,7 @@
     int spw = 0;
     const int nw = wm_dec_gemv_split(qa.K, &spw);
     WM_REQUIRE(nw >= 1 && nw <= 8, WM_ERR_INVALID, "xattn_fq: K split over more than 8 waves");
+    WM_REQUIRE(!pk == !pv, WM_ERR_INVALID, "xattn_fq: a packed cache needs both planes");
     WmProfScope ps(&ctx->prof, "dec_attn_cross_fq", ctx->stream);
     FqCold cold;
     cold.c1 = qa.c1; cold.c2 = qa.c2; cold.stats_in = qa.stats_in; cold.mean_in = qa.mean_in; cold.mean_out = qa.mean_out;
@@ -1531,6 +1691,8 @@
     const unsigned pA = (unsigned)H | ((unsigned)B << 8), pB = (unsigned)T_stride | ((unsigned)n_keys << 16);
     int grid = 8 * ((H * B + 7) / 8);
     cold.n_wg = grid; cold.pf_ptr = nullptr; cold.pf_tile_bytes = 0;
+    cold.kx = kc; cold.vx = vc;
+    const bf16_t *kin = pk ? (const bf16_t *)pk : kc, *vin = pk ? (const bf16_t *)pv : vc;
     if (pf_enabled(B) && pf_ptr && pf_rows >= 16) {
         cold.pf_ptr = (const char *)pf_ptr;
         cold.pf_tile_bytes = 16L * pf_k * 2;
@@ -1539,12 +1701,36 @@
     const size_t lds = ((size_t)nw * 1024 + 128 + 64) * sizeof(float);
     hipStream_t s = ctx->stream;
     switch (spw) {
-        case 2: dec_xattn_fq_kernel<2, WM_XATTN_NT><<<grid, 512, lds, s>>>(qa.W, qa.a, kc, vc, live_rows, pA, pB, qa.K, cold); break;
-        case 4: dec_xattn_fq_kernel<4, WM_XATTN_NT><<<grid, 512, lds, s>>>(qa.W, qa.a, kc, vc, live_rows, pA, pB, qa.K, cold); break;
-        case 5: dec_xattn_fq_kernel<5, WM_XATTN_NT><<<grid, 512, lds, s>>>(qa.W, qa.a, kc, vc, live_rows, pA, pB, qa.K, cold); break;
-        case 6: dec_xattn_fq_kernel<6, WM_XATTN_NT><<<grid, 512, lds, s>>>(qa.W, qa.a, kc, vc, live_rows, pA, pB, qa.K, cold); break;
+        case 2:
+            if (pk) dec_xattn_fq_kernel<2, WM_XATTN_NT, true><<<grid, 512, lds, s>>>(qa.W, qa.a, kin, vin, live_rows, pA, pB, qa.K, cold);
+            else dec_xattn_fq_kernel<2, WM_XATTN_NT><<<grid, 512, lds, s>>>(qa.W, qa.a, kc, vc, live_rows, pA, pB, qa.K, cold);
+            break;
+        case 4:
+            if (pk) dec_xattn_fq_kernel<4, WM_XATTN_NT, true><<<grid, 512, lds, s>>>(qa.W, qa.a, kin, vin, live_rows, pA, pB, qa.K, cold);
+            else dec_xattn_fq_kernel<4, WM_XATTN_NT><<<grid, 512, lds, s>>>(qa.W, qa.a, kc, vc, live_rows, pA, pB, qa.K, cold);
+            break;
+        case 5:
+            if (pk) dec_xattn_fq_kernel<5, WM_XATTN_NT, true><<<grid, 512, lds, s>>>(qa.W, qa.a, kin, vin, live_rows, pA, pB, qa.K, cold);
+            else dec_xattn_fq_kernel<5, WM_XATTN_NT><<<grid, 512, lds, s>>>(qa.W, qa.a, kc, vc, live_rows, pA, pB, qa.K, cold);
+            break;
+        case 6:
+            if (pk) dec_xattn_fq_kernel<6, WM_XATTN_NT, true><<<grid, 512, lds, s>>>(qa.W, qa.a, kin, vin, live_rows, pA, pB, qa.K, cold);
+            else dec_xattn_fq_kernel<6, WM_XATTN_NT><<<grid, 512, lds, s>>>(qa.W, qa.a, kc, vc, live_rows, pA, pB, qa.K, cold);
+            break;
         default: wm_set_error("xattn_fq: unsupported k-steps per wave %d", spw); return WM_ERR_INVALID;
     }
+    WM_HIP(hipGetLastError());
+    return WM_OK;
+}
+
+long wm_xkv_plane_bytes(int T_stride) { return xkv_plane_bytes(T_stride); }
+
+int wm_xkv_pack(wm_ctx *ctx, const bf16_t *src, char *dst, long n_planes, int T_stride, unsigned long long *stats) {
+    WM_REQUIRE(T_stride >= 1 && T_stride <= ATT_MAXK && n_planes >= 1, WM_ERR_INVALID, "xkv_pack: bad geometry");
+    WmProfScope ps(&ctx->prof, "xkv_pack", ctx->stream);
+    const long blocks = n_planes * (ATT_MAXK / 4);
+    WM_REQUIRE(blocks < (1L << 31), WM_ERR_INVALID, "xkv_pack: too many planes");
+    xkv_pack_kernel<<<(unsigned)blocks, 256, 0, ctx->stream>>>(src, dst, n_planes, T_stride, stats);
     WM_HIP(hipGetLastError());
     return WM_OK;
 }
diff --git a/openai-whisper-coreml_amd/csrc/model.cpp b/openai-whisper-coreml_amd/csrc/model.cpp
--- a/openai-whisper-coreml_amd/csrc/model.cpp
+++ b/openai-whisper-coreml_amd/csrc/model.cpp
@@ -54,6 +54,7 @@
     WM_TRY(dalloc_t(m, &m->dseq, (size_t)WM_DEC_MAXB * (D.n_text_ctx + 1), s));
     WM_TRY(dalloc_t(m, &m->dpos, 4, s));
     WM_TRY(dalloc_t(m, &m->darrive, 4, s));
+    WM_TRY(dalloc_t(m, &m->xkv_stats, 3, s));
     WM_TRY(dalloc_t(m, &m->ddone, WM_DEC_MAXB, s));
     WM_TRY(dalloc_t(m, &m->dbudget, WM_DEC_MAXB, s));
     WM_TRY(dalloc_t(m, &m->dlive, WM_DEC_MAXB + 4, s));
@@ -412,7 +413,7 @@
     WM_REQUIRE(m, WM_ERR_STATE, "context has no model");
     if (B <= m->cap_b) return WM_OK;
     WM_HIP(hipStreamSynchronize(ctx->stream));
-    void *olds[] = {m->mel_t, m->h1p, m->x, m->xn, m->qk, m->vt, m->att, m->hid, m->xa_f32, m->mel_f32, m->xkv, m->skv};
+    void *olds[] = {m->mel_t, m->h1p, m->x, m->xn, m->qk, m->vt, m->att, m->hid, m->xa_f32, m->mel_f32, m->xkv, m->xkvp, m->skv};
     for (void *p : olds)
         if (p) {
             (void)hipFree(p);
@@ -434,6 +435,7 @@
     WM_TRY(dalloc_t(m, &m->xa_f32, M * d, s));
     WM_TRY(dalloc_t(m, &m->mel_f32, (size_t)B * D.n_mels * WM_N_FRAMES, s));
     WM_TRY(dalloc_t(m, &m->xkv, (size_t)D.n_text_layer * 2 * B * H * 1500 * 64, s));
+    WM_TRY(dalloc_t(m, &m->xkvp, (size_t)D.n_text_layer * 2 * B * H * wm_xkv_plane_bytes(1500), s));
     const int Bd = B < WM_DEC_MAXB ? B : WM_DEC_MAXB;
     WM_TRY(dalloc_t(m, &m->skv, (size_t)D.n_text_layer * 2 * Bd * H * D.n_text_ctx * 64, s));
     m->cap_b = B;
@@ -512,6 +514,8 @@
                                 EPI_XKV);
         g.d_model = d; g.n_head = H; g.seq = S; g.batch = B;
         WM_TRY(wm_gemm(ctx, g));
+        WM_TRY(wm_xkv_pack(ctx, m->xkv + (size_t)l * 2 * B * H * S * 64, m->xkvp + (size_t)l * 2 * B * H * wm_xkv_plane_bytes(S),
+                           2L * B * H, S, m->xkv_stats));
     }
     return WM_OK;
 }
@@ -552,6 +556,11 @@
         bf16_t *vc = m->skv + (size_t)(l * 2 + 1) * B * H * T * 64;
         const bf16_t *xk = m->xkv + (size_t)(l * 2 + 0) * B * H * S * 64;
         const bf16_t *xv = m->xkv + (size_t)(l * 2 + 1) * B * H * S * 64;
+        const char *pk = nullptr, *pv = nullptr;
+        if (!g_wm_tuning.xkv_bf16) {
+            pk = m->xkvp + (size_t)(l * 2 + 0) * B * H * wm_xkv_plane_bytes(S);
+            pv = m->xkvp + (size_t)(l * 2 + 1) * B * H * wm_xkv_plane_bytes(S);
+        }
         DecGemvArgs a;
         memset(&a, 0, sizeof(a));
         a.epi = DE_QKV; a.B = B; a.N = 3 * d; a.K = d; a.W = L.wqkv_f; a.c1 = L.qkv_c1; a.c2 = L.qkv_c2;
@@ -576,10 +585,11 @@
         a.stats_in = m->dstats;
         a.mean_in = mean_buf(cur); a.mean_out = mean_buf(cur ^ 1); cur ^= 1;
         if (fuse_q) {
-            WM_TRY(wm_dec_xattn_fq(ctx, a, xk, xv, B, H, S, S, m->datt, live, nlive, L.wxo, d, d));
+            WM_TRY(wm_dec_xattn_fq(ctx, a, xk, xv, B, H, S, S, m->datt, live, nlive, L.wxo, d, d, pk, pv));
         } else {
             WM_TRY(wm_dec_gemv(ctx, a));
-            WM_TRY(wm_dec_attention(ctx, m->dq, xk, xv, B, H, S, S, nullptr, xns, m->dpart, m->datt, true, L.wxo, d, d, live, nlive, xshort));
+            WM_TRY(wm_dec_attention(ctx, m->dq, xk, xv, B, H, S, S, nullptr, xns, m->dpart, m->datt, true, L.wxo, d, d, live, nlive, xshort,
+                                    pk, pv));
         }
         memset(&a, 0, sizeof(a));
         a.epi = DE_RESID; a.B = B; a.N = d; a.K = d; a.W = L.wxo; a.c2 = L.bxo;
diff --git a/openai-whisper-coreml_amd/csrc/model.h b/openai-whisper-coreml_amd/csrc/model.h
--- a/openai-whisper-coreml_amd/csrc/model.h
+++ b/openai-whisper-coreml_amd/csrc/model.h
@@ -97,6 +97,8 @@
     float *xa_f32 = nullptr;
     float *mel_f32 = nullptr;
     bf16_t *xkv = nullptr;
+    char *xkvp = nullptr;
+    unsigned long long *xkv_stats = nullptr;
     bf16_t *skv = nullptr;
     float *dx = nullptr;
     bf16_t *dxb = nullptr;
@@ -256,7 +258,7 @@
 bool wm_dec_xattn_fq_applies(int B, int H, int K, bool short_lived);
 int wm_dec_xattn_fq(wm_ctx *ctx, const DecGemvArgs &qa, const bf16_t *kc, const bf16_t *vc, int B, int H, int T_stride,
                     int n_keys, bf16_t *att, const int *live_rows, const int *n_live, const bf16_t *pf_ptr = nullptr,
-                    int pf_rows = 0, int pf_k = 0);
+                    int pf_rows = 0, int pf_k = 0, const char *pk = nullptr, const char *pv = nullptr);
 int wm_dec_gemv_split(int K, int *spw);
 int wm_ln_fold(wm_ctx *ctx, const bf16_t *W, const float *g, const float *beta, const float *bias , int N,
                int K, bf16_t *Wf, float *c1, float *c2);
@@ -266,7 +268,10 @@
 int wm_dec_attention(wm_ctx *ctx, const float *q, const bf16_t *kc, const bf16_t *vc, int B, int H,
                      int T_stride, int n_keys, const int *pos_ptr, int nsplit, float *part, bf16_t *att,
                      bool cross, const bf16_t *pf_ptr = nullptr, int pf_rows = 0, int pf_k = 0,
-                     const int *live_rows = nullptr, const int *n_live = nullptr, bool short_lived = false);
+                     const int *live_rows = nullptr, const int *n_live = nullptr, bool short_lived = false,
+                     const char *pk = nullptr, const char *pv = nullptr);
+long wm_xkv_plane_bytes(int T_stride);
+int wm_xkv_pack(wm_ctx *ctx, const bf16_t *src, char *dst, long n_planes, int T_stride, unsigned long long *stats);
 int wm_dec_self_attention(wm_ctx *ctx, const float *q, const bf16_t *kc, const bf16_t *vc, int B, int H, int T_stride,
                           int n_keys, const int *pos_ptr, bf16_t *att, const bf16_t *pf_ptr = nullptr, int pf_rows = 0,
                           int pf_k = 0, const int *live_rows = nullptr, const int *n_live = nullptr);
diff --git a/openai-whisper-coreml_amd/csrc/wm_internal.h b/openai-whisper-coreml_amd/csrc/wm_internal.h
--- a/openai-whisper-coreml_amd/csrc/wm_internal.h
+++ b/openai-whisper-coreml_amd/csrc/wm_internal.h
@@ -166,6 +166,7 @@
     int group_chunks = 0;
     int frontend_per_wave_twiddles = 0;
     int lane_parts = 0;
+    int xkv_bf16 = 0;
     int lane_solo_cus = 0;
 };
 extern WmTuning g_wm_tuning;
```

After: 2180, median of 6. Within noise of the previous version (-1.2%).
